# sshaoshuai/PointRCNN

Hardware: AMD Instinct MI355X
Metric: KITTI frames/sec, RPN inference end-to-end (16384 pts/frame, bs32 per GPU) (higher is better)
Workload: dtype f32 via split-bf16x6 MFMA (every fp32 operand cut exactly into 3 bf16 pieces, 6 bf16 MFMA products per fp32 product, fp32 accumulate: fp32-grade, measured error 2.9e-7 of sum|x||w| vs 3.0e-7 for the fp32-MFMA kernel; hoisted grouped layers on the split kernel too, unhoisted grouped first layers (xyz; 1 GPU; Full RPN PointNet++ backbone (4 SA-MSG + 4 FP) + cls/reg heads, tools/cfgs/default.yaml, 16384 pts/frame, batch 32 per GPU, random-init weights, eval-mode BN; frames_per_gpu=32, npoints=16384, parallelism=frames sharded, dp1, launch=hipGraph replay, streams=20, hw_queues=4, proposal_layer=normal, clouds=uniform, group_dedup=True, roi_dedup=True

## Files before the change

include/prcnn_pointops.h:

```cpp
#ifndef PRCNN_POINTOPS_H
#define PRCNN_POINTOPS_H

#include <stddef.h>
#include <stdint.h>

#ifdef __cplusplus
extern "C" {
#endif

typedef void* prcnn_stream_t;

#define PRCNN_OK 0
#define PRCNN_EINVAL (-1)
#define PRCNN_EHIP (-2)
#define PRCNN_EUNSUPPORTED (-3)

int prcnn_abi_version(void);
const char* prcnn_last_error(void);
const char* prcnn_build_id(void);
int prcnn_switches_reload(void);
int prcnn_switch_get(const char* name, int* set, long* num);


int prcnn_fps(const float* xyz, int B, int N, int npoint, float* tmp, int32_t* idx, prcnn_stream_t stream);

int prcnn_fps_nested(const float* xyz, const int32_t* prev_idx, int B, int N, int npoint, float* tmp, int32_t* idx, int32_t* skip,
                     prcnn_stream_t stream);

int prcnn_fps_status(void);

#define PRCNN_FPS_ORDER_CANONICAL 0
#define PRCNN_FPS_ORDER_UPSTREAM 1
int prcnn_fps_order(const float* xyz, int B, int N, int npoint, int order, float* tmp, int32_t* idx, prcnn_stream_t stream);

#define PRCNN_ARITH_CANONICAL 0
#define PRCNN_ARITH_UPSTREAM 1
int prcnn_fps_mode(const float* xyz, int B, int N, int npoint, int order, int arith, float* tmp, int32_t* idx, prcnn_stream_t stream);
int prcnn_ball_query_arith(const float* xyz, const float* new_xyz, int B, int N, int M, float radius, int nsample, int arith,
                           int32_t* idx, prcnn_stream_t stream);
int prcnn_three_nn_arith(const float* unknown, const float* known, int B, int n, int m, int arith, float* dist2, int32_t* idx,
                         prcnn_stream_t stream);

int prcnn_gather(const float* feat, const int32_t* idx, int B, int C, int N, int M, float* out, prcnn_stream_t stream);
int prcnn_gather_grad(const float* grad_out, const int32_t* idx, int B, int C, int N, int M, float* grad_feat,
                      prcnn_stream_t stream);

int prcnn_gather_rows(const float* in_cl, int ld_in, const int32_t* idx, int B, int N, int M, int C, float* out,
                      prcnn_stream_t stream);

int prcnn_ball_query(const float* xyz, const float* new_xyz, int B, int N, int M, float radius, int nsample,
                     int32_t* idx, prcnn_stream_t stream);
int prcnn_ball_query2(const float* xyz, const float* new_xyz, int B, int N, int M, float radius_a, int nsample_a,
                      int32_t* idx_a, float radius_b, int nsample_b, int32_t* idx_b, prcnn_stream_t stream);

int prcnn_group(const float* feat, const int32_t* idx, int B, int C, int N, int M, int nsample, float* out,
                prcnn_stream_t stream);
int prcnn_group_grad(const float* grad_out, const int32_t* idx, int B, int C, int N, int M, int nsample,
                     float* grad_feat, prcnn_stream_t stream);

int prcnn_three_nn(const float* unknown, const float* known, int B, int n, int m, float* dist2, int32_t* idx,
                   float* weight, prcnn_stream_t stream);

int prcnn_three_interp(const float* feat, const int32_t* idx, const float* weight, int B, int C, int m, int n,
                       float* out, prcnn_stream_t stream);
int prcnn_three_interp_grad(const float* grad_out, const int32_t* idx, const float* weight, int B, int C, int n,
                            int m, float* grad_feat, float* workspace, prcnn_stream_t stream);


size_t prcnn_wpack_floats(int Nout, int K);
int prcnn_pack_weight(const float* w, int Nout, int K, int k_rot, float* wpack, prcnn_stream_t stream);

int prcnn_mlp_rows(const float* in, int ld_in, int64_t rows, int K, const float* wpack, const float* bias, int Nout,
                   int relu, float* out, int ld_out, int col_off, int pool_ns, const int32_t* rows_dev, int rows_unit,
                   const int32_t* seg_cnt, int seg_rows, prcnn_stream_t stream);

int prcnn_mlp_group(const float* xyz, const float* new_xyz, const int32_t* idx, const float* feat_cl, int ld_feat,
                    int B, int N, int M, int nsample, int C, const float* act_wx, const float* act_bias,
                    const float* wpack, const float* bias, int Nout, int relu, float* out, int ld_out, int col_off,
                    int pool_ns, const int32_t* groups_dev, prcnn_stream_t stream);

int prcnn_mlp_interp(const float* known_cl, int ld_known, const int32_t* idx3, const float* w3, const float* skip_cl,
                     int ld_skip, int B, int n, int m, int C2, int C1, const float* act_bias, const float* wpack,
                     const float* bias, int Nout, int relu, float* out, int ld_out, int col_off,
                     prcnn_stream_t stream);

int prcnn_mlp_rows_addinterp(const float* in, int ld_in, int K, const float* wpack, const float* bias, int Nout,
                             int relu, const float* y_cl, int ld_y, const int32_t* idx3, const float* w3, int B, int n,
                             int m, float* out, int ld_out, int col_off, prcnn_stream_t stream);

size_t prcnn_wsplit_bytes(int Nout, int K);
int prcnn_pack_weight_split(const float* w, int Nout, int K, int chain, void* wsplit, prcnn_stream_t stream);
int prcnn_mlp_rows_split(const float* in, int ld_in, int64_t rows, int K, const float* wpack, const void* wsplit, int terms,
                         const float* bias, int Nout, int relu, float* out, int ld_out, int col_off, int pool_ns,
                         const int32_t* rows_dev, int rows_unit, const int32_t* seg_cnt, int seg_rows, prcnn_stream_t stream);
int prcnn_mlp_chain_rows_split(const float* in, int ld_in, int64_t rows, int K, const void* const* wchain, const float* const* wpack,
                               const float* const* bias, const int* nout, const int* relu, int terms, float* out, int ld_out,
                               int col_off, prcnn_stream_t stream);
int prcnn_mlp_chain_interp_split(const float* known_cl, int ld_known, const int32_t* idx3, const float* w3, int B, int n, int m,
                                 int C2, const float* act_bias, const void* wchain, const float* wpack, const float* bias, int Nout,
                                 int relu, int terms, float* out, int ld_out, int col_off, prcnn_stream_t stream);
int prcnn_mlp_rows_addinterp_split(const float* in, int ld_in, int K, const float* wpack, const void* wsplit, int terms,
                                   const float* bias, int Nout, int relu, const float* y_cl, int ld_y, const int32_t* idx3,
                                   const float* w3, int B, int n, int m, float* out, int ld_out, int col_off,
                                   prcnn_stream_t stream);
int prcnn_mlp_group_split(const float* xyz, const float* new_xyz, const int32_t* idx, const float* feat_cl, int ld_feat, int B, int N,
                          int M, int nsample, int C, const float* act_wx, const float* act_bias, const float* wpack,
                          const void* wsplit, int terms, const float* bias, int Nout, int relu, float* out, int ld_out, int col_off,
                          int pool_ns, const int32_t* groups_dev, prcnn_stream_t stream);

int prcnn_mlp_chain_supported(int mode, int nlayers, const int* nout, int pool_ns);
int prcnn_mlp_chain_rows(const float* in, int ld_in, int64_t rows, int K, int nlayers, const float* const* wpack,
                         const float* const* bias, const int* nout, const int* relu, float* out, int ld_out,
                         int col_off, int pool_ns, const int32_t* seg_cnt, int seg_rows, prcnn_stream_t stream);
int prcnn_mlp_chain_group(const float* xyz, const float* new_xyz, const int32_t* idx, const float* feat_cl,
                          int ld_feat, int B, int N, int M, int nsample, int C, const float* act_wx,
                          const float* act_bias, int nlayers,
                          const float* const* wpack, const float* const* bias, const int* nout, const int* relu,
                          float* out, int ld_out, int col_off, int pool_ns, const int32_t* groups_dev, prcnn_stream_t stream);
int prcnn_mlp_chain_interp(const float* known_cl, int ld_known, const int32_t* idx3, const float* w3,
                           const float* skip_cl, int ld_skip, int B, int n, int m, int C2, int C1,
                           const float* act_bias, int nlayers, const float* const* wpack, const float* const* bias, const int* nout, const int* relu,
                           float* out, int ld_out, int col_off, prcnn_stream_t stream);

typedef struct prcnn_chain_group_problem {
    const float* xyz; const float* new_xyz; const int32_t* idx; const float* feat_cl;
    const float* act_wx; const float* act_bias;
    const float* const* wpack; const float* const* bias; const int* nout; const int* relu;
    float* out; const int32_t* groups_dev;
    int ld_feat, B, N, M, nsample, C, nlayers, ld_out, col_off, pool_ns;
} prcnn_chain_group_problem_t;
int prcnn_mlp_chain_group_multi(int nprob, const prcnn_chain_group_problem_t* prob, prcnn_stream_t stream);

int prcnn_maxpool_rows(const float* in, int ld_in, int64_t rows_out, int ns, int C, float* out, int ld_out,
                       int col_off, prcnn_stream_t stream);

int prcnn_roipool3d(const float* xyz, const float* boxes3d, const float* feat, int B, int N, int M, int C, int S,
                    float* pooled, int32_t* empty, prcnn_stream_t stream);
size_t prcnn_roipool3d_work_bytes(int B, int N);
int prcnn_roipool3d_ws(const float* xyz, const float* boxes3d, const float* feat, int B, int N, int M, int C, int S, float* pooled,
                       int32_t* empty, void* work, size_t work_bytes, prcnn_stream_t stream);

int prcnn_pts_in_boxes3d(const float* pts, const float* boxes3d, int N, int M, int32_t* flags, prcnn_stream_t stream);

int prcnn_rpn_labels(const float* pts, const float* gt_boxes3d, const int32_t* num_gt, int B, int N, int G, float extra_width,
                     int32_t* cls_label, float* reg_label, prcnn_stream_t stream);

int prcnn_gt_aug_edit(const float* pts, const float* intensity, const int32_t* num_pts, const float* boxes3d,
                      const int32_t* num_boxes, float extra_h, const float* new_pts, const float* new_intensity,
                      const int32_t* num_new, int B, int N, int K, int P, float* out_pts, float* out_intensity,
                      int32_t* out_count, int32_t* removed, prcnn_stream_t stream);

int prcnn_corner_iou3d(const float* corners_a, int N, const float* corners_b, int M, float* iou3d, float* iou_bev, prcnn_stream_t stream);

int prcnn_gt_aug_sample(const float* gt_boxes3d, const int32_t* num_gt, const double* planes, int B, int G, const float* db_boxes, const float* db_alpha, const int32_t* db_npts, int D, const int32_t* easy_idx, int E, const int32_t* hard_idx, int H, const double* cfg4, const double* scope, int try_times, int K, uint32_t seed, int32_t* count, int32_t* db_id, float* boxes3d, float* alpha, double* y_shift, int32_t* stats, int32_t* status, prcnn_stream_t stream);

int prcnn_host_pts_in_boxes3d(const float* pts, const float* boxes3d, int64_t N, int64_t M, int64_t* flags);
int prcnn_host_roipool3d(const float* pts, const float* boxes3d, const float* feat, int64_t N, int64_t M, int64_t C, int64_t S,
                         float* pooled_pts, float* pooled_feat, int64_t* empty);

int prcnn_boxes_overlap_bev(const float* boxes_a, int Na, const float* boxes_b, int Nb, float* out,
                            prcnn_stream_t stream);
int prcnn_boxes_iou_bev(const float* boxes_a, int Na, const float* boxes_b, int Nb, float* out, prcnn_stream_t stream);

#define PRCNN_NMS_ROTATED 0
#define PRCNN_NMS_NORMAL 1
size_t prcnn_nms_workspace_bytes(int N);
int prcnn_nms(const float* boxes, int N, float thresh, int kind, int max_keep, int64_t* keep, int32_t* num_keep,
              void* workspace, size_t workspace_bytes, prcnn_stream_t stream);


int prcnn_decode_bbox_target(const float* roi, int roi_cols, const float* pred_reg, long N, int C, double loc_scope,
                             double loc_bin_size, int num_head_bin, const float* anchor_size_host, int get_xz_fine,
                             int get_y_by_bin, double loc_y_scope, double loc_y_bin_size, int get_ry_fine, int y_to_bottom,
                             float* out, prcnn_stream_t stream);

size_t prcnn_proposal_workspace_bytes(int B, int N, int pre_max, int post_max);
int prcnn_proposal_layer(const float* scores, const float* boxes3d, int B, int N, int use_range, float r0, float r1, float r2,
                         int pre1, int pre2, int post1, int post2, float nms_thresh, int nms_kind, float* out_boxes,
                         float* out_scores, int32_t* out_count, void* workspace, size_t workspace_bytes, prcnn_stream_t stream);

size_t prcnn_nms_batched_workspace_bytes(int B, int M);
int prcnn_nms_batched(const float* boxes3d, const float* scores, const uint8_t* valid, int B, int M, float thresh, int kind,
                      int max_keep, int32_t* keep, int32_t* num_keep, void* workspace, size_t workspace_bytes,
                      prcnn_stream_t stream);

int prcnn_roipool3d_canonical(const float* xyz, const float* pool_boxes3d, const float* rois, const float* extra0,
                              const float* extra1, const float* feat, int ld_feat, int B, int N, int M, int C, int S,
                              float* out_pts, int ld_pts, float* out_feat, int ld_out, int32_t* empty, int32_t* distinct,
                              prcnn_stream_t stream);
int prcnn_roipool3d_canonical_ws(const float* xyz, const float* pool_boxes3d, const float* rois, const float* extra0,
                                 const float* extra1, const float* feat, int ld_feat, int B, int N, int M, int C, int S,
                                 float* out_pts, int ld_pts, float* out_feat, int ld_out, int32_t* empty, int32_t* distinct,
                                 void* work, size_t work_bytes, prcnn_stream_t stream);

size_t prcnn_grid_bytes(int B, int N);
int prcnn_grid_build(const float* xyz, int B, int N, float min_cell, int cells_per_axis, void* grid, size_t grid_bytes,
                     prcnn_stream_t stream);
int prcnn_ball_query2_grid(const void* grid, const float* xyz, const float* new_xyz, int B, int N, int M, float radius_a,
                           int nsample_a, int32_t* idx_a, float radius_b, int nsample_b, int32_t* idx_b, prcnn_stream_t stream);
int prcnn_three_nn_grid(const void* grid, const float* unknown, int B, int n, int m, float* dist2, int32_t* idx, float* weight,
                        prcnn_stream_t stream);

int prcnn_rotate_iou_eval(const float* boxes, int N, const float* query, int K, int criterion, float* out, prcnn_stream_t stream);
int prcnn_kitti_overlaps(int metric, const double* dt, const int32_t* dt_off, const double* gt, const int32_t* gt_off,
                         const int64_t* ov_off, int F, double* out, prcnn_stream_t stream);
int prcnn_kitti_statistics(const double* overlaps, const int64_t* ov_off, const double* gt_datas, const int32_t* gt_off,
                           const double* dt_datas, const int32_t* dt_off, const int32_t* ign_gt, const int32_t* ign_det,
                           const double* dc, const int32_t* dc_off, int F, int max_det_per_frame, int metric, double min_overlap,
                           const double* thresholds, int T, int compute_fp, int compute_aos, double* res, double* matched,
                           prcnn_stream_t stream);

int prcnn_group_compact(const int32_t* idx, const float* new_xyz, int B, int N, int M, int nsample, int sparse_max,
                        const int32_t* valid_n, int32_t* ridx, float* rnx, int32_t* slist, int32_t* soff, int32_t* scnt,
                        int32_t* idxn, float* nxn, int32_t* listn, int32_t* counts, prcnn_stream_t stream);
int prcnn_segmax_scatter(const float* src, int ld_src, const int32_t* list, const int32_t* off, const int32_t* cnt,
                         const int32_t* count, int max_groups, int C, float* dst, int ld_dst, int col_off, prcnn_stream_t stream);
int prcnn_scatter_rows(const float* src, int ld_src, const int32_t* list, const int32_t* count, int max_rows, int C, float* dst,
                       int ld_dst, int col_off, prcnn_stream_t stream);
int prcnn_group_compact_pair(const int32_t* idx_a, int ns_a, int T_a, const int32_t* idx_b, int ns_b, int T_b, const float* new_xyz,
                             int B, int N, int M, void* const* lists_a, void* const* lists_b, int32_t* counts, prcnn_stream_t stream);
int prcnn_level_pool(int nprob, const float* const* src, const int* ld_src, const int32_t* const* list, const int32_t* const* off,
                     const int32_t* const* cnt, const int32_t* const* count, const int* max_items, const int* C, const int* col_off,
                     float* dst, int ld_dst, prcnn_stream_t stream);

size_t prcnn_scene_workspace_bytes(int64_t total_points, int B);
int prcnn_scene_prepare(const float* raw, const int64_t* offsets, int B, int64_t total_points, int max_points_per_frame,
                        const float* calib, const int32_t* img_hw, const double* scope, int npoints, uint32_t seed,
                        float* out_xyz, float* out_intensity, int32_t* out_src, int32_t* nvalid, int32_t* status,
                        void* workspace, size_t workspace_bytes, prcnn_stream_t stream);

size_t prcnn_train_scene_workspace_bytes(int64_t total_points, int B, int K, int db_max_points);
int prcnn_train_scene_prepare(const float* raw, const int64_t* offsets, int B, int64_t total_points, int max_points_per_frame,
                              const float* calib, const int32_t* img_hw, const double* scope, int npoints, uint32_t seed,
                              const float* gt_boxes3d, const float* gt_alpha, const int32_t* num_gt, int G,
                              const int32_t* acc_count, const int32_t* acc_db_id, const float* acc_boxes3d, const float* acc_alpha,
                              const double* acc_y_shift, const int32_t* acc_status, int K, const float* db_points,
                              const float* db_intensity, const int64_t* db_offsets, int D, int db_max_points,
                              const double* aug_cfg, float* out_xyz, float* out_input, float* out_features, int32_t* out_src,
                              int32_t* nvalid, int32_t* status, float* out_gt_boxes3d, int32_t* out_num_gt, double* aug,
                              void* workspace, size_t workspace_bytes, prcnn_stream_t stream);

size_t prcnn_gt_database_workspace_bytes(int64_t max_points_per_frame, int B, int G);
int prcnn_gt_database_count(const float* raw, const int64_t* offsets, int B, int64_t total_points, int max_points_per_frame,
                            const float* calib, const float* boxes3d, const int32_t* num_boxes, int G, int32_t* npts,
                            void* workspace, size_t workspace_bytes, prcnn_stream_t stream);
int prcnn_gt_database_fill(const float* raw, const int64_t* offsets, int B, int64_t total_points, int max_points_per_frame,
                           const float* calib, const float* boxes3d, const int32_t* num_boxes, int G, const int64_t* obj_offsets,
                           int64_t total_out, float* points, float* intensity, int32_t* src, void* workspace,
                           size_t workspace_bytes, prcnn_stream_t stream);

int prcnn_aug_scene_sample(const float* gt_boxes3d, const int32_t* num_gt, const double* planes, const int32_t* frame_ids, int B, int G,
                           const float* db_boxes, const int32_t* db_npts, int D, const double* scope, int K, uint32_t seed,
                           int32_t* count, int32_t* db_id, float* boxes3d, double* y_shift, int32_t* stats, int32_t* status,
                           prcnn_stream_t stream);
size_t prcnn_aug_scene_workspace_bytes(int64_t max_points_per_frame, int B);
int prcnn_aug_scene_count(const float* raw, const int64_t* offsets, int B, int64_t total_points, int max_points_per_frame,
                          const float* calib, const int32_t* img_hw, const double* scope, const int32_t* acc_count,
                          const int32_t* acc_db_id, const float* acc_boxes3d, const int32_t* acc_status, int K,
                          const int64_t* db_offsets, int D, int64_t db_total_points, int32_t* rows, void* workspace,
                          size_t workspace_bytes, prcnn_stream_t stream);
int prcnn_aug_scene_fill(const float* raw, const int64_t* offsets, int B, int64_t total_points, int max_points_per_frame,
                         const float* calib, const int32_t* img_hw, const double* scope, const int32_t* acc_count,
                         const int32_t* acc_db_id, const float* acc_boxes3d, const double* acc_y_shift, const int32_t* acc_status,
                         int K, const float* db_points, const float* db_intensity, const int64_t* db_offsets, int D,
                         int64_t db_total_points, const int64_t* out_offsets, int64_t total_out, float* out, int32_t* src,
                         void* workspace, size_t workspace_bytes, prcnn_stream_t stream);

typedef struct prcnn_train_src {
    int mode;
    int64_t rows;
    int K;
    const float* in; int ld_in; const float* pro_scale; const float* pro_shift;
    const float* xyz; const float* new_xyz; const int32_t* idx; const float* feat; int ld_feat; int B, N, M, ns, C;
    const float* known; const int32_t* idx3; const float* w3; const float* skip; int ld_known, ld_skip, n, m, C2, C1;
    const float* mult; const int32_t* rows_dev; int64_t norm_rows; const int32_t* seg_off; const int32_t* seg_cnt; const int32_t* row_grp;
    int groups;
} prcnn_train_src_t;

typedef struct prcnn_train_layer {
    int Nout;
    const float* W; const float* gamma; const float* beta;
    float eps, momentum;
    float* running_mean; float* running_var;
    float* y;
    float* cst; int ld_c;
    float* wpack; float* wpack_t;
    float* dW; float* dgamma; float* dbeta;
} prcnn_train_layer_t;

size_t prcnn_train_stack_work_bytes(int64_t rows, const prcnn_train_layer_t* layers, int nl, int K0, int backward);
int prcnn_train_stack_fwd(const prcnn_train_src_t* src, const prcnn_train_layer_t* layers, int nl, int pool_ns, float* a_dump, int ld_dump,
                          float* out, int ld_out, int col_off, uint8_t* arg, void* work, size_t work_bytes, prcnn_stream_t stream);
int prcnn_train_stack_bwd(const prcnn_train_src_t* src, const prcnn_train_layer_t* layers, int nl, int pool_ns, const float* a_dump,
                          int ld_dump, const float* gout, int ld_gout, const uint8_t* arg, float* gin, int ld_gin, void* work,
                          size_t work_bytes, prcnn_stream_t stream);
int prcnn_train_stack_fwd_split(const prcnn_train_src_t* src, const prcnn_train_layer_t* layers, int nl, int pool_ns, float* a_dump,
                                int ld_dump, float* out, int ld_out, int col_off, uint8_t* arg, void* const* wsplit, void* work,
                                size_t work_bytes, prcnn_stream_t stream);
int prcnn_train_stack_bwd_split(const prcnn_train_src_t* src, const prcnn_train_layer_t* layers, int nl, int pool_ns, const float* a_dump,
                                int ld_dump, const float* gout, int ld_gout, const uint8_t* arg, float* gin, int ld_gin,
                                void* const* wsplit_t, void* work, size_t work_bytes, prcnn_stream_t stream);
int prcnn_train_stack_bwd_wsplit(const prcnn_train_src_t* src, const prcnn_train_layer_t* layers, int nl, int pool_ns, const float* a_dump,
                                 int ld_dump, const float* gout, int ld_gout, const uint8_t* arg, float* gin, int ld_gin,
                                 void* const* wsplit_t, void* work, size_t work_bytes, prcnn_stream_t stream);
int prcnn_train_group_rows(const int32_t* idx, const float* new_xyz, int B, int N, int M, int ns, int32_t* cnt, int32_t* off,
                           int32_t* rows_dev, int32_t* ridx, float* rnx, float* mult, int32_t* row_grp, prcnn_stream_t stream);
int prcnn_flat_rows_grad(const float* G, int ldG, const int32_t* ridx, const int32_t* rows_dev, int64_t max_rows, int C, float* dfeat,
                         int ld_d, prcnn_stream_t stream);
size_t prcnn_flat_rows_grad_work_bytes(int B, int N, int64_t max_rows);
int prcnn_flat_rows_grad_ws(const float* G, int ldG, const int32_t* ridx, const int32_t* rows_dev, int64_t max_rows, int C, float* dfeat,
                            int ld_d, const int32_t* seg_off, int B, int N, int M, void* work, size_t work_bytes, prcnn_stream_t stream);
int prcnn_group_rows_grad(const float* G, int ldG, const int32_t* idx, int B, int M, int ns, int C, int N, float* dfeat, int ld_d,
                          prcnn_stream_t stream);
int prcnn_interp_rows_grad(const float* G, int ldG, const int32_t* idx3, const float* w3, int B, int n, int m, int C, float* dknown,
                           int ld_d, prcnn_stream_t stream);
size_t prcnn_interp_rows_grad_work_bytes(int B, int n, int m);
int prcnn_interp_rows_grad_ws(const float* G, int ldG, const int32_t* idx3, const float* w3, int B, int n, int m, int C, float* dknown,
                              int ld_d, void* work, size_t work_bytes, prcnn_stream_t stream);

int prcnn_boxes_iou3d(const float* a, int Na, const float* b, int Nb, float* out, prcnn_stream_t stream);
int prcnn_ref_trig(const float* a, const float* b, int n, int fn, float* out, prcnn_stream_t stream);
int prcnn_proposal_target_sample(const float* roi_boxes3d, const float* gt_boxes3d, int B, int M, int G, int gt_cols, int roi_per_image,
                                 const double* cfg6, int aug_times, int aug_method, uint32_t seed, float* rois, float* gt_of_rois,
                                 float* roi_iou, int32_t* src, float* max_overlaps, int32_t* gt_assignment, int32_t* counts,
                                 int32_t* status, prcnn_stream_t stream);

int prcnn_rcnn_offline_sample(const float* roi_boxes3d, const int32_t* num_roi, const float* gt_boxes3d, const int32_t* num_gt,
                              const int32_t* frame_ids, int B, int M, int G, int roi_per_image, const double* cfg6, int aug_times,
                              int aug_method, uint32_t seed, float* iou3d, float* rois, float* gt_of_rois, float* roi_iou, int32_t* src,
                              float* max_overlaps, int32_t* gt_assignment, int32_t* counts, int32_t* status, prcnn_stream_t stream);

int prcnn_rcnn_offline_finish(float* pooled, int ld, int B, int R, int S, const float* rois, const float* gt_of_rois,
                              const float* roi_iou, const int32_t* pooled_empty_flag, const int32_t* status, const int32_t* frame_ids,
                              const double* cfg5, int aug_methods, uint32_t seed, float* out_rois, float* out_gt_of_rois,
                              float* gt_boxes3d_ct, int32_t* cls_label, int32_t* reg_valid_mask, prcnn_stream_t stream);

typedef struct prcnn_rpn_loss_cfg {
    double loc_scope, loc_bin_size;
    double mean_size[3];
    double gamma, alpha;
    double loss_weight[2];
    int num_head_bin, xz_fine, y_by_bin, ry_fine;
    int loss_cls;
    int has_alpha;
} prcnn_rpn_loss_cfg_t;
size_t prcnn_rpn_loss_workspace_bytes(int64_t npts);
int prcnn_rpn_loss_counts(const void* cls_label, int label_is_i64, int64_t npts, int32_t* counts, float* norm, void* work,
                          size_t work_bytes, prcnn_stream_t stream);
int prcnn_rpn_loss_forward(const float* rpn_cls, int64_t ld_cls, const float* rpn_reg, int64_t ld_reg, const void* cls_label,
                           int label_is_i64, const float* reg_label, int64_t npts, int C, const prcnn_rpn_loss_cfg_t* cfg,
                           const int32_t* counts, const float* norm, float* terms, void* work, size_t work_bytes, prcnn_stream_t stream);
int prcnn_rpn_loss_backward(const float* rpn_cls, int64_t ld_cls, const float* rpn_reg, int64_t ld_reg, const void* cls_label,
                            int label_is_i64, const float* reg_label, int64_t npts, int C, const prcnn_rpn_loss_cfg_t* cfg,
                            const int32_t* counts, const float* norm, const float* grad_out, float* dcls, float* dreg,
                            prcnn_stream_t stream);
int prcnn_rpn_loss_cls_sums(const float* rpn_cls, int64_t ld_cls, const void* cls_label, int label_is_i64, int64_t npts, double* cls_sums,
                            void* work, size_t work_bytes, prcnn_stream_t stream);
int prcnn_rpn_loss_forward_kind(const float* rpn_cls, int64_t ld_cls, const float* rpn_reg, int64_t ld_reg, const void* cls_label,
                                int label_is_i64, const float* reg_label, int64_t npts, int C, const prcnn_rpn_loss_cfg_t* cfg,
                                const int32_t* counts, const float* norm, float* terms, void* work, size_t work_bytes,
                                const double* cls_sums, double fg_weight, prcnn_stream_t stream);
int prcnn_rpn_loss_backward_kind(const float* rpn_cls, int64_t ld_cls, const float* rpn_reg, int64_t ld_reg, const void* cls_label,
                                 int label_is_i64, const float* reg_label, int64_t npts, int C, const prcnn_rpn_loss_cfg_t* cfg,
                                 const int32_t* counts, const float* norm, const float* grad_out, float* dcls, float* dreg,
                                 const double* cls_sums, double fg_weight, prcnn_stream_t stream);

typedef struct prcnn_rcnn_loss_cfg {
    double loc_scope, loc_bin_size;
    double loc_y_scope, loc_y_bin_size;
    double mean_size[3];
    double gamma, alpha;
    int num_head_bin, y_by_bin, size_res_on_roi;
    int loss_cls;
    int has_alpha;
} prcnn_rcnn_loss_cfg_t;
size_t prcnn_rcnn_loss_workspace_bytes(int64_t npts);
// ... 65 lines not shown
```

pointrcnn_amd/_cabi.py:

```python
import contextlib
import ctypes
import os

from . import build as _build

_P = ctypes.c_void_p
_I = ctypes.c_int
_F = ctypes.c_float
_L = ctypes.c_int64
_Z = ctypes.c_size_t
_D = ctypes.c_double
_U = ctypes.c_uint32



class TrainSrc(ctypes.Structure):
    _fields_ = [("mode", _I), ("rows", _L), ("K", _I),
                ("in_", _P), ("ld_in", _I), ("pro_scale", _P), ("pro_shift", _P),
                ("xyz", _P), ("new_xyz", _P), ("idx", _P), ("feat", _P), ("ld_feat", _I),
                ("B", _I), ("N", _I), ("M", _I), ("ns", _I), ("C", _I),
                ("known", _P), ("idx3", _P), ("w3", _P), ("skip", _P), ("ld_known", _I), ("ld_skip", _I),
                ("n", _I), ("m", _I), ("C2", _I), ("C1", _I),
                ("mult", _P), ("rows_dev", _P), ("norm_rows", _L), ("seg_off", _P), ("seg_cnt", _P), ("row_grp", _P), ("groups", _I)]


class TrainLayer(ctypes.Structure):
    _fields_ = [("Nout", _I), ("W", _P), ("gamma", _P), ("beta", _P), ("eps", _F), ("momentum", _F),
                ("running_mean", _P), ("running_var", _P), ("y", _P), ("cst", _P), ("ld_c", _I), ("wpack", _P), ("wpack_t", _P),
                ("dW", _P), ("dgamma", _P), ("dbeta", _P)]


class ChainGroupProblem(ctypes.Structure):
    _fields_ = [("xyz", _P), ("new_xyz", _P), ("idx", _P), ("feat_cl", _P), ("act_wx", _P), ("act_bias", _P),
                ("wpack", _P), ("bias", _P), ("nout", _P), ("relu", _P), ("out", _P), ("groups_dev", _P),
                ("ld_feat", _I), ("B", _I), ("N", _I), ("M", _I), ("nsample", _I), ("C", _I), ("nlayers", _I), ("ld_out", _I),
                ("col_off", _I), ("pool_ns", _I)]


class RpnLossCfg(ctypes.Structure):
    _fields_ = [("loc_scope", _D), ("loc_bin_size", _D), ("mean_size", _D * 3), ("gamma", _D), ("alpha", _D), ("loss_weight", _D * 2),
                ("num_head_bin", _I), ("xz_fine", _I), ("y_by_bin", _I), ("ry_fine", _I), ("loss_cls", _I), ("has_alpha", _I)]


class RcnnLossCfg(ctypes.Structure):
    _fields_ = [("loc_scope", _D), ("loc_bin_size", _D), ("loc_y_scope", _D), ("loc_y_bin_size", _D), ("mean_size", _D * 3), ("gamma", _D),
                ("alpha", _D), ("num_head_bin", _I), ("y_by_bin", _I), ("size_res_on_roi", _I), ("loss_cls", _I), ("has_alpha", _I)]


REQUIRED_ABI = 12

SIGNATURES = {
    "prcnn_abi_version": (_I, []),
    "prcnn_last_error": (ctypes.c_char_p, []),
    "prcnn_build_id": (ctypes.c_char_p, []),
    "prcnn_switches_reload": (_I, []),
    "prcnn_switch_get": (_I, [ctypes.c_char_p, ctypes.POINTER(_I), ctypes.POINTER(ctypes.c_long)]),
    "prcnn_fps": (_I, [_P, _I, _I, _I, _P, _P, _P]),
    "prcnn_fps_nested": (_I, [_P, _P, _I, _I, _I, _P, _P, _P, _P]),
    "prcnn_fps_status": (_I, []),
    "prcnn_fps_order": (_I, [_P, _I, _I, _I, _I, _P, _P, _P]),
    "prcnn_fps_mode": (_I, [_P, _I, _I, _I, _I, _I, _P, _P, _P]),
    "prcnn_ball_query_arith": (_I, [_P, _P, _I, _I, _I, _F, _I, _I, _P, _P]),
    "prcnn_three_nn_arith": (_I, [_P, _P, _I, _I, _I, _I, _P, _P, _P]),
    "prcnn_rpn_labels": (_I, [_P, _P, _P, _I, _I, _I, _F, _P, _P, _P]),
    "prcnn_gt_aug_edit": (_I, [_P, _P, _P, _P, _P, _F, _P, _P, _P, _I, _I, _I, _I, _P, _P, _P, _P, _P]),
    "prcnn_corner_iou3d": (_I, [_P, _I, _P, _I, _P, _P, _P]),
    "prcnn_gt_aug_sample": (_I, [_P, _P, _P, _I, _I, _P, _P, _P, _I, _P, _I, _P, _I, _P, _P, _I, _I, ctypes.c_uint32,
                                 _P, _P, _P, _P, _P, _P, _P, _P]),
    "prcnn_host_pts_in_boxes3d": (_I, [_P, _P, _L, _L, _P]),
    "prcnn_host_roipool3d": (_I, [_P, _P, _P, _L, _L, _L, _L, _P, _P, _P]),
    "prcnn_gather": (_I, [_P, _P, _I, _I, _I, _I, _P, _P]),
    "prcnn_gather_grad": (_I, [_P, _P, _I, _I, _I, _I, _P, _P]),
    "prcnn_gather_rows": (_I, [_P, _I, _P, _I, _I, _I, _I, _P, _P]),
    "prcnn_ball_query": (_I, [_P, _P, _I, _I, _I, _F, _I, _P, _P]),
    "prcnn_ball_query2": (_I, [_P, _P, _I, _I, _I, _F, _I, _P, _F, _I, _P, _P]),
    "prcnn_group": (_I, [_P, _P, _I, _I, _I, _I, _I, _P, _P]),
    "prcnn_group_grad": (_I, [_P, _P, _I, _I, _I, _I, _I, _P, _P]),
    "prcnn_three_nn": (_I, [_P, _P, _I, _I, _I, _P, _P, _P, _P]),
    "prcnn_three_interp": (_I, [_P, _P, _P, _I, _I, _I, _I, _P, _P]),
    "prcnn_three_interp_grad": (_I, [_P, _P, _P, _I, _I, _I, _I, _P, _P, _P]),
    "prcnn_wpack_floats": (_Z, [_I, _I]),
    "prcnn_pack_weight": (_I, [_P, _I, _I, _I, _P, _P]),
    "prcnn_mlp_rows": (_I, [_P, _I, _L, _I, _P, _P, _I, _I, _P, _I, _I, _I, _P, _I, _P, _I, _P]),
    "prcnn_mlp_group": (_I, [_P, _P, _P, _P, _I, _I, _I, _I, _I, _I, _P, _P, _P, _P, _I, _I, _P, _I, _I, _I, _P, _P]),
    "prcnn_mlp_group_split": (_I, [_P, _P, _P, _P, _I, _I, _I, _I, _I, _I, _P, _P, _P, _P, _I, _P, _I, _I, _P, _I, _I, _I, _P, _P]),
    "prcnn_mlp_interp": (_I, [_P, _I, _P, _P, _P, _I, _I, _I, _I, _I, _I, _P, _P, _P, _I, _I, _P, _I, _I, _P]),
    "prcnn_mlp_rows_addinterp": (_I, [_P, _I, _I, _P, _P, _I, _I, _P, _I, _P, _P, _I, _I, _I, _P, _I, _I, _P]),
    "prcnn_wsplit_bytes": (_Z, [_I, _I]),
    "prcnn_pack_weight_split": (_I, [_P, _I, _I, _I, _P, _P]),
    "prcnn_mlp_chain_interp_split": (_I, [_P, _I, _P, _P, _I, _I, _I, _I, _P, _P, _P, _P, _I, _I, _I, _P, _I, _I, _P]),
    "prcnn_mlp_chain_rows_split": (_I, [_P, _I, _L, _I, _P, _P, _P, _P, _P, _I, _P, _I, _I, _P]),
    "prcnn_mlp_rows_split": (_I, [_P, _I, _L, _I, _P, _P, _I, _P, _I, _I, _P, _I, _I, _I, _P, _I, _P, _I, _P]),
    "prcnn_mlp_rows_addinterp_split": (_I, [_P, _I, _I, _P, _P, _I, _P, _I, _I, _P, _I, _P, _P, _I, _I, _I, _P, _I, _I, _P]),
    "prcnn_mlp_chain_supported": (_I, [_I, _I, _P, _I]),
    "prcnn_mlp_chain_rows": (_I, [_P, _I, _L, _I, _I, _P, _P, _P, _P, _P, _I, _I, _I, _P, _I, _P]),
    "prcnn_mlp_chain_group": (_I, [_P, _P, _P, _P, _I, _I, _I, _I, _I, _I, _P, _P, _I, _P, _P, _P, _P, _P, _I, _I, _I, _P, _P]),
    "prcnn_mlp_chain_interp": (_I, [_P, _I, _P, _P, _P, _I, _I, _I, _I, _I, _I, _P, _I, _P, _P, _P, _P, _P, _I, _I, _P]),
    "prcnn_mlp_chain_group_multi": (_I, [_I, _P, _P]),
    "prcnn_maxpool_rows": (_I, [_P, _I, _L, _I, _I, _P, _I, _I, _P]),
    "prcnn_roipool3d": (_I, [_P, _P, _P, _I, _I, _I, _I, _I, _P, _P, _P]),
    "prcnn_roipool3d_work_bytes": (_Z, [_I, _I]),
    "prcnn_roipool3d_ws": (_I, [_P, _P, _P, _I, _I, _I, _I, _I, _P, _P, _P, _Z, _P]),
    "prcnn_pts_in_boxes3d": (_I, [_P, _P, _I, _I, _P, _P]),
    "prcnn_boxes_overlap_bev": (_I, [_P, _I, _P, _I, _P, _P]),
    "prcnn_boxes_iou_bev": (_I, [_P, _I, _P, _I, _P, _P]),
    "prcnn_nms_workspace_bytes": (_Z, [_I]),
    "prcnn_nms": (_I, [_P, _I, _F, _I, _I, _P, _P, _P, _Z, _P]),
    "prcnn_decode_bbox_target": (_I, [_P, _I, _P, ctypes.c_long, _I, _D, _D, _I, _P, _I, _I, _D, _D, _I, _I, _P, _P]),
    "prcnn_proposal_workspace_bytes": (_Z, [_I, _I, _I, _I]),
    "prcnn_proposal_layer": (_I, [_P, _P, _I, _I, _I, _F, _F, _F, _I, _I, _I, _I, _F, _I, _P, _P, _P, _P, _Z, _P]),
    "prcnn_nms_batched_workspace_bytes": (_Z, [_I, _I]),
    "prcnn_roipool3d_canonical": (_I, [_P, _P, _P, _P, _P, _P, _I, _I, _I, _I, _I, _I, _P, _I, _P, _I, _P, _P, _P]),
    "prcnn_roipool3d_canonical_ws": (_I, [_P, _P, _P, _P, _P, _P, _I, _I, _I, _I, _I, _I, _P, _I, _P, _I, _P, _P, _P, _Z, _P]),
    "prcnn_grid_bytes": (_Z, [_I, _I]),
    "prcnn_grid_build": (_I, [_P, _I, _I, _F, _I, _P, _Z, _P]),
    "prcnn_ball_query2_grid": (_I, [_P, _P, _P, _I, _I, _I, _F, _I, _P, _F, _I, _P, _P]),
    "prcnn_three_nn_grid": (_I, [_P, _P, _I, _I, _I, _P, _P, _P, _P]),
    "prcnn_rotate_iou_eval": (_I, [_P, _I, _P, _I, _I, _P, _P]),
    "prcnn_kitti_overlaps": (_I, [_I, _P, _P, _P, _P, _P, _I, _P, _P]),
    "prcnn_kitti_statistics": (_I, [_P, _P, _P, _P, _P, _P, _P, _P, _P, _P, _I, _I, _I, _D, _P, _I, _I, _I, _P, _P, _P]),
    "prcnn_group_compact": (_I, [_P, _P, _I, _I, _I, _I, _I, _P, _P, _P, _P, _P, _P, _P, _P, _P, _P, _P]),
    "prcnn_segmax_scatter": (_I, [_P, _I, _P, _P, _P, _P, _I, _I, _P, _I, _I, _P]),
    "prcnn_scatter_rows": (_I, [_P, _I, _P, _P, _I, _I, _P, _I, _I, _P]),
    "prcnn_group_compact_pair": (_I, [_P, _I, _I, _P, _I, _I, _P, _I, _I, _I, _P, _P, _P, _P]),
    "prcnn_level_pool": (_I, [_I, _P, _P, _P, _P, _P, _P, _P, _P, _P, _P, _I, _P]),
    "prcnn_scene_workspace_bytes": (_Z, [_L, _I]),
    "prcnn_scene_prepare": (_I, [_P, _P, _I, _L, _I, _P, _P, _P, _I, ctypes.c_uint32, _P, _P, _P, _P, _P, _P, _Z, _P]),
    "prcnn_train_scene_workspace_bytes": (_Z, [_L, _I, _I, _I]),
    "prcnn_train_scene_prepare": (_I, [_P, _P, _I, _L, _I, _P, _P, _P, _I, ctypes.c_uint32, _P, _P, _P, _I, _P, _P, _P, _P, _P, _P, _I,
                                       _P, _P, _P, _I, _I, _P, _P, _P, _P, _P, _P, _P, _P, _P, _P, _P, _Z, _P]),
    "prcnn_gt_database_workspace_bytes": (_Z, [_L, _I, _I]),
    "prcnn_gt_database_count": (_I, [_P, _P, _I, _L, _I, _P, _P, _P, _I, _P, _P, _Z, _P]),
    "prcnn_gt_database_fill": (_I, [_P, _P, _I, _L, _I, _P, _P, _P, _I, _P, _L, _P, _P, _P, _P, _Z, _P]),
    "prcnn_aug_scene_sample": (_I, [_P, _P, _P, _P, _I, _I, _P, _P, _I, _P, _I, ctypes.c_uint32, _P, _P, _P, _P, _P, _P, _P]),
    "prcnn_aug_scene_workspace_bytes": (_Z, [_L, _I]),
    "prcnn_aug_scene_count": (_I, [_P, _P, _I, _L, _I, _P, _P, _P, _P, _P, _P, _P, _I, _P, _I, _L, _P, _P, _Z, _P]),
    "prcnn_aug_scene_fill": (_I, [_P, _P, _I, _L, _I, _P, _P, _P, _P, _P, _P, _P, _P, _I, _P, _P, _P, _I, _L, _P, _L, _P, _P, _P, _Z, _P]),
    "prcnn_nms_batched": (_I, [_P, _P, _P, _I, _I, _F, _I, _I, _P, _P, _P, _Z, _P]),
    "prcnn_train_stack_work_bytes": (_Z, [_L, ctypes.POINTER(TrainLayer), _I, _I, _I]),
    "prcnn_train_stack_fwd": (_I, [ctypes.POINTER(TrainSrc), ctypes.POINTER(TrainLayer), _I, _I, _P, _I, _P, _I, _I, _P, _P, _Z, _P]),
    "prcnn_train_stack_bwd": (_I, [ctypes.POINTER(TrainSrc), ctypes.POINTER(TrainLayer), _I, _I, _P, _I, _P, _I, _P, _P, _I, _P, _Z, _P]),
    "prcnn_train_stack_fwd_split": (_I, [ctypes.POINTER(TrainSrc), ctypes.POINTER(TrainLayer), _I, _I, _P, _I, _P, _I, _I, _P,
                                         ctypes.POINTER(_P), _P, _Z, _P]),
    "prcnn_train_stack_bwd_split": (_I, [ctypes.POINTER(TrainSrc), ctypes.POINTER(TrainLayer), _I, _I, _P, _I, _P, _I, _P, _P, _I,
                                         ctypes.POINTER(_P), _P, _Z, _P]),
    "prcnn_train_stack_bwd_wsplit": (_I, [ctypes.POINTER(TrainSrc), ctypes.POINTER(TrainLayer), _I, _I, _P, _I, _P, _I, _P, _P, _I,
                                          ctypes.POINTER(_P), _P, _Z, _P]),
    "prcnn_ref_trig": (_I, [_P, _P, _I, _I, _P, _P]),
    "prcnn_boxes_iou3d": (_I, [_P, _I, _P, _I, _P, _P]),
    "prcnn_proposal_target_sample": (_I, [_P, _P, _I, _I, _I, _I, _I, _P, _I, _I, ctypes.c_uint32, _P, _P, _P, _P, _P, _P, _P, _P, _P]),
    "prcnn_rcnn_offline_sample": (_I, [_P, _P, _P, _P, _P, _I, _I, _I, _I, _P, _I, _I, ctypes.c_uint32, _P, _P, _P, _P, _P, _P, _P, _P, _P, _P]),
    "prcnn_rcnn_offline_finish": (_I, [_P, _I, _I, _I, _I, _P, _P, _P, _P, _P, _P, _P, _I, ctypes.c_uint32, _P, _P, _P, _P, _P, _P]),
    "prcnn_train_group_rows": (_I, [_P, _P, _I, _I, _I, _I, _P, _P, _P, _P, _P, _P, _P, _P]),
    "prcnn_flat_rows_grad": (_I, [_P, _I, _P, _P, _L, _I, _P, _I, _P]),
    "prcnn_flat_rows_grad_work_bytes": (_Z, [_I, _I, _L]),
    "prcnn_flat_rows_grad_ws": (_I, [_P, _I, _P, _P, _L, _I, _P, _I, _P, _I, _I, _I, _P, _Z, _P]),
    "prcnn_group_rows_grad": (_I, [_P, _I, _P, _I, _I, _I, _I, _I, _P, _I, _P]),
    "prcnn_interp_rows_grad": (_I, [_P, _I, _P, _P, _I, _I, _I, _I, _P, _I, _P]),
    "prcnn_interp_rows_grad_work_bytes": (_Z, [_I, _I, _I]),
    "prcnn_interp_rows_grad_ws": (_I, [_P, _I, _P, _P, _I, _I, _I, _I, _P, _I, _P, _Z, _P]),
    "prcnn_rpn_loss_workspace_bytes": (_Z, [_L]),
    "prcnn_rpn_loss_counts": (_I, [_P, _I, _L, _P, _P, _P, _Z, _P]),
    "prcnn_rpn_loss_forward": (_I, [_P, _L, _P, _L, _P, _I, _P, _L, _I, ctypes.POINTER(RpnLossCfg), _P, _P, _P, _P, _Z, _P]),
    "prcnn_rpn_loss_backward": (_I, [_P, _L, _P, _L, _P, _I, _P, _L, _I, ctypes.POINTER(RpnLossCfg), _P, _P, _P, _P, _P, _P]),
    "prcnn_rpn_loss_cls_sums": (_I, [_P, _L, _P, _I, _L, _P, _P, _Z, _P]),
    "prcnn_rpn_loss_forward_kind": (_I, [_P, _L, _P, _L, _P, _I, _P, _L, _I, ctypes.POINTER(RpnLossCfg), _P, _P, _P, _P, _Z, _P, _D, _P]),
    "prcnn_rpn_loss_backward_kind": (_I, [_P, _L, _P, _L, _P, _I, _P, _L, _I, ctypes.POINTER(RpnLossCfg), _P, _P, _P, _P, _P, _P, _D, _P]),
    "prcnn_rcnn_loss_workspace_bytes": (_Z, [_L]),
    "prcnn_rcnn_loss_forward": (_I, [_P, _L, _P, _L, _P, _I, _P, _I, _P, _P, _L, _I, ctypes.POINTER(RcnnLossCfg), _I, _P, _P, _P, _Z, _P]),
    "prcnn_rcnn_loss_finalize": (_I, [_L, _I, ctypes.POINTER(RcnnLossCfg), _P, _P, _P, _P, _Z, _P]),
    "prcnn_rcnn_loss_backward": (_I, [_P, _L, _P, _L, _P, _I, _P, _I, _P, _P, _L, _I, ctypes.POINTER(RcnnLossCfg), _P, _P, _P, _P, _P, _P]),
    "prcnn_eval_stats_workspace_bytes": (_Z, [_I, _I, _I]),
    "prcnn_eval_gt_max_iou": (_I, [_P, _P, _I, _I, _I, _P, _I, _I, _I, _P, _P, _P]),
    "prcnn_eval_stats_accumulate": (_I, [_P, _P, _I, _I, _I, _P, _P, _P, _I, _L, _I, _P, _P, _I, _F, _F, _F, _P, _P]),
    "prcnn_optim_chunk_elems": (_Z, []),
    "prcnn_optim_grad_norm": (_I, [_P, _P, _L, _P, _P]),
    "prcnn_optim_step": (_I, [_P, _P, _L, _P, _F, _P, _P, _F, _F, _F, _F, _F, _F, _F, _P]),
    "prcnn_optim_step_adam": (_I, [_P, _P, _L, _P, _F, _P, _P, _F, _F, _F, _F, _F, _F, _F, _P]),
    "prcnn_optim_step_sgd": (_I, [_P, _P, _L, _P, _F, _P, _P, _F, _F, _F, _P]),
    "prcnn_kitti_result_text": (_I, [_P, _P, _P, _P, _I, _I, _P, _P, ctypes.c_char_p, _P, _P, _P, _P, _P, _P]),
    "prcnn_head_tail_fwd": (_I, [_P, _P, _P, _P, _L, _I, _I, _U, _U, _U, _F, _P]),
    "prcnn_head_tail_work_bytes": (_Z, [_L, _I, _I]),
    "prcnn_head_tail_bwd": (_I, [_P, _P, _P, _L, _P, _P, _P, _P, _Z, _L, _I, _I, _U, _U, _U, _F, _P]),
    "prcnn_dropout_rows": (_I, [_P, _P, _L, _I, _U, _U, _U, _F, _P]),
}

_lib = None


class PointOpsError(RuntimeError):
    pass


def library_path():
    return _build.LIB


def lib():
    global _lib
    if _lib is not None:
        return _lib
    import torch
    path = _build.LIB
    if not os.path.exists(path):
        try:
            _build.build(verbose=False)
        except Exception as e:
            raise PointOpsError(
                "libprcnn_pointops.so is missing and could not be built (%s). The HIP extension is "
                "mandatory: there is no CPU fallback. Run `python -m pointrcnn_amd.build`." % e)
    elif not os.environ.get("PRCNN_POINTOPS_LIB") and _build.have_sources() and _build.library_id(path) != _build.source_id():
        if not os.path.exists(_build.HIPCC):
            raise PointOpsError("%s is stale (built from %s, sources are %s) and hipcc is not available to rebuild it"
                                % (path, _build.library_id(path), _build.source_id()))
        try:
            _build.build(verbose=False)
        except Exception as e:
            raise PointOpsError("%s is stale and could not be rebuilt (%s)" % (path, e))
    try:
        handle = ctypes.CDLL(path)
    except OSError as e:
        raise PointOpsError("cannot load %s: %s" % (path, e))
    handle.prcnn_abi_version.restype = _I
    if handle.prcnn_abi_version() < REQUIRED_ABI:
        raise PointOpsError("%s implements ABI %d, this binding needs %d (include/prcnn_pointops.h)"
                            % (path, handle.prcnn_abi_version(), REQUIRED_ABI))
    for name, (res, args) in SIGNATURES.items():
        fn = getattr(handle, name)
        fn.restype = res
        fn.argtypes = args
    _lib = handle
    return handle


EUNSUPPORTED = -3


def check(rc, what=""):
    if rc != 0:
        msg = lib().prcnn_last_error()
        raise PointOpsError("%s failed (code %d): %s" % (what or "prcnn call", rc, msg.decode() if msg else "?"))


def switch_get(name):
    is_set, num = _I(), ctypes.c_long()
    check(lib().prcnn_switch_get(name.encode(), ctypes.byref(is_set), ctypes.byref(num)), "prcnn_switch_get")
    return bool(is_set.value), num.value


@contextlib.contextmanager
def switches(**env):
    for name in env:
        switch_get(name)
    old = {name: os.environ.get(name) for name in env}

    def apply(values):
        for name, value in values.items():
            if value is None:
                os.environ.pop(name, None)
            else:
                os.environ[name] = value
        lib().prcnn_switches_reload()
    apply(env)
    try:
        yield
    finally:
        apply(old)
```

pointrcnn_amd/csrc/dedup.hip:

```cpp
#include "common.h"

struct CompactParams {
    const int32_t* idx;
    const float* new_xyz;
    int32_t* ridx;
    float* rnx;
    int32_t* slist;
    int32_t* soff;
    int32_t* scnt;
    int32_t* idxn;
    float* nxn;
    int32_t* listn;
    int32_t* counts;
    const int32_t* valid_n;
    int G, N, M, ns, T;
};

constexpr int COMPACT_THREADS = 1024;
constexpr int DEDUP_GRID_CAP = 8192;

template <int NS>
__device__ __forceinline__ void group_compact_body(const CompactParams& P, int block, int (*wsum)[3], int* bbase) {
    const int g = block * COMPACT_THREADS + threadIdx.x;
    const int lane = threadIdx.x & 63;
    const bool ok = g < P.G;
    const int ns = NS > 0 ? NS : P.ns;
    int cnt = 0, first = 0;
    const int32_t* row = P.idx + (size_t)(ok ? g : 0) * ns;
    if (ok) {
        if constexpr (NS > 0) {
            int4 v[NS / 4];
#pragma unroll
            for (int q = 0; q < NS / 4; q++) v[q] = reinterpret_cast<const int4*>(row)[q];
            first = v[0].x;
            cnt = NS;
#pragma unroll
            for (int q = NS / 4 - 1; q >= 0; q--) {
                if (v[q].w == first) cnt = 4 * q + 3;
                if (v[q].z == first) cnt = 4 * q + 2;
                if (v[q].y == first) cnt = 4 * q + 1;
                if (q > 0 && v[q].x == first) cnt = 4 * q;
            }
        } else {
            first = row[0];
            cnt = ns;
            for (int s = 1; s < ns; s++)
                if (row[s] == first) { cnt = s; break; }
        }
    }
    const int b = (ok ? g : 0) / P.M;
    const int vn = P.valid_n ? P.valid_n[b] : P.N;
    if (ok && P.valid_n) {
        int c2 = 0;
        while (c2 < cnt && row[c2] < vn) c2++;
        cnt = c2 > 0 ? c2 : 1;
    }
    const bool sparse = ok && cnt <= P.T, dense = ok && cnt > P.T;
    const int v = sparse ? cnt : 0;
    int incl = v;
#pragma unroll
    for (int d = 1; d < 64; d <<= 1) {
        const int t = __shfl_up(incl, d);
        if (lane >= d) incl += t;
    }
    const int total = __shfl(incl, 63);
    const unsigned long long bs = __ballot(sparse), bd = __ballot(dense);
    const int wave = threadIdx.x >> 6;
    if (lane == 0) { wsum[wave][0] = total; wsum[wave][1] = (int)__popcll(bd); wsum[wave][2] = (int)__popcll(bs); }
    __syncthreads();
    if (threadIdx.x < 3) {
        int t = 0;
        for (int w = 0; w < COMPACT_THREADS / 64; w++) t += wsum[w][threadIdx.x];
        bbase[threadIdx.x] = t > 0 ? atomicAdd(P.counts + threadIdx.x, t) : 0;
    }
    __syncthreads();
    int base_rows = bbase[0], base_d = bbase[1], base_s = bbase[2];
    for (int w = 0; w < wave; w++) { base_rows += wsum[w][0]; base_d += wsum[w][1]; base_s += wsum[w][2]; }
    const unsigned long long below = (1ULL << lane) - 1ULL;
    float c3[3] = {0.f, 0.f, 0.f};
    if (ok) {
#pragma unroll
        for (int c = 0; c < 3; c++) c3[c] = P.new_xyz[(size_t)g * 3 + c];
    }
    if (sparse) {
        const int j = base_s + (int)__popcll(bs & below), r0 = base_rows + incl - v;
        P.slist[j] = g; P.soff[j] = r0; P.scnt[j] = cnt;
        for (int s = 0; s < cnt; s++) {
            P.ridx[r0 + s] = b * P.N + row[s];
#pragma unroll
            for (int c = 0; c < 3; c++) P.rnx[(size_t)(r0 + s) * 3 + c] = c3[c];
        }
    }
    if (dense) {
        const int pn = base_d + (int)__popcll(bd & below);
        P.listn[pn] = g;
        for (int s = 0; s < ns; s++) P.idxn[(size_t)pn * ns + s] = b * P.N + (row[s] < vn ? row[s] : first);
#pragma unroll
        for (int c = 0; c < 3; c++) P.nxn[(size_t)pn * 3 + c] = c3[c];
    }
}

template <int NS>
__global__ __launch_bounds__(COMPACT_THREADS) void group_compact_kernel(CompactParams P) {
    __shared__ int wsum[COMPACT_THREADS / 64][3];
    __shared__ int bbase[3];
    group_compact_body<NS>(P, blockIdx.x, wsum, bbase);
}

template <int NSA, int NSB>
__global__ __launch_bounds__(COMPACT_THREADS) void group_compact_pair_kernel(CompactParams A, CompactParams B) {
    __shared__ int wsum[COMPACT_THREADS / 64][3];
    __shared__ int bbase[3];
    if (blockIdx.y == 0) group_compact_body<NSA>(A, blockIdx.x, wsum, bbase);
    else group_compact_body<NSB>(B, blockIdx.x, wsum, bbase);
}

__global__ __launch_bounds__(256) void scatter_rows_kernel(const float* __restrict__ src, int ld_src, const int32_t* __restrict__ list,
                                                           const int32_t* __restrict__ count, int C, float* __restrict__ dst, int ld_dst,
                                                           int col_off) {
    const long total = (long)(*count) * C;
    for (long e = (long)blockIdx.x * 256 + threadIdx.x; e < total; e += (long)gridDim.x * 256) {
        const long r = e / C;
        const int c = (int)(e - r * C);
        dst[(size_t)list[r] * ld_dst + col_off + c] = src[(size_t)r * ld_src + c];
    }
}

__global__ __launch_bounds__(256) void segmax_scatter_kernel(const float* __restrict__ src, int ld_src, const int32_t* __restrict__ list,
                                                             const int32_t* __restrict__ off, const int32_t* __restrict__ cnt,
                                                             const int32_t* __restrict__ count, int C, float* __restrict__ dst,
                                                             int ld_dst, int col_off) {
    const long total = (long)(*count) * C;
    for (long e = (long)blockIdx.x * 256 + threadIdx.x; e < total; e += (long)gridDim.x * 256) {
        const long j = e / C;
        const int c = (int)(e - j * C);
        const float* p = src + (size_t)off[j] * ld_src + c;
        const int rows = cnt[j];
        float m = p[0];
        for (int r = 1; r < rows; r++) m = fmaxf(m, p[(size_t)r * ld_src]);
        dst[(size_t)list[j] * ld_dst + col_off + c] = m;
    }
}

#define LEVEL_POOL_MAX 4
struct LevelPoolParams {
    const float* src[LEVEL_POOL_MAX];
    const int32_t* list[LEVEL_POOL_MAX];
    const int32_t* off[LEVEL_POOL_MAX];
    const int32_t* cnt[LEVEL_POOL_MAX];
    const int32_t* count[LEVEL_POOL_MAX];
    int ld_src[LEVEL_POOL_MAX], C[LEVEL_POOL_MAX], col_off[LEVEL_POOL_MAX];
    float* dst;
    int ld_dst;
};

__global__ __launch_bounds__(256) void level_pool_kernel(LevelPoolParams L) {
    const int q = blockIdx.y;
    const float* __restrict__ src = L.src[q];
    const int32_t* __restrict__ list = L.list[q];
    const int32_t* __restrict__ off = L.off[q];
    const int32_t* __restrict__ cnt = L.cnt[q];
    const int ld_src = L.ld_src[q], C = L.C[q], col_off = L.col_off[q], ld_dst = L.ld_dst;
    float* __restrict__ dst = L.dst;
    const long total = (long)(*L.count[q]) * C;
    if (off) {
        for (long e = (long)blockIdx.x * 256 + threadIdx.x; e < total; e += (long)gridDim.x * 256) {
            const long j = e / C;
            const int c = (int)(e - j * C);
            const float* p = src + (size_t)off[j] * ld_src + c;
            const int rows = cnt[j];
            float m = p[0];
            for (int r = 1; r < rows; r++) m = fmaxf(m, p[(size_t)r * ld_src]);
            dst[(size_t)list[j] * ld_dst + col_off + c] = m;
        }
    } else {
        for (long e = (long)blockIdx.x * 256 + threadIdx.x; e < total; e += (long)gridDim.x * 256) {
            const long r = e / C;
            const int c = (int)(e - r * C);
            dst[(size_t)list[r] * ld_dst + col_off + c] = src[(size_t)r * ld_src + c];
        }
    }
}

static int compact_check(const char* who, int B, int N, int M, int nsample, int sparse_max) {
    PRCNN_REQUIRE(B >= 0 && N > 0 && M >= 0 && nsample > 0, "%s: bad shape B=%d N=%d M=%d nsample=%d", who, B, N, M, nsample);
    PRCNN_REQUIRE(sparse_max >= 1 && sparse_max <= nsample, "%s: sparse_max=%d (1..nsample)", who, sparse_max);
    PRCNN_REQUIRE((long)B * N < 2147483647L && (long)B * M * sparse_max < 2147483647L, "%s: 32-bit row index overflow", who);
    return PRCNN_OK;
}

PRCNN_API int prcnn_group_compact_pair(const int32_t* idx_a, int ns_a, int T_a, const int32_t* idx_b, int ns_b, int T_b, const float* new_xyz,
                                       int B, int N, int M, void* const* lists_a, void* const* lists_b, int32_t* counts, prcnn_stream_t stream) {
    int rc = compact_check("prcnn_group_compact_pair", B, N, M, ns_a, T_a);
    if (rc) return rc;
    rc = compact_check("prcnn_group_compact_pair", B, N, M, ns_b, T_b);
    if (rc) return rc;
    PRCNN_REQUIRE(counts && lists_a && lists_b, "prcnn_group_compact_pair: null counts / list table");
    hipStream_t s = (hipStream_t)stream;
    if (prcnn_fill_words(counts, 0u, 6, s) != hipSuccess) return prcnn_fail(PRCNN_EHIP, "prcnn_group_compact_pair: clearing the counters failed");
    if (B == 0 || M == 0) return PRCNN_OK;
    PRCNN_REQUIRE(idx_a && idx_b && new_xyz, "prcnn_group_compact_pair: null pointer");
    CompactParams P[2];
    for (int q = 0; q < 2; q++) {
        void* const* L = q ? lists_b : lists_a;
        const int ns = q ? ns_b : ns_a, T = q ? T_b : T_a;
        for (int i = 0; i < 5; i++) PRCNN_REQUIRE(L[i], "prcnn_group_compact_pair: null pointer");
        PRCNN_REQUIRE(T == ns || (L[5] && L[6] && L[7]), "prcnn_group_compact_pair: null dense-list pointer");
        P[q].idx = q ? idx_b : idx_a; P[q].new_xyz = new_xyz;
        P[q].ridx = (int32_t*)L[0]; P[q].rnx = (float*)L[1]; P[q].slist = (int32_t*)L[2]; P[q].soff = (int32_t*)L[3]; P[q].scnt = (int32_t*)L[4];
        P[q].idxn = (int32_t*)L[5]; P[q].nxn = (float*)L[6]; P[q].listn = (int32_t*)L[7];
        P[q].counts = counts + 3 * q; P[q].valid_n = nullptr; P[q].G = B * M; P[q].N = N; P[q].M = M; P[q].ns = ns; P[q].T = T;
    }
    const dim3 grid(prcnn_divup(B * M, COMPACT_THREADS), 2);
    const bool vec = ((uintptr_t)idx_a % 16) == 0 && ((uintptr_t)idx_b % 16) == 0;
    if (vec && ns_a == 16 && ns_b == 32) hipLaunchKernelGGL((group_compact_pair_kernel<16, 32>), grid, dim3(COMPACT_THREADS), 0, s, P[0], P[1]);
    else hipLaunchKernelGGL((group_compact_pair_kernel<0, 0>), grid, dim3(COMPACT_THREADS), 0, s, P[0], P[1]);
    PRCNN_LAUNCH_CHECK("prcnn_group_compact_pair");
    return PRCNN_OK;
}

PRCNN_API int prcnn_level_pool(int nprob, const float* const* src, const int* ld_src, const int32_t* const* list, const int32_t* const* off,
                               const int32_t* const* cnt, const int32_t* const* count, const int* max_items, const int* C, const int* col_off,
                               float* dst, int ld_dst, prcnn_stream_t stream) {
    PRCNN_REQUIRE(nprob >= 1 && nprob <= LEVEL_POOL_MAX, "prcnn_level_pool: nprob=%d (1..%d)", nprob, LEVEL_POOL_MAX);
    PRCNN_REQUIRE(src && ld_src && list && off && cnt && count && max_items && C && col_off, "prcnn_level_pool: null table");
    LevelPoolParams L = {};
    int n = 0;
    long need = 0;
    for (int q = 0; q < nprob; q++) {
        PRCNN_REQUIRE(max_items[q] >= 0 && C[q] > 0 && ld_src[q] >= C[q] && ld_dst >= col_off[q] + C[q] && col_off[q] >= 0,
                      "prcnn_level_pool: bad shape of problem %d", q);
        if (max_items[q] == 0) continue;
        PRCNN_REQUIRE(src[q] && list[q] && count[q] && dst && (!off[q] || cnt[q]), "prcnn_level_pool: null pointer in problem %d", q);
        L.src[n] = src[q]; L.list[n] = list[q]; L.off[n] = off[q]; L.cnt[n] = cnt[q]; L.count[n] = count[q];
        L.ld_src[n] = ld_src[q]; L.C[n] = C[q]; L.col_off[n] = col_off[q];
        need = max(need, (long)prcnn_divup((long)max_items[q] * C[q], 256));
        n++;
    }
    if (n == 0) return PRCNN_OK;
    L.dst = dst; L.ld_dst = ld_dst;
    hipLaunchKernelGGL(level_pool_kernel, dim3((unsigned)min(need, (long)(DEDUP_GRID_CAP / 2)), n), dim3(256), 0, (hipStream_t)stream, L);
    PRCNN_LAUNCH_CHECK("prcnn_level_pool");
    return PRCNN_OK;
}

PRCNN_API int prcnn_group_compact(const int32_t* idx, const float* new_xyz, int B, int N, int M, int nsample, int sparse_max,
                                  const int32_t* valid_n, int32_t* ridx, float* rnx, int32_t* slist, int32_t* soff, int32_t* scnt,
                                  int32_t* idxn, float* nxn, int32_t* listn, int32_t* counts, prcnn_stream_t stream) {
    PRCNN_REQUIRE(B >= 0 && N > 0 && M >= 0 && nsample > 0, "prcnn_group_compact: bad shape B=%d N=%d M=%d nsample=%d", B, N, M, nsample);
    PRCNN_REQUIRE(sparse_max >= 1 && sparse_max <= nsample, "prcnn_group_compact: sparse_max=%d (1..nsample)", sparse_max);
    PRCNN_REQUIRE(counts, "prcnn_group_compact: null counts");
    hipStream_t s = (hipStream_t)stream;
    if (prcnn_fill_words(counts, 0u, 3, s) != hipSuccess) return prcnn_fail(PRCNN_EHIP, "prcnn_group_compact: clearing the counters failed");
    if (B == 0 || M == 0) return PRCNN_OK;
    PRCNN_REQUIRE((long)B * N < 2147483647L && (long)B * M * sparse_max < 2147483647L, "prcnn_group_compact: 32-bit row index overflow");
    PRCNN_REQUIRE(idx && new_xyz && ridx && rnx && slist && soff && scnt, "prcnn_group_compact: null pointer");
    PRCNN_REQUIRE(sparse_max == nsample || (idxn && nxn && listn), "prcnn_group_compact: null dense-list pointer");
    CompactParams P;
    P.idx = idx; P.new_xyz = new_xyz; P.ridx = ridx; P.rnx = rnx; P.slist = slist; P.soff = soff; P.scnt = scnt;
    P.idxn = idxn; P.nxn = nxn; P.listn = listn;
    P.counts = counts; P.valid_n = valid_n; P.G = B * M; P.N = N; P.M = M; P.ns = nsample; P.T = sparse_max;
    const dim3 grid(prcnn_divup(P.G, COMPACT_THREADS));
    const bool vec = ((uintptr_t)idx % 16) == 0;
    if (vec && nsample == 16) hipLaunchKernelGGL(group_compact_kernel<16>, grid, dim3(COMPACT_THREADS), 0, s, P);
    else if (vec && nsample == 32) hipLaunchKernelGGL(group_compact_kernel<32>, grid, dim3(COMPACT_THREADS), 0, s, P);
    else if (vec && nsample == 64) hipLaunchKernelGGL(group_compact_kernel<64>, grid, dim3(COMPACT_THREADS), 0, s, P);
    else hipLaunchKernelGGL(group_compact_kernel<0>, grid, dim3(COMPACT_THREADS), 0, s, P);
    PRCNN_LAUNCH_CHECK("prcnn_group_compact");
    return PRCNN_OK;
}

PRCNN_API int prcnn_segmax_scatter(const float* src, int ld_src, const int32_t* list, const int32_t* off, const int32_t* cnt,
                                   const int32_t* count, int max_groups, int C, float* dst, int ld_dst, int col_off,
                                   prcnn_stream_t stream) {
    PRCNN_REQUIRE(max_groups >= 0 && C > 0 && ld_src >= C && ld_dst >= col_off + C, "prcnn_segmax_scatter: bad shape");
    if (max_groups == 0) return PRCNN_OK;
    PRCNN_REQUIRE(src && list && off && cnt && count && dst, "prcnn_segmax_scatter: null pointer");
    hipLaunchKernelGGL(segmax_scatter_kernel, dim3(min(prcnn_divup((long)max_groups * C, 256), DEDUP_GRID_CAP)), dim3(256), 0, (hipStream_t)stream, src, ld_src,
                       list, off, cnt, count, C, dst, ld_dst, col_off);
    PRCNN_LAUNCH_CHECK("prcnn_segmax_scatter");
    return PRCNN_OK;
}

PRCNN_API int prcnn_scatter_rows(const float* src, int ld_src, const int32_t* list, const int32_t* count, int max_rows, int C, float* dst,
                                 int ld_dst, int col_off, prcnn_stream_t stream) {
    PRCNN_REQUIRE(max_rows >= 0 && C > 0 && ld_src >= C && ld_dst >= col_off + C, "prcnn_scatter_rows: bad shape");
    if (max_rows == 0) return PRCNN_OK;
    PRCNN_REQUIRE(src && list && count && dst, "prcnn_scatter_rows: null pointer");
    hipLaunchKernelGGL(scatter_rows_kernel, dim3(min(prcnn_divup((long)max_rows * C, 256), DEDUP_GRID_CAP)), dim3(256), 0, (hipStream_t)stream, src, ld_src, list,
                       count, C, dst, ld_dst, col_off);
    PRCNN_LAUNCH_CHECK("prcnn_scatter_rows");
    return PRCNN_OK;
}
```

pointrcnn_amd/csrc/mlp.hip:

```cpp
#include "common.h"
#include "switches.h"

#define MLP_BM 128
#define MLP_BN 64
#define MLP_BK 32
#define MLP_THREADS 256
#define MLP_ALD 36

typedef float f32x16 __attribute__((ext_vector_type(16)));

enum { MODE_PLAIN = 0, MODE_GROUP = 1, MODE_INTERP = 2 };

struct MlpParams {
    long rows;
    int K, KB, NB;
    const float* wpack;
    const float* bias;
    int Nout, relu;
    float* out;
    int ld_out, col_off, pool_ns;
    const float* in;
    int ld_in;
    const float* xyz;
    const float* new_xyz;
    const int32_t* idx;
    const float* feat;
    int ld_feat, N, M, ns, C;
    const float* known;
    const int32_t* idx3;
    const float* w3;
    const float* skip;
    int ld_known, ld_skip, n, m, C2, C1;
    int vec_a, vec_b;
    int act;
    const float* act_wx;
    const float* act_bias;
    const float* addY;
    int ldY;
    const int32_t* rows_dev;
    int rows_unit;
    const int32_t* seg_cnt;
    int seg_rows;
    int xcd_tpf;
    int wgm_cols;
    int addy_phase;
    const void* wsplit;
    int split_terms;
};

__device__ __forceinline__ long tile_of_block(const MlpParams& P, long bid) {
    if (P.xcd_tpf > 0) {
        const long xcd = bid & 7, slot = bid >> 3;
        const long k = slot / P.xcd_tpf, t = slot - k * P.xcd_tpf;
        return (k * 8 + xcd) * P.xcd_tpf + t;
    }
    if (!P.seg_cnt) return bid;
    const long nseg = P.rows / P.seg_rows, tps = P.seg_rows / 128;
    const long q = bid / nseg, sg = bid - q * nseg;
    return sg * tps + q;
}
__device__ __forceinline__ bool tile_dead(const MlpParams& P, long row0) {
    if (!P.seg_cnt) return false;
    const long s = row0 / P.seg_rows;
    return (int)(row0 - s * P.seg_rows) >= P.seg_cnt[s];
}
__device__ __forceinline__ long effective_rows(const MlpParams& P) {
    if (!P.rows_dev) return P.rows;
    const long r = (long)(*P.rows_dev) * P.rows_unit;
    return r < P.rows ? r : P.rows;
}

template <int MODE> struct RowMeta;
template <> struct RowMeta<MODE_PLAIN> { long off; bool valid; };
template <> struct RowMeta<MODE_GROUP> { long off; float dx, dy, dz; bool valid; };
template <> struct RowMeta<MODE_INTERP> { long o0, o1, o2, os; float w0, w1, w2; bool valid; };

template <int MODE> struct Raw;
template <> struct Raw<MODE_PLAIN> { float4 a; };
template <> struct Raw<MODE_GROUP> { float4 a; };
template <> struct Raw<MODE_INTERP> { float4 a, b, c; };

__host__ __device__ static inline bool aligned16(const void* p) { return (reinterpret_cast<uintptr_t>(p) & 15) == 0; }

__device__ __forceinline__ float4 ld4(const float* p) { return *reinterpret_cast<const float4*>(p); }

template <int MODE> __device__ __forceinline__ void make_meta(const MlpParams& P, long grow, RowMeta<MODE>& r);

template <> __device__ __forceinline__ void make_meta<MODE_PLAIN>(const MlpParams& P, long grow, RowMeta<MODE_PLAIN>& r) {
    r.valid = grow < P.rows;
    r.off = r.valid ? grow * (long)P.ld_in : 0;
}
template <> __device__ __forceinline__ void make_meta<MODE_GROUP>(const MlpParams& P, long grow, RowMeta<MODE_GROUP>& r) {
    r.valid = grow < P.rows;
    r.off = 0; r.dx = r.dy = r.dz = 0.f;
    if (r.valid) {
        long per_b = (long)P.M * P.ns;
        int b = (int)(grow / per_b);
        int m_ = (int)((grow - (long)b * per_b) / P.ns);
        int p = P.idx[grow];
        long pt = (long)b * P.N + p;
        r.off = pt * (long)P.ld_feat;
        float x = P.xyz[pt * 3], y = P.xyz[pt * 3 + 1], z = P.xyz[pt * 3 + 2];
        if (P.new_xyz) {
            const float* q = P.new_xyz + ((long)b * P.M + m_) * 3;
            x = x - q[0]; y = y - q[1]; z = z - q[2];
        }
        r.dx = x; r.dy = y; r.dz = z;
    }
}
template <> __device__ __forceinline__ void make_meta<MODE_INTERP>(const MlpParams& P, long grow, RowMeta<MODE_INTERP>& r) {
    r.valid = grow < P.rows;
    r.o0 = r.o1 = r.o2 = r.os = 0; r.w0 = r.w1 = r.w2 = 0.f;
    if (r.valid) {
        int b = (int)(grow / P.n);
        const int32_t* id = P.idx3 + grow * 3;
        const float* w = P.w3 + grow * 3;
        long base = (long)b * P.m;
        r.o0 = (base + id[0]) * (long)P.ld_known;
        r.o1 = (base + id[1]) * (long)P.ld_known;
        r.o2 = (base + id[2]) * (long)P.ld_known;
        r.os = grow * (long)P.ld_skip;
        r.w0 = w[0]; r.w1 = w[1]; r.w2 = w[2];
    }
}

template <int MODE> __device__ __forceinline__ void fetch(const MlpParams& P, const RowMeta<MODE>& r, int k, Raw<MODE>& v);
template <int MODE> __device__ __forceinline__ float4 finish(const MlpParams& P, const RowMeta<MODE>& r, int k, const Raw<MODE>& v);

template <> __device__ __forceinline__ void fetch<MODE_PLAIN>(const MlpParams& P, const RowMeta<MODE_PLAIN>& r, int k, Raw<MODE_PLAIN>& v) {
    v.a = make_float4(0.f, 0.f, 0.f, 0.f);
    if (!r.valid || k >= P.K) return;
    const float* s = P.in + r.off + k;
    if (P.vec_a && k + 4 <= P.K) { v.a = ld4(s); return; }
    v.a.x = s[0];
    if (k + 1 < P.K) v.a.y = s[1];
    if (k + 2 < P.K) v.a.z = s[2];
    if (k + 3 < P.K) v.a.w = s[3];
}
template <> __device__ __forceinline__ float4 finish<MODE_PLAIN>(const MlpParams&, const RowMeta<MODE_PLAIN>&, int, const Raw<MODE_PLAIN>& v) {
    return v.a;
}

__device__ __forceinline__ float group_elem(const MlpParams& P, const RowMeta<MODE_GROUP>& r, int kk) {
    if (kk < P.C) return P.feat[r.off + kk];
    if (P.act) return 0.f;
    int t = kk - P.C;
    return t == 0 ? r.dx : (t == 1 ? r.dy : (t == 2 ? r.dz : 0.f));
}
template <> __device__ __forceinline__ void fetch<MODE_GROUP>(const MlpParams& P, const RowMeta<MODE_GROUP>& r, int k, Raw<MODE_GROUP>& v) {
    v.a = make_float4(0.f, 0.f, 0.f, 0.f);
    if (!r.valid || k >= P.K) return;
    if (P.vec_a && k + 4 <= P.C) { v.a = ld4(P.feat + r.off + k); return; }
    v.a.x = group_elem(P, r, k);
    v.a.y = group_elem(P, r, k + 1);
    v.a.z = group_elem(P, r, k + 2);
    v.a.w = group_elem(P, r, k + 3);
}
__device__ __forceinline__ float4 act_group4(const MlpParams& P, float4 z, int k, float dx, float dy, float dz) {
    const float4 w0 = ld4(P.act_wx + (long)k * 3), w1 = ld4(P.act_wx + (long)k * 3 + 4), w2 = ld4(P.act_wx + (long)k * 3 + 8);
    const float4 b = ld4(P.act_bias + k);
    float4 o;
    o.x = fmaxf(z.x + (w0.x * dx + w0.y * dy + w0.z * dz) + b.x, 0.f);
    o.y = fmaxf(z.y + (w0.w * dx + w1.x * dy + w1.y * dz) + b.y, 0.f);
    o.z = fmaxf(z.z + (w1.z * dx + w1.w * dy + w2.x * dz) + b.z, 0.f);
    o.w = fmaxf(z.w + (w2.y * dx + w2.z * dy + w2.w * dz) + b.w, 0.f);
    return o;
}
template <> __device__ __forceinline__ float4 finish<MODE_GROUP>(const MlpParams& P, const RowMeta<MODE_GROUP>& r, int k, const Raw<MODE_GROUP>& v) {
    if (!P.act || !r.valid || k >= P.K) return v.a;
    float4 o = act_group4(P, v.a, k, r.dx, r.dy, r.dz);
    if (k + 1 >= P.K) o.y = 0.f;
    if (k + 2 >= P.K) o.z = 0.f;
    if (k + 3 >= P.K) o.w = 0.f;
    return o;
}

__device__ __forceinline__ float interp1(float w0, float f0, float w1, float f1, float w2, float f2) {
    return __fadd_rn(__fadd_rn(__fmul_rn(w0, f0), __fmul_rn(w1, f1)), __fmul_rn(w2, f2));
}
template <> __device__ __forceinline__ void fetch<MODE_INTERP>(const MlpParams& P, const RowMeta<MODE_INTERP>& r, int k, Raw<MODE_INTERP>& v) {
    v.a = v.b = v.c = make_float4(0.f, 0.f, 0.f, 0.f);
    if (!r.valid || k >= P.K) return;
    if (k + 4 <= P.C2) {
        if (P.vec_a) {
            v.a = ld4(P.known + r.o0 + k); v.b = ld4(P.known + r.o1 + k); v.c = ld4(P.known + r.o2 + k);
        } else {
            const float *a = P.known + r.o0 + k, *b = P.known + r.o1 + k, *c = P.known + r.o2 + k;
            v.a = make_float4(a[0], a[1], a[2], a[3]);
            v.b = make_float4(b[0], b[1], b[2], b[3]);
            v.c = make_float4(c[0], c[1], c[2], c[3]);
        }
        return;
    }
    if (k >= P.C2) {
        int ks = k - P.C2;
        const float* s = P.skip + r.os + ks;
        if (P.vec_b && ks + 4 <= P.C1) { v.a = ld4(s); return; }
        if (ks < P.C1) v.a.x = s[0];
        if (ks + 1 < P.C1) v.a.y = s[1];
        if (ks + 2 < P.C1) v.a.z = s[2];
        if (ks + 3 < P.C1) v.a.w = s[3];
// ... 779 lines not shown
    for (int c = 0; c < nchunks; c += 2) {
        chunk_body(c, raB, raA);
        if (c + 1 < nchunks) chunk_body(c + 1, raA, raB);
    }
#undef SPL_STEP
#undef SPL_TERM
    if (PRCNN_ABL & (16 | 128)) {
        float sum = 0.f;
#pragma unroll
        for (int r = 0; r < 2; r++)
#pragma unroll
            for (int n = 0; n < WNB; n++)
#pragma unroll
                for (int e = 0; e < 16; e++) sum += acc[r][n][e];
        if (PRCNN_ABL & 128) {
#pragma unroll
            for (int r = 0; r < 2; r++)
#pragma unroll
                for (int p = 0; p < NP; p++) sum += (float)a0[r][p][0] + (float)a1[r][p][3] + __uint_as_float(bq[0][0][p].x) + __uint_as_float(bq[1][WNB - 1][p].w);
        }
        if (sum == 123.456f) P.out[tid] = sum;
        if (PRCNN_ABL & 16) return;
    }
    if (!(PRCNN_ABL & (16 | 128))) {
        bool bad = wave_has_nonfinite<2 * WNB>(reinterpret_cast<const f32x16 (&)[2 * WNB]>(acc));
        if (ADDY && addy_done) bad = __syncthreads_or(bad) != 0;
        if (bad && n_active) split_redo_f32<MODE, WNB>(P, acc, row0, wm, wn, nb0, lane);
        if (bad) addy_done = false;
    }
    layer_epilogue<MODE, WNB, ADDY>(P, acc, reinterpret_cast<float*>(Ls), nullptr, tid, row0, nb0, n_active, addy_done);
}

template <int MODE, int WNB, int TERMS, bool ADDY, bool LOOP>
__global__ __launch_bounds__(MLP_THREADS, 2) void mlp_layer_s_kernel(const MlpParams Pin) {
    MlpParams P = Pin;
    P.rows = effective_rows(Pin);
    __shared__ __attribute__((aligned(16))) unsigned char Ls[2 * 3 * SPL_PLANE];
    if constexpr (LOOP) {
        const long nbid = ((P.rows + MLP_BM - 1) / MLP_BM + 7) / 8 * 8 * P.wgm_cols;
        for (long bid = blockIdx.x; bid < nbid; bid += gridDim.x) {
            int tid;
            asm volatile("v_mov_b32 %0, %1" : "=v"(tid) : "v"(threadIdx.x));
            layer_s_tile<MODE, WNB, TERMS, ADDY>(P, bid, 0, tid, Ls);
            __syncthreads();
        }
    } else {
        layer_s_tile<MODE, WNB, TERMS, ADDY>(P, blockIdx.x, blockIdx.y, threadIdx.x, Ls);
    }
}

struct ChainParams {
    MlpParams a;
    const float* wpack1; const float* bias1; int KB1, N1, relu1;
    const float* wpack2; const float* bias2; int KB2, N2, relu2;
    int nlayers;
    int stack_split;
    const void* wsplit1;
};

#define CH_DPP_FMAX(v, ctrl) asm volatile("s_nop 1\n\tv_max_f32_dpp %0, %0, %0 " ctrl : "+v"(v))
#define CH_DPP_FMAX4(v, ctrl)                                                                                   \
    asm volatile("s_nop 1\n\tv_max_f32_dpp %0, %0, %0 " ctrl "\n\tv_max_f32_dpp %1, %1, %1 " ctrl               \
                 "\n\tv_max_f32_dpp %2, %2, %2 " ctrl "\n\tv_max_f32_dpp %3, %3, %3 " ctrl                       \
                 : "+v"(v[0]), "+v"(v[1]), "+v"(v[2]), "+v"(v[3]))

__device__ __forceinline__ float4 ldw(const float* __restrict__ wpack, int KB, int ob, int kb, int lane) {
    return ld4(wpack + (((long)ob * KB + kb) * 64 + lane) * 4);
}

template <int NB>
__device__ __forceinline__ void bias_act(f32x16 (&acc)[NB], const float* __restrict__ bias, int relu, int h) {
#pragma unroll
    for (int ob = 0; ob < NB; ob++)
#pragma unroll
        for (int q = 0; q < 4; q++) {
            float4 b = bias ? ld4(bias + ob * 32 + 8 * q + 4 * h) : make_float4(0.f, 0.f, 0.f, 0.f);
            float v0 = acc[ob][4 * q + 0] + b.x, v1 = acc[ob][4 * q + 1] + b.y;
            float v2 = acc[ob][4 * q + 2] + b.z, v3 = acc[ob][4 * q + 3] + b.w;
            if (relu) { v0 = fmaxf(v0, 0.f); v1 = fmaxf(v1, 0.f); v2 = fmaxf(v2, 0.f); v3 = fmaxf(v3, 0.f); }
            acc[ob][4 * q + 0] = v0; acc[ob][4 * q + 1] = v1; acc[ob][4 * q + 2] = v2; acc[ob][4 * q + 3] = v3;
        }
}

#define CH_WAVES 4
#define CH_STAGE_TILES 16
template <int NB> struct ChStage { static constexpr int G = CH_STAGE_TILES / NB; static constexpr int TPW = (G * NB + CH_WAVES - 1) / CH_WAVES; };

template <int NB>
__device__ __forceinline__ void stage_load(const float* __restrict__ wpack, int KB, int st, int wave, int lane, float4 (&r)[4]) {
    constexpr int G = ChStage<NB>::G;
#pragma unroll
    for (int u = 0; u < ChStage<NB>::TPW; u++) {
        int tt = wave + CH_WAVES * u, kbl = tt / NB, ob = tt - kbl * NB, kb = st * G + kbl;
        r[u] = (tt < G * NB && kb < KB) ? ldw(wpack, KB, ob, kb, lane) : make_float4(0.f, 0.f, 0.f, 0.f);
    }
}
template <int NB>
__device__ __forceinline__ void stage_store(float* ws, int wave, int lane, const float4 (&r)[4]) {
#pragma unroll
    for (int u = 0; u < ChStage<NB>::TPW; u++) {
        int tt = wave + CH_WAVES * u;
        if (tt < ChStage<NB>::G * NB) *reinterpret_cast<float4*>(ws + (tt * 64 + lane) * 4) = r[u];
    }
}
__device__ __forceinline__ float4 lds_w(const float* ws, int tile, int lane) {
    return *reinterpret_cast<const float4*>(ws + (tile * 64 + lane) * 4);
}

template <int NBI, int NBO>
__device__ __forceinline__ void chain_layer(const f32x16 (&in)[NBI], f32x16 (&out)[NBO], const float* __restrict__ wpack,
                                            int KB, float (*Ws)[CH_STAGE_TILES * 256], int wave, int lane) {
    constexpr int G = ChStage<NBO>::G;
    constexpr int NST = (NBI * 4 + G - 1) / G;
#pragma unroll
    for (int ob = 0; ob < NBO; ob++) out[ob] = (f32x16){0};
    float4 wr[4];
    stage_load<NBO>(wpack, KB, 0, wave, lane, wr);
    stage_store<NBO>(Ws[0], wave, lane, wr);
    __syncthreads();
#pragma unroll
    for (int st = 0; st < NST; st++) {
        if (st * G < KB) {
            const bool more = (st + 1) * G < KB;
            if (more) stage_load<NBO>(wpack, KB, st + 1, wave, lane, wr);
            const float* ws = Ws[st & 1];
#pragma unroll
            for (int kbl = 0; kbl < G; kbl++) {
                const int kb = st * G + kbl;
                if (kb < NBI * 4 && kb < KB) {
                    const int pb = kb < NBI * 4 ? kb / 4 : 0, q = kb % 4;
                    float4 w[NBO];
#pragma unroll
                    for (int ob = 0; ob < NBO; ob++) w[ob] = lds_w(ws, kbl * NBO + ob, lane);
#pragma unroll
                    for (int ob = 0; ob < NBO; ob++) out[ob] = __builtin_amdgcn_mfma_f32_32x32x2f32(w[ob].x, in[pb][4 * q + 0], out[ob], 0, 0, 0);
#pragma unroll
                    for (int ob = 0; ob < NBO; ob++) out[ob] = __builtin_amdgcn_mfma_f32_32x32x2f32(w[ob].y, in[pb][4 * q + 1], out[ob], 0, 0, 0);
#pragma unroll
                    for (int ob = 0; ob < NBO; ob++) out[ob] = __builtin_amdgcn_mfma_f32_32x32x2f32(w[ob].z, in[pb][4 * q + 2], out[ob], 0, 0, 0);
#pragma unroll
                    for (int ob = 0; ob < NBO; ob++) out[ob] = __builtin_amdgcn_mfma_f32_32x32x2f32(w[ob].w, in[pb][4 * q + 3], out[ob], 0, 0, 0);
                }
            }
            if (more) stage_store<NBO>(Ws[(st + 1) & 1], wave, lane, wr);
            __syncthreads();
        }
    }
}

template <int NB>
__device__ __forceinline__ void chain_store(const ChainParams& C, f32x16 (&acc)[NB], int Nlast, long row, bool valid,
                                            int lane, int h) {
    const MlpParams& P = C.a;
    const bool vec = ((P.ld_out | P.col_off) % 4 == 0) && aligned16(P.out);
    if (P.pool_ns == 0) {
        if (!valid) return;
        float* o = P.out + row * P.ld_out + P.col_off;
#pragma unroll
        for (int ob = 0; ob < NB; ob++)
#pragma unroll
            for (int q = 0; q < 4; q++) {
                int c = ob * 32 + 8 * q + 4 * h;
                if (c >= Nlast) continue;
                if (vec && c + 4 <= Nlast) {
                    *reinterpret_cast<float4*>(o + c) = make_float4(acc[ob][4 * q], acc[ob][4 * q + 1], acc[ob][4 * q + 2], acc[ob][4 * q + 3]);
                } else {
#pragma unroll
                    for (int s = 0; s < 4; s++)
                        if (c + s < Nlast) o[c + s] = acc[ob][4 * q + s];
                }
            }
        return;
    }
    const int j = lane & 31;
    const bool writer = P.pool_ns == 16 ? ((j & 15) == 15) : (j == 31);
    const long group = P.pool_ns == 16 ? (row / 16) : (row / 32);
    const long groups = P.rows / P.pool_ns;
    float* o = P.out + group * P.ld_out + P.col_off;
#pragma unroll
    for (int ob = 0; ob < NB; ob++)
#pragma unroll
        for (int q = 0; q < 4; q++) {
            float v[4] = {acc[ob][4 * q], acc[ob][4 * q + 1], acc[ob][4 * q + 2], acc[ob][4 * q + 3]};
            CH_DPP_FMAX4(v, "row_shr:1 row_mask:0xf bank_mask:0xf");
            CH_DPP_FMAX4(v, "row_shr:2 row_mask:0xf bank_mask:0xf");
            CH_DPP_FMAX4(v, "row_shr:4 row_mask:0xf bank_mask:0xf");
            CH_DPP_FMAX4(v, "row_shr:8 row_mask:0xf bank_mask:0xf");
            if (P.pool_ns == 32) CH_DPP_FMAX4(v, "row_bcast:15 row_mask:0xa bank_mask:0xf");
            asm volatile("s_nop 1");
            int c = ob * 32 + 8 * q + 4 * h;
            if (writer && valid && group < groups && c < Nlast) {
                if (vec && c + 4 <= Nlast) *reinterpret_cast<float4*>(o + c) = make_float4(v[0], v[1], v[2], v[3]);
                else {
#pragma unroll
                    for (int s = 0; s < 4; s++)
                        if (c + s < Nlast) o[c + s] = v[s];
                }
            }
        }
}

template <int NB>
__device__ __forceinline__ void chain_out1(const ChainParams& C, const f32x16 (&a)[NB], long row, bool valid, int lane, int h) {
    const MlpParams& P = C.a;
    float s0 = 0.f, s1 = 0.f, s2 = 0.f, s3 = 0.f;
#pragma unroll
    for (int ob = 0; ob < NB; ob++)
#pragma unroll
        for (int q = 0; q < 4; q++) {
            const float4 w = ld4(C.wpack1 + ((4 * ob + q) * 64 + h * 32) * 4);
            s0 = fmaf(a[ob][4 * q + 0], w.x, s0); s1 = fmaf(a[ob][4 * q + 1], w.y, s1);
            s2 = fmaf(a[ob][4 * q + 2], w.z, s2); s3 = fmaf(a[ob][4 * q + 3], w.w, s3);
        }
    float sum = (s0 + s1) + (s2 + s3);
    sum += __shfl_xor(sum, 32);
    sum += C.bias1 ? C.bias1[0] : 0.f;
    if (C.relu1) sum = fmaxf(sum, 0.f);
    if (valid && h == 0) P.out[row * P.ld_out + P.col_off] = sum;
}
template <int NB1, int NB2> __device__ __forceinline__ bool chain_out1_applies(const ChainParams& C) {
    return NB1 == 1 && NB2 == 0 && C.N1 == 1 && C.a.pool_ns == 0;
}

template <int MODE, int NB0, int NB1, int NB2>
__global__ __launch_bounds__(256) void mlp_chain_kernel(const ChainParams Cin) {
    ChainParams C = Cin;
    C.a.rows = effective_rows(Cin.a);
    const MlpParams& P = C.a;
    const long tile_id = tile_of_block(P, blockIdx.x);
    if (tile_id * 128 >= P.rows) return;
    if (tile_dead(P, tile_id * 128)) return;
    const int lane = threadIdx.x & 63, wave = threadIdx.x >> 6;
    const int h = lane >> 5, j = lane & 31;
    const long row = (tile_id * 4 + wave) * 32 + j;
    RowMeta<MODE> meta;
    make_meta<MODE>(P, row, meta);

    __shared__ __attribute__((aligned(16))) float Ws[2][CH_STAGE_TILES * 256];

    f32x16 a0[NB0];
#pragma unroll
    for (int ob = 0; ob < NB0; ob++) a0[ob] = (f32x16){0};
    {
        constexpr int G = ChStage<NB0>::G;
        const int nst = (P.KB + G - 1) / G;
        float4 wr[4];
        stage_load<NB0>(P.wpack, P.KB, 0, wave, lane, wr);
        Raw<MODE> cur, nxt;
        fetch<MODE>(P, meta, 4 * h, cur);
        stage_store<NB0>(Ws[0], wave, lane, wr);
        __syncthreads();
        for (int st = 0; st < nst; st++) {
            const bool more_st = st + 1 < nst;
            if (more_st) stage_load<NB0>(P.wpack, P.KB, st + 1, wave, lane, wr);
            const float* ws = Ws[st & 1];
            for (int kbl = 0; kbl < G; kbl++) {
                const int kb = st * G + kbl;
                if (kb >= P.KB) break;
                const bool more = kb + 1 < P.KB;
                if (more) fetch<MODE>(P, meta, 8 * (kb + 1) + 4 * h, nxt);
                float4 b = finish<MODE>(P, meta, 8 * kb + 4 * h, cur);
                float4 w[NB0];
#pragma unroll
                for (int ob = 0; ob < NB0; ob++) w[ob] = lds_w(ws, kbl * NB0 + ob, lane);
#pragma unroll
                for (int ob = 0; ob < NB0; ob++) a0[ob] = __builtin_amdgcn_mfma_f32_32x32x2f32(w[ob].x, b.x, a0[ob], 0, 0, 0);
#pragma unroll
                for (int ob = 0; ob < NB0; ob++) a0[ob] = __builtin_amdgcn_mfma_f32_32x32x2f32(w[ob].y, b.y, a0[ob], 0, 0, 0);
#pragma unroll
                for (int ob = 0; ob < NB0; ob++) a0[ob] = __builtin_amdgcn_mfma_f32_32x32x2f32(w[ob].z, b.z, a0[ob], 0, 0, 0);
#pragma unroll
                for (int ob = 0; ob < NB0; ob++) a0[ob] = __builtin_amdgcn_mfma_f32_32x32x2f32(w[ob].w, b.w, a0[ob], 0, 0, 0);
                if (more) cur = nxt;
            }
            if (more_st) stage_store<NB0>(Ws[(st + 1) & 1], wave, lane, wr);
            __syncthreads();
        }
    }
    bias_act<NB0>(a0, P.bias, P.relu, h);
    if (NB1 == 0) { chain_store<NB0>(C, a0, P.Nout, row, meta.valid, lane, h); return; }
    if (chain_out1_applies<NB1, NB2>(C)) { chain_out1<NB0>(C, a0, row, meta.valid, lane, h); return; }

    f32x16 a1[NB1 ? NB1 : 1];
    chain_layer<NB0, (NB1 ? NB1 : 1)>(a0, a1, C.wpack1, C.KB1, Ws, wave, lane);
    bias_act<(NB1 ? NB1 : 1)>(a1, C.bias1, C.relu1, h);
    if (NB2 == 0) { chain_store<(NB1 ? NB1 : 1)>(C, a1, C.N1, row, meta.valid, lane, h); return; }

    f32x16 a2[NB2 ? NB2 : 1];
    chain_layer<(NB1 ? NB1 : 1), (NB2 ? NB2 : 1)>(a1, a2, C.wpack2, C.KB2, Ws, wave, lane);
    bias_act<(NB2 ? NB2 : 1)>(a2, C.bias2, C.relu2, h);
    chain_store<(NB2 ? NB2 : 1)>(C, a2, C.N2, row, meta.valid, lane, h);
}

template <int NB> struct FStage { static constexpr int G = NB == 3 ? 4 : CH_STAGE_TILES / NB; static constexpr int TPW = (G * NB + CH_WAVES - 1) / CH_WAVES; };

template <int NB>
__device__ __forceinline__ void fstage_load(const float* __restrict__ wpack, int KB, int st, int wave, int lane, float4 (&r)[4]) {
    constexpr int G = FStage<NB>::G;
#pragma unroll
    for (int u = 0; u < FStage<NB>::TPW; u++) {
        const int tt = wave + CH_WAVES * u, kbl = tt / NB, ob = tt - kbl * NB;
        if (tt < G * NB) r[u] = ldw(wpack, KB, ob, st * G + kbl, lane);
    }
}
template <int NB>
__device__ __forceinline__ void fstage_store(float* ws, int wave, int lane, const float4 (&r)[4]) {
#pragma unroll
    for (int u = 0; u < FStage<NB>::TPW; u++) {
        const int tt = wave + CH_WAVES * u;
        if (tt < FStage<NB>::G * NB) *reinterpret_cast<float4*>(ws + (tt * 64 + lane) * 4) = r[u];
    }
}

template <int MODE> __device__ __forceinline__ void fast_fetch(const MlpParams& P, const RowMeta<MODE>& r, int k, Raw<MODE>& v);
template <> __device__ __forceinline__ void fast_fetch<MODE_PLAIN>(const MlpParams& P, const RowMeta<MODE_PLAIN>& r, int k, Raw<MODE_PLAIN>& v) {
    v.a = ld4(P.in + r.off + k);
}
template <> __device__ __forceinline__ void fast_fetch<MODE_GROUP>(const MlpParams& P, const RowMeta<MODE_GROUP>& r, int k, Raw<MODE_GROUP>& v) {
    v.a = ld4(P.feat + r.off + k);
}
template <> __device__ __forceinline__ void fast_fetch<MODE_INTERP>(const MlpParams& P, const RowMeta<MODE_INTERP>& r, int k, Raw<MODE_INTERP>& v) {
    v.a = ld4(P.known + r.o0 + k); v.b = ld4(P.known + r.o1 + k); v.c = ld4(P.known + r.o2 + k);
}
template <int MODE> __device__ __forceinline__ float4 fast_finish(const RowMeta<MODE>& r, int k, const Raw<MODE>& v, const float* s_wx, const float* s_b);
template <> __device__ __forceinline__ float4 fast_finish<MODE_PLAIN>(const RowMeta<MODE_PLAIN>&, int, const Raw<MODE_PLAIN>& v, const float*, const float*) {
    return v.a;
}
template <> __device__ __forceinline__ float4 fast_finish<MODE_GROUP>(const RowMeta<MODE_GROUP>& r, int k, const Raw<MODE_GROUP>& v, const float* s_wx, const float* s_b) {
    const float4 w0 = ld4(s_wx + k * 3), w1 = ld4(s_wx + k * 3 + 4), w2 = ld4(s_wx + k * 3 + 8), b = ld4(s_b + k);
    float4 o;
    o.x = fmaxf(v.a.x + (w0.x * r.dx + w0.y * r.dy + w0.z * r.dz) + b.x, 0.f);
// ... 1011 lines not shown
    }
    wpack[e] = val;
}

__global__ void maxpool_rows_kernel(const float* __restrict__ in, int ld_in, long rows_out, int ns, int C,
                                    float* __restrict__ out, int ld_out, int col_off) {
    long e = (long)blockIdx.x * blockDim.x + threadIdx.x;
    if (e >= rows_out * C) return;
    long r = e / C; int c = (int)(e - r * C);
    const float* p = in + r * ns * (long)ld_in + c;
    float m = p[0];
    for (int s = 1; s < ns; s++) m = fmaxf(m, p[(long)s * ld_in]);
    out[r * ld_out + col_off + c] = m;
}

#define ST_ROWS 32
#define ST_MAX_K0 256
#define ST_MAX_NB0 12
#define ST_RING 8
template <int NBW0>
__device__ __forceinline__ void mlp_stack2_body(const ChainParams& Cin, int blk, int nblk, int tiles_all, float* st_lds) {
    MlpParams P = Cin.a;
    P.rows = effective_rows(Cin.a);
    const int tiles_eff = (int)((P.rows + ST_ROWS - 1) / ST_ROWS);
    const int tiles_split = tiles_all >= 0 ? tiles_all : tiles_eff;
    const int ysplit = min(Cin.stack_split, max(1, (256 + tiles_split - 1) / max(tiles_split, 1)));
    for (long unit = blk; unit < (long)tiles_eff * ysplit; unit += nblk) {
    const int tile = (int)(unit / ysplit), ysl = (int)(unit - (long)tile * ysplit);
    const long row0 = (long)tile * ST_ROWS;
    const int lda = P.K + 4;
    const int n0pad = P.NB * 32, ldb = n0pad + 4;
    float* actA = st_lds;
    float* actB = st_lds + ST_ROWS * lda;
    const int tid = threadIdx.x;
    const int lane = tid & 63, wave = __builtin_amdgcn_readfirstlane(tid >> 6);
    const int h = lane >> 5, j = lane & 31;

    const int NB1 = (Cin.N1 + 31) / 32, NCG = (NB1 + 3) / 4;
    const int KBa = (PRCNN_ABL & 32) ? 1 : P.KB, KBb = (PRCNN_ABL & 64) ? 1 : Cin.KB1;
    int nbsA[4];
    const float* bpA[4];
    float4 bqA[ST_RING][4], bqB[ST_RING][4];
#pragma unroll
    for (int q = 0; q < 4; q++) {
        nbsA[q] = wave + 4 * q;
        bpA[q] = P.wpack + ((long)min(nbsA[q], P.NB - 1) * P.KB) * 256 + lane * 4;
    }
    const float* bpB[4];
    auto prime_b = [&](int cg) {
        bpB[0] = Cin.wpack1 + ((long)min(cg * 4 + wave, NB1 - 1) * Cin.KB1) * 256 + lane * 4;
#pragma unroll
        for (int g = 0; g < ST_RING; g++) bqB[g][0] = ld4(bpB[0] + (long)min(g, KBb - 1) * 256);
    };
#pragma unroll
    for (int g = 0; g < ST_RING; g++) {
#pragma unroll
        for (int q = 0; q < 4; q++)
            if (q < NBW0) bqA[g][q] = ld4(bpA[q] + (long)min(g, KBa - 1) * 256);
    }
    bpB[1] = bpB[2] = bpB[3] = Cin.wpack1;
    prime_b(ysl);

    {
        const int r = tid >> 3, c4 = tid & 7;
        long grow = row0 + r;
        if (grow >= P.rows) grow = P.rows - 1;
        RowMeta<MODE_GROUP> meta;
        make_meta<MODE_GROUP>(P, grow, meta);
        const float dx = meta.dx, dy = meta.dy, dz = meta.dz;
        float4 zr[ST_MAX_K0 / 32];
#pragma unroll
        for (int u = 0; u < ST_MAX_K0 / 32; u++) {
            const int k = c4 * 4 + 32 * u;
            zr[u] = (k < P.K && !(PRCNN_ABL & 16)) ? ld4(P.feat + meta.off + k) : make_float4(0.f, 0.f, 0.f, 0.f);
        }
#pragma unroll
        for (int u = 0; u < ST_MAX_K0 / 32; u++) {
            const int k = c4 * 4 + 32 * u;
            if (k >= P.K) break;
            const float4 z = zr[u];
            const float4 aw0 = ld4(P.act_wx + (long)k * 3), aw1 = ld4(P.act_wx + (long)k * 3 + 4), aw2 = ld4(P.act_wx + (long)k * 3 + 8);
            const float4 ab = ld4(P.act_bias + k);
            float4 v;
            v.x = fmaxf(z.x + (aw0.x * dx + aw0.y * dy + aw0.z * dz) + ab.x, 0.f);
            v.y = fmaxf(z.y + (aw0.w * dx + aw1.x * dy + aw1.y * dz) + ab.y, 0.f);
            v.z = fmaxf(z.z + (aw1.z * dx + aw1.w * dy + aw2.x * dz) + ab.z, 0.f);
            v.w = fmaxf(z.w + (aw2.y * dx + aw2.z * dy + aw2.w * dz) + ab.w, 0.f);
            *reinterpret_cast<float4*>(actA + r * lda + k) = v;
        }
    }

    auto run_layer = [&](auto& acc, float4 (&bq)[ST_RING][4], const float* const (&bptr)[4], int nbw, int KB, const float* act, int ld) {
        auto load_b = [&](int g, int slot) {
            const long off = (long)min(g, KB - 1) * 256;
#pragma unroll
            for (int q = 0; q < 4; q++)
                if (q < nbw) bq[slot][q] = ld4(bptr[q] + off);
        };
        const float* a_base = act + j * ld + 4 * h;
        float4 a_next = *reinterpret_cast<const float4*>(a_base);
        for (int kb0 = 0; kb0 < KB; kb0 += ST_RING) {
#pragma unroll
            for (int u = 0; u < ST_RING; u++) {
                const int kb = kb0 + u;
                if (kb < KB) {
                    const float4 a = a_next;
                    a_next = *reinterpret_cast<const float4*>(a_base + min(kb + 1, KB - 1) * 8);
#pragma unroll
                    for (int q = 0; q < 4; q++) if (q < nbw) acc[q] = __builtin_amdgcn_mfma_f32_32x32x2f32(a.x, bq[u][q].x, acc[q], 0, 0, 0);
#pragma unroll
                    for (int q = 0; q < 4; q++) if (q < nbw) acc[q] = __builtin_amdgcn_mfma_f32_32x32x2f32(a.y, bq[u][q].y, acc[q], 0, 0, 0);
#pragma unroll
                    for (int q = 0; q < 4; q++) if (q < nbw) acc[q] = __builtin_amdgcn_mfma_f32_32x32x2f32(a.z, bq[u][q].z, acc[q], 0, 0, 0);
#pragma unroll
                    for (int q = 0; q < 4; q++) if (q < nbw) acc[q] = __builtin_amdgcn_mfma_f32_32x32x2f32(a.w, bq[u][q].w, acc[q], 0, 0, 0);
                }
                if (!(PRCNN_ABL & 128)) load_b(kb + ST_RING, u);
            }
        }
    };

    __syncthreads();
    {
        f32x16 acc[4];
#pragma unroll
        for (int q = 0; q < 4; q++) acc[q] = (f32x16){0};
        run_layer(acc, bqA, bpA, NBW0, KBa, actA, lda);
#pragma unroll
        for (int q = 0; q < NBW0; q++) {
            const int nb = nbsA[q];
            if (nb >= P.NB) continue;
            const int n = nb * 32 + j;
            const float bias = (P.bias && n < P.Nout) ? P.bias[n] : 0.f;
#pragma unroll
            for (int r = 0; r < 16; r++) {
                const int rin = (r & 3) + 8 * (r >> 2) + 4 * h;
                float v = acc[q][r] + bias;
                if (P.relu) v = fmaxf(v, 0.f);
                actB[rin * ldb + n] = n < P.Nout ? v : 0.f;
            }
        }
    }
    __syncthreads();
    for (int cg = ysl; cg < NCG; cg += ysplit) {
        if (cg != ysl) prime_b(cg);
        f32x16 acc[4];
        acc[0] = (f32x16){0};
        run_layer(acc, bqB, bpB, 1, KBb, actB, ldb);
        const int nb = cg * 4 + wave;
        if (nb >= NB1) continue;
        const int n = nb * 32 + j;
        const bool n_ok = n < Cin.N1;
        const float bias = (Cin.bias1 && n_ok) ? Cin.bias1[n] : 0.f;
        if (row0 + 32 <= P.rows && nb * 32 + 32 <= Cin.N1) {
            float* o = P.out + (row0 + 4 * h) * P.ld_out + P.col_off + n;
            const long ld = P.ld_out;
#pragma unroll
            for (int r = 0; r < 16; r++) {
                float v = acc[0][r] + bias;
                v = Cin.relu1 ? fmaxf(v, 0.f) : v;
                o[((r & 3) + 8 * (r >> 2)) * ld] = v;
            }
        } else {
#pragma unroll
            for (int r = 0; r < 16; r++) {
                const int rin = (r & 3) + 8 * (r >> 2) + 4 * h;
                const long g = row0 + rin;
                float v = acc[0][r] + bias;
                if (Cin.relu1) v = fmaxf(v, 0.f);
                if (n_ok && g < P.rows) P.out[g * P.ld_out + P.col_off + n] = v;
            }
        }
    }
    __syncthreads();
    }
}
template <int NBW0>
__global__ __launch_bounds__(256, 1) void mlp_stack2_kernel(const ChainParams Cin) {
    extern __shared__ __attribute__((aligned(16))) float st_lds[];
    mlp_stack2_body<NBW0>(Cin, blockIdx.x, gridDim.x, -1, st_lds);
}

#define R32_MAX_K 1024
__global__ __launch_bounds__(256, 1) void mlp_rows32_kernel(const MlpParams Pin, int split_max) {
    MlpParams P = Pin;
    P.rows = effective_rows(Pin);
    const int tiles_eff = (int)((P.rows + ST_ROWS - 1) / ST_ROWS);
    const int ysplit = min(split_max, max(1, (256 + tiles_eff - 1) / max(tiles_eff, 1)));
    extern __shared__ __attribute__((aligned(16))) float st_lds[];
    const int lda = P.K + 4;
    const int tid = threadIdx.x;
    const int lane = tid & 63, wave = __builtin_amdgcn_readfirstlane(tid >> 6);
    const int h = lane >> 5, j = lane & 31;
    const int NCG = (P.NB + 3) / 4;
    for (long unit = blockIdx.x; unit < (long)tiles_eff * ysplit; unit += gridDim.x) {
        const int tile = (int)(unit / ysplit), ysl = (int)(unit - (long)tile * ysplit);
        const long row0 = (long)tile * ST_ROWS;
        const float* bp;
        float4 bq[ST_RING];
        auto prime = [&](int cg) {
            bp = P.wpack + ((long)min(cg * 4 + wave, P.NB - 1) * P.KB) * 256 + lane * 4;
#pragma unroll
            for (int g = 0; g < ST_RING; g++) bq[g] = ld4(bp + (long)min(g, P.KB - 1) * 256);
        };
        prime(ysl);
        {
            const int r = tid >> 3, c4 = tid & 7;
            long grow = row0 + r;
            if (grow >= P.rows) grow = P.rows - 1;
            const float* src = P.in + grow * (long)P.ld_in + c4 * 4;
            float* dst = st_lds + r * lda + c4 * 4;
            for (int k0 = 0; k0 < P.K; k0 += 512) {
                float4 v[16];
#pragma unroll
                for (int u = 0; u < 16; u++) v[u] = (k0 + 32 * u + c4 * 4 < P.K) ? ld4(src + k0 + 32 * u) : make_float4(0.f, 0.f, 0.f, 0.f);
#pragma unroll
                for (int u = 0; u < 16; u++)
                    if (k0 + 32 * u + c4 * 4 < P.K) *reinterpret_cast<float4*>(dst + k0 + 32 * u) = v[u];
            }
        }
        __syncthreads();
        const float* a_base = st_lds + j * lda + 4 * h;
        for (int cg = ysl; cg < NCG; cg += ysplit) {
            if (cg != ysl) prime(cg);
            f32x16 acc = (f32x16){0};
            float4 a_next = *reinterpret_cast<const float4*>(a_base);
            for (int kb0 = 0; kb0 < P.KB; kb0 += ST_RING) {
#pragma unroll
                for (int u = 0; u < ST_RING; u++) {
                    const int kb = kb0 + u;
                    if (kb < P.KB) {
                        const float4 a = a_next;
                        a_next = *reinterpret_cast<const float4*>(a_base + min(kb + 1, P.KB - 1) * 8);
                        acc = __builtin_amdgcn_mfma_f32_32x32x2f32(a.x, bq[u].x, acc, 0, 0, 0);
                        acc = __builtin_amdgcn_mfma_f32_32x32x2f32(a.y, bq[u].y, acc, 0, 0, 0);
                        acc = __builtin_amdgcn_mfma_f32_32x32x2f32(a.z, bq[u].z, acc, 0, 0, 0);
                        acc = __builtin_amdgcn_mfma_f32_32x32x2f32(a.w, bq[u].w, acc, 0, 0, 0);
                    }
                    bq[u] = ld4(bp + (long)min(kb + ST_RING, P.KB - 1) * 256);
                }
            }
            const int nb = cg * 4 + wave;
            if (nb >= P.NB) continue;
            const int n = nb * 32 + j;
            const bool n_ok = n < P.Nout;
            const float bias = (P.bias && n_ok) ? P.bias[n] : 0.f;
            if (row0 + 32 <= P.rows && nb * 32 + 32 <= P.Nout) {
                float* o = P.out + (row0 + 4 * h) * P.ld_out + P.col_off + n;
                const long ld = P.ld_out;
#pragma unroll
                for (int r = 0; r < 16; r++) {
                    float v = acc[r] + bias;
                    v = P.relu ? fmaxf(v, 0.f) : v;
                    o[((r & 3) + 8 * (r >> 2)) * ld] = v;
                }
            } else {
#pragma unroll
                for (int r = 0; r < 16; r++) {
                    const int rin = (r & 3) + 8 * (r >> 2) + 4 * h;
                    const long g = row0 + rin;
                    float v = acc[r] + bias;
                    if (P.relu) v = fmaxf(v, 0.f);
                    if (n_ok && g < P.rows) P.out[g * P.ld_out + P.col_off + n] = v;
                }
            }
        }
        __syncthreads();
    }
}

#include "mlp_host.h"

#include "mlp_multi.h"

#include "mlp_train.h"
```

pointrcnn_amd/csrc/mlp_multi.h:

```cpp
#pragma once
#include "level_units.h"

struct MultiParams {
    LevelUnits U;
    int variant[LEVEL_MAX_PROBLEMS];
    ChainParams c[LEVEL_MAX_PROBLEMS];
};
static_assert(sizeof(MultiParams) <= 4096, "the multi-problem kernels take their problems as kernel arguments");

#define FAST_MULTI_TABLE(X) X(3, 2)
#define STACK_MULTI_TABLE(X) X(2, 2) X(3, 2)

enum {
#define X(W0, W1, NBL, NSV) SA0V_##W0##_##NSV,
    SA0_TABLE(X)
#undef X
    SA0V_COUNT
};

__global__ __launch_bounds__(256) void sa0_multi_kernel(const MultiParams M) {
    int prob, local, count;
    level_units_find(M.U, blockIdx.x, prob, local, count);
    switch (M.variant[prob]) {
#define X(W0, W1, NBL, NSV) case SA0V_##W0##_##NSV: sa_xyz_chain_body<W0 / 8, W1 / 8, NBL, NSV>(M.c[prob], local, count); break;
        SA0_TABLE(X)
#undef X
    }
}

template <int NBA, int NBB>
__global__ __launch_bounds__(256) __attribute__((amdgpu_waves_per_eu(2, 8))) void chain_fast_multi_kernel(const MultiParams M) {
    FAST_CHAIN_LDS;
    int prob, local, count;
    level_units_find(M.U, blockIdx.x, prob, local, count);
    if (M.variant[prob] == 0) mlp_chain_fast_body<MODE_GROUP, NBA, 4, 0>(M.c[prob], local, Ws, s_wx, s_b, s_bias);
    else mlp_chain_fast_body<MODE_GROUP, NBB, 4, 0>(M.c[prob], local, Ws, s_wx, s_b, s_bias);
}

template <int NBWA, int NBWB>
__global__ __launch_bounds__(256, 1) void stack2_multi_kernel(const MultiParams M) {
    extern __shared__ __attribute__((aligned(16))) float st_lds[];
    int prob, local, count;
    level_units_find(M.U, blockIdx.x, prob, local, count);
    int tiles_all = 0;
    for (int p = 0; p < M.U.nprob; p++) tiles_all += (int)((effective_rows(M.c[p].a) + ST_ROWS - 1) / ST_ROWS);
    if (NBWA == NBWB || M.variant[prob] == 0) mlp_stack2_body<NBWA>(M.c[prob], local, count, tiles_all, st_lds);
    else mlp_stack2_body<NBWB>(M.c[prob], local, count, tiles_all, st_lds);
}

#define STACK_MULTI_GRID_CAP 2048L

PRCNN_API int prcnn_mlp_chain_group_multi(int nprob, const prcnn_chain_group_problem_t* prob, prcnn_stream_t stream) {
    PRCNN_REQUIRE(nprob >= 1 && nprob <= LEVEL_MAX_PROBLEMS && prob, "prcnn_mlp_chain_group_multi: nprob=%d (1..%d) or a null table", nprob,
                  LEVEL_MAX_PROBLEMS);
    MultiParams M = {};
    MlpLaunch L[LEVEL_MAX_PROBLEMS];
    int n = 0, family = K_NONE;
    for (int q = 0; q < nprob; q++) {
        const prcnn_chain_group_problem_t& a = prob[q];
        ChainParams& C = M.c[n];
        C = ChainParams{};
        int rc = fill_chain_group(C, a.xyz, a.new_xyz, a.idx, a.feat_cl, a.ld_feat, a.B, a.N, a.M, a.nsample, a.C, a.act_wx, a.act_bias, a.nlayers, a.wpack,
                                  a.bias, a.nout, a.relu, a.out, a.ld_out, a.col_off, a.pool_ns, a.groups_dev);
        if (rc) return rc;
        L[n] = MlpLaunch();
        rc = decide_chain(MODE_GROUP, C, L[n]);
        if (rc) return rc;
        if (L[n].family == K_NONE) continue;
        const bool known = L[n].family == K_SA0 || L[n].family == K_CHAIN_FAST || L[n].family == K_STACK2;
        if (!known || L[n].block.x != 256 || (family != K_NONE && L[n].family != family)) return PRCNN_EUNSUPPORTED;
        family = L[n].family;
        n++;
    }
    if (n == 0) return PRCNN_OK;
    hipStream_t s = (hipStream_t)stream;
    long want[LEVEL_MAX_PROBLEMS] = {0, 0, 0, 0};
    for (int p = 0; p < n; p++) want[p] = L[p].grid.x;
    if (family == K_SA0) {
        for (int p = 0; p < n; p++) {
            M.variant[p] = -1;
#define X(W0, W1, NBL, NSV) if (L[p].a == W0 / 8 && L[p].b == W1 / 8 && L[p].c == NBL && L[p].d == NSV) M.variant[p] = SA0V_##W0##_##NSV;
            SA0_TABLE(X)
#undef X
            if (M.variant[p] < 0) return PRCNN_EUNSUPPORTED;
        }
        const long grid = level_units_share(M.U, want, nullptr, n, 0);
        if (grid <= 0) return prcnn_fail(PRCNN_EINVAL, "prcnn_mlp_chain_group_multi: bad grid");
        hipLaunchKernelGGL(sa0_multi_kernel, dim3((unsigned)grid), dim3(256), 0, s, M);
        PRCNN_LAUNCH_CHECK("prcnn_mlp_chain_group_multi(sa0)");
        return PRCNN_OK;
    }
    int va = 0, vb = 1 << 30;
    for (int p = 0; p < n; p++) {
        if (family == K_CHAIN_FAST && (L[p].b != 4 || L[p].c != 0)) return PRCNN_EUNSUPPORTED;
        va = max(va, L[p].a);
        vb = min(vb, L[p].a);
    }
    for (int p = 0; p < n; p++) {
        if (L[p].a != va && L[p].a != vb) return PRCNN_EUNSUPPORTED;
        M.variant[p] = L[p].a == va ? 0 : 1;
    }
    if (family == K_CHAIN_FAST) {
        const long grid = level_units_share(M.U, want, nullptr, n, 0);
        if (grid <= 0) return prcnn_fail(PRCNN_EINVAL, "prcnn_mlp_chain_group_multi: bad grid");
#define X(A, B)                                                                                                          \
        if (va == A && vb == B) {                                                                                        \
            hipLaunchKernelGGL((chain_fast_multi_kernel<A, B>), dim3((unsigned)grid), dim3(256), 0, s, M);               \
            PRCNN_LAUNCH_CHECK("prcnn_mlp_chain_group_multi(fast)");                                                     \
            return PRCNN_OK;                                                                                             \
        }
        FAST_MULTI_TABLE(X)
#undef X
        return PRCNN_EUNSUPPORTED;
    }
    size_t lds = 0;
    for (int p = 0; p < n; p++) lds = max(lds, L[p].lds);
    const long grid = level_units_share(M.U, want, nullptr, n, STACK_MULTI_GRID_CAP);
    if (grid <= 0) return prcnn_fail(PRCNN_EINVAL, "prcnn_mlp_chain_group_multi: bad grid");
#define X(A, B)                                                                                                          \
    if (va == A && vb == B) {                                                                                            \
        static PrcnnLdsLimit attr;                                                                                       \
        if (!attr.raise((const void*)stack2_multi_kernel<A, B>, 96 * 1024))                                              \
            return prcnn_fail(PRCNN_EHIP, "prcnn_mlp_chain_group_multi(stack): cannot raise the dynamic LDS limit");     \
        hipLaunchKernelGGL((stack2_multi_kernel<A, B>), dim3((unsigned)grid), dim3(256), lds, s, M);                     \
        PRCNN_LAUNCH_CHECK("prcnn_mlp_chain_group_multi(stack)");                                                        \
        return PRCNN_OK;                                                                                                 \
    }
    STACK_MULTI_TABLE(X)
#undef X
    return PRCNN_EUNSUPPORTED;
}
```

pointrcnn_amd/dropin/pointnet2_lib/pointnet2/pointnet2_modules.py:

```python
import os

import torch
import torch.nn as nn
import torch.nn.functional as F

from pointrcnn_amd import ops, train_mlp
from . import pointnet2_utils
from . import pytorch_utils as pt_utils

_POOL_FUSED = (16, 32, 64)
HOIST_FIRST_LAYER = True
GROUP_DEDUP = os.environ.get("PRCNN_GROUP_DEDUP", "1") != "0"
DEDUP_SPARSE_DIV = int(os.environ.get("PRCNN_DEDUP_SPARSE_DIV", "4"))
STACK_ALL_FLAT = os.environ.get("PRCNN_STACK_ALL_FLAT", "1") != "0"
STACK_ALL_FLAT_MAX_ROWS = 1 << 20
LEVEL_MERGE = os.environ.get("PRCNN_LEVEL_MERGE", "1") != "0"
DENSE_CHUNK_BYTES = int(float(os.environ.get("PRCNN_DENSE_CHUNK_MB", "2048")) * 2 ** 20) or (1 << 62)
TRAIN_FUSED = os.environ.get("PRCNN_TRAIN_FUSED", "1") != "0"
TRAIN_DEDUP = os.environ.get("PRCNN_TRAIN_DEDUP", "1") != "0"


def _channels_last(features):
    if features is None:
        return None
    return pt_utils._rows_view(features.transpose(1, 2))


def _run_mlp_tail(x_rows, layers, start, out, pool_ns):
    n = len(layers)
    for li in range(start, n):
        last = li == n - 1
        x_rows = ops.mlp_rows(x_rows, layers[li], out=out if last else None, pool_ns=pool_ns if last else 0)
    return x_rows


def _flatten_frames(x):
    B, N, C = x.shape
    if C == 1 and x.stride(2) != 1:
        x = x.as_strided((B, N, 1), (x.stride(0), x.stride(1), 1), x.storage_offset())
    assert x.stride(2) == 1 and (B == 1 or x.stride(0) == N * x.stride(1)), "rows must have one uniform stride"
    return x.as_strided((1, B * N, C), (B * N * x.stride(1), x.stride(1), 1), x.storage_offset())


def _stack_scale(layers, act, src):
    return (any(l.nout > 128 for l in layers) and act is not None and src is not None and src.shape[-1] <= 256
            and src.shape[-1] % 8 == 0 and ops.chain_supported(1, layers, 0))


class _SliceCount:
    slice_count = True

    def __init__(self, counts):
        self.counts = counts


def _one_launch(src, layers, act, ns, pool):
    wide = any(l.nout > 128 for l in layers)
    return (ns == 1 or (pool and ns in (16, 32))) and (not wide or (ns == 1 and _stack_scale(layers, act, src))) \
        and ops.chain_supported(1, layers, ns if pool else 0)


def _run_scale(xyz, ctr, idx, src, layers, act, out, ns, pool, groups_dev):
    pool_ns = ns if pool else 0
    if _one_launch(src, layers, act, ns, pool):
        return ops.mlp_chain_group(xyz, ctr, idx, src, layers, out=out, pool_ns=pool_ns, act=act, groups_dev=groups_dev)
    if len(layers) == 1:
        return ops.mlp_group(xyz, ctr, idx, src, layers[0], out=out, pool_ns=pool_ns, act=act, groups_dev=groups_dev)
    n = len(layers)
    G = idx.shape[1] if idx.shape[0] == 1 else 0
    inter_bytes = idx.numel() * max(l.nout for l in layers[:-1]) * 4
    if groups_dev is not None and (pool or ns == 1) and out is not None and G > 1 and inter_bytes > DENSE_CHUNK_BYTES:
        nchunk = -(-inter_bytes // DENSE_CHUNK_BYTES)
        gc = -(-G // nchunk)
        dst, col = out
        for g0 in range(0, G, gc):
            g1 = min(G, g0 + gc)
            cnt = (groups_dev - g0).clamp_(0, g1 - g0)
            if ops._split_log is not None:
                ops._split_log.append(_SliceCount(cnt))
            x = ops.mlp_group(xyz, None if ctr is None else ctr[:, g0:g1], idx[:, g0:g1], src, layers[0], act=act, groups_dev=cnt)
            for li in range(1, n):
                last = li == n - 1
                x = ops.mlp_rows(x, layers[li], out=(dst[g0:g1], col) if last else None, pool_ns=pool_ns if last else 0, rows_dev=cnt, rows_unit=ns)
            del x
        return dst
    x = ops.mlp_group(xyz, ctr, idx, src, layers[0], act=act, groups_dev=groups_dev)
    for li in range(1, n):
        last = li == n - 1
        x = ops.mlp_rows(x, layers[li], out=out if last else None, pool_ns=pool_ns if last else 0, rows_dev=groups_dev, rows_unit=ns)
    return x


class _PointnetSAModuleBase(nn.Module):
    def __init__(self):
        super().__init__()
        self.npoint = None
        self.groupers = None
        self.mlps = None
        self.pool_method = "max_pool"

    def _fused_ok(self, xyz, features):
        if torch.is_grad_enabled() or not xyz.is_cuda or self.pool_method != "max_pool":
            return False
        if xyz.dtype != torch.float32 or (features is not None and features.dtype != torch.float32):
            return False
        for g, m in zip(self.groupers, self.mlps):
            if not getattr(g, "use_xyz", True) or not m.fusable():
                return False
        return True

    def forward(self, xyz, features=None, new_xyz=None):
        if self._fused_ok(xyz, features):
            return self._forward_fused(xyz, features, new_xyz)
        if self._train_ok(xyz, features):
            return self._forward_train(xyz, features, new_xyz)
        new_features_list = []
        xyz_flipped = xyz.transpose(1, 2).contiguous()
        if new_xyz is None:
            new_xyz = pointnet2_utils.gather_operation(
                xyz_flipped, pointnet2_utils.furthest_point_sample(xyz, self.npoint)
            ).transpose(1, 2).contiguous() if self.npoint is not None else None
        for i in range(len(self.groupers)):
            new_features = self.groupers[i](xyz, new_xyz, features)
            new_features = self.mlps[i](new_features)
            if self.pool_method == "max_pool":
                new_features = new_features.max(dim=3, keepdim=True)[0]
            elif self.pool_method == "avg_pool":
                new_features = F.avg_pool2d(new_features, kernel_size=[1, new_features.size(3)])
            else:
                raise NotImplementedError
            new_features_list.append(new_features.squeeze(-1))
        return new_xyz, torch.cat(new_features_list, dim=1)

    def _train_ok(self, xyz, features):
        if not TRAIN_FUSED or not train_mlp.usable(xyz, features) or self.pool_method != "max_pool":
            return False
        if self.npoint is None:
            g = self.groupers[0]
            return len(self.groupers) == 1 and isinstance(g, pointnet2_utils.GroupAll) and g.use_xyz and features is not None \
                and xyz.shape[1] <= 255 and train_mlp.stack_ok(self.mlps[0].layers())
        for g, m in zip(self.groupers, self.mlps):
            if not isinstance(g, pointnet2_utils.QueryAndGroup) or not g.use_xyz or g.nsample > 255 or not train_mlp.stack_ok(m.layers()):
                return False
        return True

    def _forward_train(self, xyz, features, new_xyz):
        xyz = xyz.contiguous()
        B = xyz.shape[0]
        if self.npoint is None:
            N = xyz.shape[1]
            idx = torch.arange(N, dtype=torch.int32, device=xyz.device).view(1, 1, N).expand(B, 1, N).contiguous()
            src = train_mlp.Source("group", xyz=xyz, new_xyz=torch.zeros((B, 1, 3), dtype=xyz.dtype, device=xyz.device), idx=idx)
            out = train_mlp.run_stack(self.mlps[0].layers(), src, _channels_last(features), None, pool_ns=N)
            return None, out.view(B, 1, -1).transpose(1, 2)
        with torch.no_grad():
            if new_xyz is None:
                new_xyz = ops.gather_rows(xyz, ops.furthest_point_sample(xyz, self.npoint))
            new_xyz = new_xyz.contiguous()
            if len(self.groupers) == 2:
                a, b = self.groupers
                idxs = list(ops.ball_query2(a.radius, a.nsample, b.radius, b.nsample, xyz, new_xyz))
            else:
                idxs = [ops.ball_query(g.radius, g.nsample, xyz, new_xyz) for g in self.groupers]
        feat_cl = _channels_last(features)
        M = new_xyz.shape[1]
        outs = []
        for g, mlp, idx in zip(self.groupers, self.mlps, idxs):
            if TRAIN_DEDUP:
                with torch.no_grad():
                    rows = train_mlp.GroupRows(idx, new_xyz, xyz.shape[1])
                src = train_mlp.Source("group", xyz=xyz.view(1, -1, 3), rows=rows)
            else:
                src = train_mlp.Source("group", xyz=xyz, new_xyz=new_xyz, idx=idx)
            outs.append(train_mlp.run_stack(mlp.layers(), src, feat_cl, None, pool_ns=g.nsample).view(B, M, -1))
        out_cl = outs[0] if len(outs) == 1 else torch.cat(outs, dim=2)
        return new_xyz, out_cl.transpose(1, 2)

    def _forward_fused(self, xyz, features, new_xyz):
        valid_n = getattr(xyz, "_prcnn_valid_n", None)
        xyz = xyz.contiguous()
        B, N, _ = xyz.shape
        feat_cl = _channels_last(features)
        if new_xyz is None and self.npoint is not None:
            new_xyz = ops.gather_rows(xyz, ops.furthest_point_sample(xyz, self.npoint))
        M = new_xyz.shape[1] if new_xyz is not None else 1
        c_outs = [m.layers()[-1]._parts()[0].out_channels for m in self.mlps]
        out_cl = torch.empty((B, M, sum(c_outs)), dtype=torch.float32, device=xyz.device)

        idxs = [None] * len(self.groupers)
        qg = [i for i, g in enumerate(self.groupers) if isinstance(g, pointnet2_utils.QueryAndGroup)]
        if len(qg) == 2 and new_xyz is not None:
            a, b = self.groupers[qg[0]], self.groupers[qg[1]]
            idxs[qg[0]], idxs[qg[1]] = ops.ball_query2(a.radius, a.nsample, b.radius, b.nsample, xyz, new_xyz)
        for i, g in enumerate(self.groupers):
            if idxs[i] is not None:
                continue
            if isinstance(g, pointnet2_utils.QueryAndGroup):
                idxs[i] = ops.ball_query(g.radius, g.nsample, xyz, new_xyz)
            else:
                idxs[i] = torch.arange(N, dtype=torch.int32, device=xyz.device).view(1, 1, N).expand(B, 1, N).contiguous()

        hoist = None
        if feat_cl is not None and HOIST_FIRST_LAYER:
            parts = [mlp.layers()[0].hoisted_group() if len(mlp.layers()) >= 2 else None for mlp in self.mlps]
            if all(p is not None for p in parts):
                key = tuple(id(p[0]) for p in parts)
                if getattr(self, "_prcnn_zlin", (None, None))[0] != key:
                    self._prcnn_zlin = (key, ops.PackedLinear(torch.cat([p[0] for p in parts], 0).contiguous(), None, relu=False))
                z_all = ops.mlp_rows(feat_cl, self._prcnn_zlin[1], seg=None if valid_n is None else (valid_n, N)).view(B, N, -1)
                hoist, zoff = [], 0
                for p in parts:
                    hoist.append((z_all[..., zoff:zoff + p[0].shape[0]], (p[1], p[2])))
                    zoff += p[0].shape[0]

        if LEVEL_MERGE and GROUP_DEDUP and valid_n is None and len(self.groupers) == 2 and len(qg) == 2 and new_xyz is not None \
                and self._forward_merged(xyz, new_xyz, idxs, hoist, feat_cl, out_cl, c_outs):
            return new_xyz, out_cl.transpose(1, 2)

        col = 0
        for i, (g, mlp) in enumerate(zip(self.groupers, self.mlps)):
            group_all = not isinstance(g, pointnet2_utils.QueryAndGroup)
            ns = idxs[i].shape[2]
            mods = mlp.layers()
            fused_pool = ns in _POOL_FUSED
            dst = (out_cl.view(B * M, -1), col)
            ctr = None if group_all else new_xyz
            if hoist is not None:
                src, act = hoist[i]
                layers = [m.packed() for m in mods[1:]]
            else:
                src, act = feat_cl, None
                layers = [mods[0].packed(k_rot=3 if feat_cl is not None else 0)] + [m.packed() for m in mods[1:]]
            if valid_n is not None and not (GROUP_DEDUP and not group_all and fused_pool):
                raise RuntimeError("a cloud tagged with _prcnn_valid_n needs the padding-free grouping path on every scale")
            if GROUP_DEDUP and not group_all and fused_pool:
                all_flat = STACK_ALL_FLAT and B * M * ns <= STACK_ALL_FLAT_MAX_ROWS and _stack_scale(layers, act, src)
                sp = ops.GroupSplit(idxs[i], new_xyz, N, ns if all_flat else max(1, ns // DEDUP_SPARSE_DIV), valid_n=valid_n)
                xyz_f = xyz.view(1, B * N, 3)
                src_f = None if src is None else _flatten_frames(src)
                t1 = torch.empty((sp.max_rows, c_outs[i]), dtype=torch.float32, device=xyz.device)
                _run_scale(xyz_f, sp.rnx, sp.ridx, src_f, layers, act, (t1, 0), 1, False, sp.rows)
                ops.segmax_scatter(t1, sp, dst[0], col)
                del t1
                if not all_flat:
                    tn = torch.empty((sp.G, c_outs[i]), dtype=torch.float32, device=xyz.device)
                    _run_scale(xyz_f, sp.nxn, sp.idxn, src_f, layers, act, (tn, 0), ns, True, sp.count_dense)
                    ops.scatter_rows(tn, sp.listn, sp.count_dense, dst[0], col)
            else:
                x = _run_scale(xyz, ctr, idxs[i], src, layers, act, dst if fused_pool else None, ns, fused_pool, None)
                if not fused_pool:
                    ops.maxpool_rows(x, ns, out=dst)
            col += c_outs[i]
        return new_xyz, out_cl.transpose(1, 2)

    def _forward_merged(self, xyz, new_xyz, idxs, hoist, feat_cl, out_cl, c_outs):
        B, N, _ = xyz.shape
        M = new_xyz.shape[1]
        scales = []
        for i, mlp in enumerate(self.mlps):
            ns = idxs[i].shape[2]
            mods = mlp.layers()
            if hoist is not None:
                src, act = hoist[i]
                layers = [m.packed() for m in mods[1:]]
            else:
                src, act = feat_cl, None
                layers = [mods[0].packed(k_rot=3 if feat_cl is not None else 0)] + [m.packed() for m in mods[1:]]
            all_flat = STACK_ALL_FLAT and B * M * ns <= STACK_ALL_FLAT_MAX_ROWS and _stack_scale(layers, act, src)
            if ns not in _POOL_FUSED or not _one_launch(src, layers, act, 1, False) or not (all_flat or _one_launch(src, layers, act, ns, True)):
                return False
            scales.append((ns, src, act, layers, all_flat))
        (ns_a, _, _, _, flat_a), (ns_b, _, _, _, flat_b) = scales
        sps = ops.GroupSplit.pair(idxs[0], ns_a if flat_a else max(1, ns_a // DEDUP_SPARSE_DIV),
                                  idxs[1], ns_b if flat_b else max(1, ns_b // DEDUP_SPARSE_DIV), new_xyz, N)
        xyz_f = xyz.view(1, B * N, 3)
        dst = out_cl.view(B * M, -1)
        flat, dense, pools, col = [], [], [], 0
        order = sorted(range(2), key=lambda i: -sum(l.nout for l in scales[i][3]) * scales[i][0])
        cols = [0, c_outs[0]]
        for i in order:
            (ns, src, act, layers, all_flat), sp, col = scales[i], sps[i], cols[i]
            src_f = None if src is None else _flatten_frames(src)
            t1 = torch.empty((sp.max_rows, c_outs[i]), dtype=torch.float32, device=xyz.device)
            flat.append(dict(xyz=xyz_f, new_xyz=sp.rnx, idx=sp.ridx, feat_cl=src_f, layers=layers, out=(t1, 0), pool_ns=0, act=act, groups_dev=sp.rows))
            pools.append((t1, sp, col, "flat"))
            if not all_flat:
                tn = torch.empty((sp.G, c_outs[i]), dtype=torch.float32, device=xyz.device)
                dense.append(dict(xyz=xyz_f, new_xyz=sp.nxn, idx=sp.idxn, feat_cl=src_f, layers=layers, out=(tn, 0), pool_ns=ns, act=act,
                                  groups_dev=sp.count_dense))
                pools.append((tn, sp, col, "dense"))
        if not ops.mlp_chain_group_multi(flat + dense):
            for pr in flat + dense:
                ops.mlp_chain_group(**pr)
        ops.level_pool(pools, dst)
        return True


class PointnetSAModuleMSG(_PointnetSAModuleBase):

    def __init__(self, *, npoint, radii, nsamples, mlps, bn=True, use_xyz=True, pool_method="max_pool",
                 instance_norm=False):
        super().__init__()
        assert len(radii) == len(nsamples) == len(mlps)
        self.npoint = npoint
        self.groupers = nn.ModuleList()
        self.mlps = nn.ModuleList()
        for i in range(len(radii)):
            self.groupers.append(pointnet2_utils.QueryAndGroup(radii[i], nsamples[i], use_xyz=use_xyz)
                                 if npoint is not None else pointnet2_utils.GroupAll(use_xyz))
            mlp_spec = list(mlps[i])
            if use_xyz:
                mlp_spec[0] += 3
            self.mlps.append(pt_utils.SharedMLP(mlp_spec, bn=bn, instance_norm=instance_norm))
        self.pool_method = pool_method


class PointnetSAModule(PointnetSAModuleMSG):

    def __init__(self, *, mlp, npoint=None, radius=None, nsample=None, bn=True, use_xyz=True,
                 pool_method="max_pool", instance_norm=False):
        super().__init__(mlps=[mlp], npoint=npoint, radii=[radius], nsamples=[nsample], bn=bn, use_xyz=use_xyz,
                         pool_method=pool_method, instance_norm=instance_norm)


class PointnetFPModule(nn.Module):

    def __init__(self, *, mlp, bn=True):
        super().__init__()
        self.mlp = pt_utils.SharedMLP(mlp, bn=bn)

    def forward(self, unknown, known, unknow_feats, known_feats):
        if (not torch.is_grad_enabled()) and known is not None and unknown.is_cuda and self.mlp.fusable() \
                and known_feats.dtype == torch.float32:
            return self._forward_fused(unknown, known, unknow_feats, known_feats)
        if TRAIN_FUSED and known is not None and train_mlp.usable(unknown, known_feats, unknow_feats) \
                and train_mlp.stack_ok(self.mlp.layers()):
            unknown, known = unknown.contiguous(), known.contiguous()
            B, n, _ = unknown.shape
            with torch.no_grad():
                _, idx3, w3 = ops.three_nn(unknown, known, want_weight=True)
            src = train_mlp.Source("interp", idx3=idx3, w3=w3)
            x = train_mlp.run_stack(self.mlp.layers(), src, _channels_last(known_feats), _channels_last(unknow_feats))
            return x.view(B, n, -1).transpose(1, 2)
        if known is not None:
            dist, idx = pointnet2_utils.three_nn(unknown, known)
            dist_recip = 1.0 / (dist + 1e-8)
            norm = torch.sum(dist_recip, dim=2, keepdim=True)
            weight = dist_recip / norm
            interpolated_feats = pointnet2_utils.three_interpolate(known_feats, idx, weight)
        else:
            interpolated_feats = known_feats.expand(*known_feats.size()[0:2], unknown.size(1))
        if unknow_feats is not None:
            new_features = torch.cat([interpolated_feats, unknow_feats], dim=1)
        else:
            new_features = interpolated_feats
        new_features = self.mlp(new_features.unsqueeze(-1))
        return new_features.squeeze(-1)

    def _forward_fused(self, unknown, known, unknow_feats, known_feats):
        unknown, known = unknown.contiguous(), known.contiguous()
        B, n, _ = unknown.shape
        _, idx3, w3 = ops.three_nn(unknown, known, want_weight=True)
        known_cl = _channels_last(known_feats)
        skip_cl = _channels_last(unknow_feats)
        mods = self.mlp.layers()
        parts = mods[0].hoisted_interp(known_cl.shape[-1]) if HOIST_FIRST_LAYER else None
        if parts is not None and (skip_cl is not None or len(mods) >= 2):
            lin_a, lin_b, bias0 = parts
            y = ops.mlp_rows(known_cl, lin_a).view(B, known_cl.shape[1], -1)
            rest = [m.packed() for m in mods[1:]]
            if skip_cl is not None:
                x = ops.mlp_rows_addinterp(skip_cl, lin_b, y, idx3, w3)
                x = _run_mlp_tail(x, rest, 0, None, 0) if rest else x
            elif ops.chain_supported(2, rest, 0):
                x = ops.mlp_chain_interp(y, idx3, w3, None, rest, act_bias=bias0)
            else:
                x = ops.mlp_interp(y, idx3, w3, None, rest[0], act_bias=bias0)
                x = _run_mlp_tail(x, rest, 1, None, 0)
            return x.view(B, n, -1).transpose(1, 2)
        layers = [m.packed() for m in mods]
        if ops.chain_supported(2, layers, 0):
            x = ops.mlp_chain_interp(known_cl, idx3, w3, skip_cl, layers)
        else:
            x = ops.mlp_interp(known_cl, idx3, w3, skip_cl, layers[0])
            x = _run_mlp_tail(x, layers, 1, None, 0)
        return x.view(B, n, -1).transpose(1, 2)
```

pointrcnn_amd/ops.py:

```python
import ctypes
import math
import os
import threading
import weakref

import torch

from . import _cabi

_INT = torch.int32
_F32 = torch.float32
FPS_PRUNED = os.environ.get("PRCNN_FPS_PRUNED", "1") == "1"
FPS_NESTED = os.environ.get("PRCNN_FPS_NESTED", "1") == "1"


def _stream():
    return torch.cuda.current_stream().cuda_stream


def _chk(t, name, dtype=_F32, ndim=None):
    if not isinstance(t, torch.Tensor):
        raise TypeError("%s must be a torch.Tensor" % name)
    if not t.is_cuda:
        raise RuntimeError("%s must be a CUDA(HIP) tensor: the HIP kernels are the only implementation" % name)
# ... 211 lines not shown
    out = torch.empty((B, C, n), dtype=_F32, device=features.device)
    _cabi.check(_cabi.lib().prcnn_three_interp(_p(features), _p(idx), _p(weight), B, C, m, n, _p(out), _stream()),
                "prcnn_three_interp")
    return out


def three_interpolate_grad(grad_out, idx, weight, m):
    _chk(grad_out, "grad_out", ndim=3); _chk(idx, "idx", _INT, 3); _chk(weight, "weight", ndim=3)
    B, C, n = grad_out.shape
    g = torch.zeros((B, C, m), dtype=_F32, device=grad_out.device)
    ws = torch.empty((B, m, C), dtype=_F32, device=grad_out.device)
    _cabi.check(_cabi.lib().prcnn_three_interp_grad(_p(grad_out), _p(idx), _p(weight), B, C, n, m, _p(g), _p(ws), _stream()),
                "prcnn_three_interp_grad")
    return g


class PackedLinear:

    def __init__(self, weight, bias=None, relu=True, k_rot=0):
        _chk(weight, "weight", ndim=2)
        self.nout, self.k = weight.shape
        self.relu = bool(relu)
        L = _cabi.lib()
        self.wpack = torch.empty((L.prcnn_wpack_floats(self.nout, self.k),), dtype=_F32, device=weight.device)
        _cabi.check(L.prcnn_pack_weight(_p(weight), self.nout, self.k, k_rot, _p(self.wpack), _stream()),
                    "prcnn_pack_weight")
        self._w = weight if k_rot == 0 else None
        self._wsplit = None
        self.bias = None
        if bias is not None:
            _chk(bias.contiguous(), "bias", ndim=1)
            self.bias = torch.zeros(((self.nout + 31) // 32 * 32,), dtype=_F32, device=weight.device)
            self.bias[: self.nout] = bias


    def wsplit(self, chain=0):
        if self._wsplit is None:
            self._wsplit = {}
        if chain not in self._wsplit and self._w is not None and self.k % 32 == 0:
            L = _cabi.lib()
            img = torch.empty((L.prcnn_wsplit_bytes(self.nout, self.k),), dtype=torch.uint8, device=self._w.device)
            _cabi.check(L.prcnn_pack_weight_split(_p(self._w.contiguous()), self.nout, self.k, int(chain), _p(img), _stream()),
                        "prcnn_pack_weight_split")
            self._wsplit[chain] = img
        return self._wsplit.get(chain)


MLP_SPLIT_TERMS = int(os.environ.get("PRCNN_MLP_SPLIT", "6") or 0)
if MLP_SPLIT_TERMS not in (0, 3, 6):
    raise RuntimeError("PRCNN_MLP_SPLIT=%r: 6 (default) / 3 split-bf16 terms, 0 = fp32 MFMA" % os.environ.get("PRCNN_MLP_SPLIT"))

_MODE_ROWS, _MODE_GROUP, _MODE_INTERP = 0, 1, 2
_chain_ok = {}


def chain_supported(mode, layers, pool_ns=0):
    key = (mode, tuple(l.nout for l in layers), pool_ns)
    hit = _chain_ok.get(key)
    if hit is None:
        arr = (ctypes.c_int * len(layers))(*[l.nout for l in layers])
        hit = bool(_cabi.lib().prcnn_mlp_chain_supported(mode, len(layers), arr, pool_ns)) if 1 <= len(layers) <= 3 else False
        _chain_ok[key] = hit
    return hit


class _ChainArgs:

    def __init__(self, layers):
        n = len(layers)
        self.n = n
        self.layers = tuple(layers)
        self.wpack = (ctypes.c_void_p * n)(*[l.wpack.data_ptr() for l in layers])
        self.bias = (ctypes.c_void_p * n)(*[(l.bias.data_ptr() if l.bias is not None else None) for l in layers])
        self.nout = (ctypes.c_int * n)(*[l.nout for l in layers])
        self.relu = (ctypes.c_int * n)(*[int(l.relu) for l in layers])


def _chain_args(layers):
    key = tuple(id(l) for l in layers)
    hit = getattr(layers[0], "_chain_cache", None)
    if hit is None or hit[0] != key:
        hit = (key, _ChainArgs(layers))
        layers[0]._chain_cache = hit
    return hit[1]


def _row_stride(x):
    for size, stride in zip(reversed(x.shape[:-1]), reversed(x.stride()[:-1])):
        if size != 1:
            return stride
    return x.shape[-1]


def _out_buf(out, rows, nout, device):
    if out is None:
        return torch.empty((rows, nout), dtype=_F32, device=device), nout, 0
    buf, col_off = out
    return buf, _row_stride(buf), col_off


def _rows_prelude(name, x, last, out, pool_ns):
    if x.stride(-1) != 1:
        raise RuntimeError("%s: last dim must be contiguous" % name)
    K = x.shape[-1]
    rows = x.numel() // K
    return (K, rows, _row_stride(x)) + _out_buf(out, rows // pool_ns if pool_ns else rows, last.nout, x.device)


def _group_prelude(xyz, idx, feat_cl, last, out, pool_ns, act):
    B, N, _ = xyz.shape
    _, M, ns = idx.shape
    C = 0 if feat_cl is None else feat_cl.shape[-1]
    ld_feat = 0 if feat_cl is None else _row_stride(feat_cl)
    rows = B * M * ns
    return (B, N, M, ns, C, ld_feat) + ((None, None) if act is None else tuple(act)) + _out_buf(out, rows // pool_ns if pool_ns else rows, last.nout, xyz.device)


def _interp_prelude(known_cl, idx3, skip_cl, last, out):
    B, m, C2 = known_cl.shape
    n = idx3.shape[1]
    C1 = 0 if skip_cl is None else skip_cl.shape[-1]
    ld_skip = 0 if skip_cl is None else _row_stride(skip_cl)
    return (B, n, m, C2, C1, ld_skip) + _out_buf(out, B * n, last.nout, known_cl.device)


def mlp_chain_rows(x, layers, out=None, pool_ns=0, seg=None):
    K, rows, ld_in, buf, ld_out, col_off = _rows_prelude("mlp_chain_rows", x, layers[-1], out, pool_ns)
    a = _chain_args(layers)
    seg_cnt, seg_rows = (None, 0) if seg is None else (seg[0], int(seg[1]))
    if (MLP_SPLIT_TERMS and not pool_ns and seg is None and a.n == 2 and K == 128 and layers[0].nout == 128
            and (layers[1].nout == 1 or 64 < layers[1].nout <= 128) and layers[0].wsplit(1) is not None and layers[1].wsplit(1) is not None):
        if getattr(a, "wchain", None) is None:
            a.wchain = (ctypes.c_void_p * 2)(layers[0].wsplit(1).data_ptr(), layers[1].wsplit(1).data_ptr())
        rc = _cabi.lib().prcnn_mlp_chain_rows_split(_p(x), ld_in, rows, K, a.wchain, a.wpack, a.bias, a.nout, a.relu,
                                                    MLP_SPLIT_TERMS, _p(buf), ld_out, col_off, _stream())
        if rc != _cabi.EUNSUPPORTED:
            _cabi.check(rc, "prcnn_mlp_chain_rows_split")
            return buf
    _cabi.check(_cabi.lib().prcnn_mlp_chain_rows(_p(x), ld_in, rows, K, a.n, a.wpack, a.bias, a.nout, a.relu, _p(buf),
                                                 ld_out, col_off, pool_ns, _p(seg_cnt), seg_rows, _stream()), "prcnn_mlp_chain_rows")
    return buf


def mlp_chain_group(xyz, new_xyz, idx, feat_cl, layers, out=None, pool_ns=0, act=None, groups_dev=None):
    B, N, M, ns, C, ld_feat, awx, ab, buf, ld_out, col_off = _group_prelude(xyz, idx, feat_cl, layers[-1], out, pool_ns, act)
    a = _chain_args(layers)
    _cabi.check(_cabi.lib().prcnn_mlp_chain_group(_p(xyz), _p(new_xyz), _p(idx), _p(feat_cl), ld_feat, B, N, M, ns, C, _p(awx), _p(ab), a.n,
                                                  a.wpack, a.bias, a.nout, a.relu, _p(buf), ld_out, col_off, pool_ns,
                                                  _p(groups_dev), _stream()), "prcnn_mlp_chain_group")
    return buf


def mlp_chain_group_multi(problems):
    arr = (_cabi.ChainGroupProblem * len(problems))()
    for q, pr in zip(arr, problems):
        layers = pr["layers"]
        B, N, M, ns, C, ld_feat, awx, ab, buf, ld_out, col_off = _group_prelude(pr["xyz"], pr["idx"], pr.get("feat_cl"), layers[-1], pr["out"],
                                                                                pr.get("pool_ns", 0), pr.get("act"))
        a = _chain_args(layers)
        q.xyz, q.new_xyz, q.idx, q.feat_cl, q.act_wx, q.act_bias = (_p(pr["xyz"]), _p(pr.get("new_xyz")), _p(pr["idx"]), _p(pr.get("feat_cl")),
                                                                    _p(awx), _p(ab))
        q.wpack, q.bias = ctypes.cast(a.wpack, ctypes.c_void_p), ctypes.cast(a.bias, ctypes.c_void_p)
        q.nout, q.relu = ctypes.cast(a.nout, ctypes.c_void_p), ctypes.cast(a.relu, ctypes.c_void_p)
        q.out, q.groups_dev = _p(buf), _p(pr.get("groups_dev"))
        q.ld_feat, q.B, q.N, q.M, q.nsample, q.C, q.nlayers = ld_feat, B, N, M, ns, C, a.n
        q.ld_out, q.col_off, q.pool_ns = ld_out, col_off, pr.get("pool_ns", 0)
    rc = _cabi.lib().prcnn_mlp_chain_group_multi(len(problems), arr, _stream())
    if rc == _cabi.EUNSUPPORTED:
        return False
    _cabi.check(rc, "prcnn_mlp_chain_group_multi")
    return True


def mlp_chain_interp(known_cl, idx3, w3, skip_cl, layers, out=None, act_bias=None):
    B, n, m, C2, C1, ld_skip, buf, ld_out, col_off = _interp_prelude(known_cl, idx3, skip_cl, layers[-1], out)
    a = _chain_args(layers)
    if (MLP_SPLIT_TERMS and skip_cl is None and act_bias is not None and a.n == 1 and C2 == 128 and layers[0].nout == 128
            and layers[0].wsplit(1) is not None):
        l0 = layers[0]
        rc = _cabi.lib().prcnn_mlp_chain_interp_split(_p(known_cl), _row_stride(known_cl), _p(idx3), _p(w3), B, n, m, C2, _p(act_bias),
                                                      _p(l0.wsplit(1)), _p(l0.wpack), _p(l0.bias), l0.nout, int(l0.relu), MLP_SPLIT_TERMS, _p(buf),
                                                      ld_out, col_off, _stream())
        if rc != _cabi.EUNSUPPORTED:
            _cabi.check(rc, "prcnn_mlp_chain_interp_split")
            return buf
    _cabi.check(_cabi.lib().prcnn_mlp_chain_interp(_p(known_cl), _row_stride(known_cl), _p(idx3), _p(w3), _p(skip_cl), ld_skip,
                                                   B, n, m, C2, C1, _p(act_bias), a.n, a.wpack, a.bias, a.nout, a.relu, _p(buf),
                                                   ld_out, col_off, _stream()), "prcnn_mlp_chain_interp")
    return buf


def mlp_rows(x, lin, out=None, pool_ns=0, rows_dev=None, rows_unit=1, seg=None):
    K, rows, ld_in, buf, ld_out, col_off = _rows_prelude("mlp_rows", x, lin, out, pool_ns)
    if MLP_SPLIT_TERMS and ld_in % 4 == 0 and (seg is None or (rows_dev is None and not pool_ns)) and lin.wsplit() is not None:
        _cabi.check(_cabi.lib().prcnn_mlp_rows_split(_p(x), ld_in, rows, K, _p(lin.wpack), _p(lin.wsplit()), MLP_SPLIT_TERMS,
                                                     _p(lin.bias), lin.nout, int(lin.relu), _p(buf), ld_out, col_off, int(pool_ns), _p(rows_dev),
                                                     int(rows_unit), _p(None if seg is None else seg[0]), 0 if seg is None else int(seg[1]),
                                                     _stream()), "prcnn_mlp_rows_split")
        return buf
    _cabi.check(_cabi.lib().prcnn_mlp_rows(_p(x), ld_in, rows, K, _p(lin.wpack), _p(lin.bias), lin.nout, int(lin.relu),
                                           _p(buf), ld_out, col_off, pool_ns, _p(rows_dev), int(rows_unit),
                                           _p(None if seg is None else seg[0]), 0 if seg is None else int(seg[1]), _stream()), "prcnn_mlp_rows")
    return buf


def mlp_group(xyz, new_xyz, idx, feat_cl, lin, out=None, pool_ns=0, act=None, groups_dev=None):
    B, N, M, ns, C, ld_feat, awx, ab, buf, ld_out, col_off = _group_prelude(xyz, idx, feat_cl, lin, out, pool_ns, act)
    if MLP_SPLIT_TERMS and act is not None and C % 32 == 0 and ld_feat % 4 == 0 and lin.wsplit() is not None:
        _cabi.check(_cabi.lib().prcnn_mlp_group_split(_p(xyz), _p(new_xyz), _p(idx), _p(feat_cl), ld_feat, B, N, M, ns, C, _p(awx), _p(ab),
                                                      _p(lin.wpack), _p(lin.wsplit()), MLP_SPLIT_TERMS, _p(lin.bias), lin.nout, int(lin.relu),
                                                      _p(buf), ld_out, col_off, pool_ns, _p(groups_dev), _stream()), "prcnn_mlp_group_split")
        return buf
    _cabi.check(_cabi.lib().prcnn_mlp_group(_p(xyz), _p(new_xyz), _p(idx), _p(feat_cl), ld_feat, B, N, M, ns, C, _p(awx), _p(ab),
                                            _p(lin.wpack), _p(lin.bias), lin.nout, int(lin.relu), _p(buf), ld_out,
                                            col_off, pool_ns, _p(groups_dev), _stream()), "prcnn_mlp_group")
    return buf


def mlp_interp(known_cl, idx3, w3, skip_cl, lin, out=None, act_bias=None):
    B, n, m, C2, C1, ld_skip, buf, ld_out, col_off = _interp_prelude(known_cl, idx3, skip_cl, lin, out)
    _cabi.check(_cabi.lib().prcnn_mlp_interp(_p(known_cl), _row_stride(known_cl), _p(idx3), _p(w3), _p(skip_cl), ld_skip,
                                             B, n, m, C2, C1, _p(act_bias), _p(lin.wpack), _p(lin.bias), lin.nout,
                                             int(lin.relu), _p(buf), ld_out, col_off, _stream()), "prcnn_mlp_interp")
    return buf


def mlp_rows_addinterp(skip_cl, lin_b, y_cl, idx3, w3, out=None):
    B, n, C1 = skip_cl.shape
    m = y_cl.shape[1]
    buf, ld_out, col_off = _out_buf(out, B * n, lin_b.nout, skip_cl.device)
    if MLP_SPLIT_TERMS and _row_stride(skip_cl) % 4 == 0 and lin_b.wsplit() is not None:
        _cabi.check(_cabi.lib().prcnn_mlp_rows_addinterp_split(_p(skip_cl), _row_stride(skip_cl), C1, _p(lin_b.wpack), _p(lin_b.wsplit()),
                                                               MLP_SPLIT_TERMS, _p(lin_b.bias), lin_b.nout, int(lin_b.relu), _p(y_cl),
                                                               _row_stride(y_cl), _p(idx3), _p(w3), B, n, m, _p(buf), ld_out, col_off,
                                                               _stream()), "prcnn_mlp_rows_addinterp_split")
        return buf
    _cabi.check(_cabi.lib().prcnn_mlp_rows_addinterp(_p(skip_cl), _row_stride(skip_cl), C1, _p(lin_b.wpack), _p(lin_b.bias),
                                                     lin_b.nout, int(lin_b.relu), _p(y_cl), _row_stride(y_cl), _p(idx3),
                                                     _p(w3), B, n, m, _p(buf), ld_out, col_off, _stream()),
                "prcnn_mlp_rows_addinterp")
    return buf


def maxpool_rows(x, ns, out=None):
    rows, C = x.shape
    rows_out = rows // ns
    buf, ld_out, col_off = _out_buf(out, rows_out, C, x.device)
    _cabi.check(_cabi.lib().prcnn_maxpool_rows(_p(x), x.stride(0), rows_out, ns, C, _p(buf), ld_out, col_off, _stream()),
                "prcnn_maxpool_rows")
    return buf


ROIPOOL_BINS = os.environ.get("PRCNN_ROIPOOL_BINS", "1") != "0"
ROIPOOL_BINS_MIN_BOXES = 8


def _roipool_work(B, N, M, dev):
    if not ROIPOOL_BINS or M < ROIPOOL_BINS_MIN_BOXES:
        return None, 0
    nbytes = _cabi.lib().prcnn_roipool3d_work_bytes(B, N)
    if nbytes == 0:
        return None, 0
    return torch.empty((nbytes,), dtype=torch.uint8, device=dev), nbytes


def roipool3d(xyz, boxes3d_enlarged, pts_feature, sampled_pt_num):
    _chk(xyz, "xyz", ndim=3); _chk(boxes3d_enlarged, "boxes3d", ndim=3); _chk(pts_feature, "pts_feature", ndim=3)
    B, N, _ = xyz.shape
    M, C = boxes3d_enlarged.shape[1], pts_feature.shape[2]
    pooled = torch.empty((B, M, sampled_pt_num, 3 + C), dtype=_F32, device=xyz.device)
    empty = torch.empty((B, M), dtype=_INT, device=xyz.device)
    work, nbytes = _roipool_work(B, N, M, xyz.device)
    _cabi.check(_cabi.lib().prcnn_roipool3d_ws(_p(xyz), _p(boxes3d_enlarged), _p(pts_feature), B, N, M, C, sampled_pt_num,
                                               _p(pooled), _p(empty), _p(work), nbytes, _stream()), "prcnn_roipool3d")
    return pooled, empty


def roipool3d_canonical(xyz, pool_boxes3d, rois, extras, feat_cl, sampled_pt_num, out_feat=None, want_distinct=False):
    _chk(xyz, "xyz", ndim=3); _chk(pool_boxes3d, "pool_boxes3d", ndim=3)
    B, N, _ = xyz.shape
    if not (isinstance(feat_cl, torch.Tensor) and feat_cl.is_cuda and feat_cl.dtype == _F32 and feat_cl.dim() == 3
            and feat_cl.stride(-1) == 1 and feat_cl.stride(0) == N * feat_cl.stride(1)):
        raise RuntimeError("roipool3d_canonical: feat must be a (B,N,C) fp32 device tensor of uniformly strided rows")
    M, C, S = pool_boxes3d.shape[1], feat_cl.shape[2], int(sampled_pt_num)
    ex = [e.contiguous() for e in extras]
    if len(ex) > 2:
        raise ValueError("roipool3d_canonical: at most 2 scalar channels")
    for e in ex:
        _chk(e, "extra", ndim=2)
    P = 3 + len(ex)
    dev = xyz.device
    pts = torch.empty((B * M, S, P), dtype=_F32, device=dev)
    if out_feat is None:
        fbuf, col = torch.empty((B * M * S, C), dtype=_F32, device=dev), 0
    else:
        fbuf, col = out_feat
        if fbuf.dim() != 2 or fbuf.shape[0] != B * M * S or fbuf.stride(1) != 1 or col + C > fbuf.shape[1]:
            raise ValueError("roipool3d_canonical: out_feat buffer must be (B*M*S, >= col + C) rows")
    empty = torch.empty((B, M), dtype=_INT, device=dev)
    distinct = torch.empty((B, M), dtype=_INT, device=dev) if want_distinct else None
    if rois is not None:
        _chk(rois, "rois", ndim=3)
    work, nbytes = _roipool_work(B, N, M, dev)
    _cabi.check(_cabi.lib().prcnn_roipool3d_canonical_ws(
        _p(xyz), _p(pool_boxes3d), _p(rois), _p(ex[0]) if ex else None, _p(ex[1]) if len(ex) > 1 else None, _p(feat_cl),
        _row_stride(feat_cl), B, N, M, C, S, _p(pts), P, fbuf.data_ptr() + 4 * col, fbuf.stride(0), _p(empty), _p(distinct),
        _p(work), nbytes, _stream()), "prcnn_roipool3d_canonical")
    return (pts, fbuf, empty, distinct) if want_distinct else (pts, fbuf, empty)


def rpn_labels(pts, gt_boxes3d, num_gt=None, extra_width=0.2):
    _chk(pts, "pts", ndim=3); _chk(gt_boxes3d, "gt_boxes3d", ndim=3)
    B, N, _ = pts.shape
    G = gt_boxes3d.shape[1]
    if gt_boxes3d.shape[0] != B or gt_boxes3d.shape[2] != 7:
        raise ValueError("rpn_labels: gt_boxes3d must be (%d, G, 7)" % B)
    if num_gt is not None:
        _chk(num_gt, "num_gt", _INT, 1)
    cls = torch.empty((B, N), dtype=_INT, device=pts.device)
    reg = torch.empty((B, N, 7), dtype=_F32, device=pts.device)
    _cabi.check(_cabi.lib().prcnn_rpn_labels(_p(pts), _p(gt_boxes3d), _p(num_gt), B, N, G, float(extra_width), _p(cls), _p(reg),
                                             _stream()), "prcnn_rpn_labels")
    return cls, reg
# ... 455 lines not shown
_NMS_STAGE = threading.local()


def nms_sorted_to_host(boxes_sorted, thresh, rotated, keep_cpu):
    _chk(boxes_sorted, "boxes", ndim=2)
    N = boxes_sorted.shape[0]
    if N == 0:
        return 0
    dev = boxes_sorted.device
    stages = getattr(_NMS_STAGE, "buf", None)
    if stages is None:
        stages = _NMS_STAGE.buf = {}
    stage = stages.get(dev.index)
    if stage is None or stage.numel() < N + 1:
        stage = stages[dev.index] = torch.empty((max(2 * N, 8192) + 1,), dtype=torch.int64).pin_memory()
    L = _cabi.lib()
    wsb = L.prcnn_nms_workspace_bytes(N)
    ws = torch.empty((max(wsb, 8),), dtype=torch.uint8, device=dev)
    out = torch.empty((N + 1,), dtype=torch.int64, device=dev)
    stream = torch.cuda.current_stream(dev)
    _cabi.check(L.prcnn_nms(_p(boxes_sorted), N, float(thresh), 0 if rotated else 1, 0, _p(out), _p(out) + 8 * N,
                            _p(ws), wsb, stream.cuda_stream), "prcnn_nms")
    stage[:N + 1].copy_(out, non_blocking=True)
    stream.synchronize()
    n = int(stage[N:N + 1].view(torch.int32)[0])
    if n:
        keep_cpu[:n].copy_(stage[:n])
    return n


def decode_bbox_target(roi, pred_reg, loc_scope, loc_bin_size, num_head_bin, anchor_size, get_xz_fine=True,
                       get_y_by_bin=False, loc_y_scope=0.5, loc_y_bin_size=0.25, get_ry_fine=False, y_to_bottom=False):
    _chk(roi, "roi", ndim=2)
    _chk(pred_reg, "pred_reg", ndim=2)
    if roi.shape[0] != pred_reg.shape[0]:
        raise ValueError("decode_bbox_target: %d rois vs %d regression rows" % (roi.shape[0], pred_reg.shape[0]))
    N, C = pred_reg.shape
    out = torch.empty((N, 7), dtype=torch.float32, device=pred_reg.device)
    anchor = (ctypes.c_float * 3)(*[float(a) for a in anchor_size])
    _cabi.check(_cabi.lib().prcnn_decode_bbox_target(
        _p(roi), roi.shape[1], _p(pred_reg), N, C, float(loc_scope), float(loc_bin_size), int(num_head_bin),
        ctypes.cast(anchor, ctypes.c_void_p), int(bool(get_xz_fine)), int(bool(get_y_by_bin)), float(loc_y_scope),
        float(loc_y_bin_size), int(bool(get_ry_fine)), int(bool(y_to_bottom)), _p(out), _stream()), "prcnn_decode_bbox_target")
    return out


def proposal_layer(scores, boxes3d, pre, post, nms_thresh, rotated=False, ranges=(0.0, 40.0, 80.0)):
    _chk(scores, "scores", ndim=2)
    _chk(boxes3d, "boxes3d", ndim=3)
    B, N = scores.shape
    if tuple(boxes3d.shape) != (B, N, 7):
        raise ValueError("proposal_layer: boxes3d must be (%d, %d, 7), got %s" % (B, N, tuple(boxes3d.shape)))
    L = _cabi.lib()
    tot = int(post[0]) + int(post[1])
    dev = scores.device
    rois = torch.empty((B, tot, 7), dtype=torch.float32, device=dev)
    roi_scores = torch.empty((B, tot), dtype=torch.float32, device=dev)
    count = torch.empty((B,), dtype=_INT, device=dev)
    wsb = L.prcnn_proposal_workspace_bytes(B, N, max(pre), max(post))
    ws = torch.empty((max(wsb, 8),), dtype=torch.uint8, device=dev)
    r = ranges if ranges is not None else (0.0, 0.0, 0.0)
    _cabi.check(L.prcnn_proposal_layer(_p(scores), _p(boxes3d), B, N, int(ranges is not None), float(r[0]), float(r[1]),
                                       float(r[2]), int(pre[0]), int(pre[1]), int(post[0]), int(post[1]), float(nms_thresh),
                                       0 if rotated else 1, _p(rois), _p(roi_scores), _p(count), _p(ws), wsb, _stream()),
                "prcnn_proposal_layer")
    return rois, roi_scores, count


def nms_batched(boxes3d, scores, valid=None, thresh=0.1, rotated=True, max_keep=0):
    _chk(boxes3d, "boxes3d", ndim=3)
    _chk(scores, "scores", ndim=2)
    B, M = scores.shape
    if tuple(boxes3d.shape) != (B, M, 7):
        raise ValueError("nms_batched: boxes3d must be (%d, %d, 7), got %s" % (B, M, tuple(boxes3d.shape)))
    if valid is not None:
        if tuple(valid.shape) != (B, M) or not valid.is_cuda:
            raise ValueError("nms_batched: valid must be a (%d, %d) device tensor" % (B, M))
        valid = valid.to(torch.uint8).contiguous()
    mk = M if max_keep <= 0 or max_keep > M else int(max_keep)
    L = _cabi.lib()
    dev = scores.device
    keep = torch.empty((B, max(mk, 1)), dtype=_INT, device=dev)
    num = torch.empty((B,), dtype=_INT, device=dev)
    wsb = L.prcnn_nms_batched_workspace_bytes(B, M)
    ws = torch.empty((max(wsb, 8),), dtype=torch.uint8, device=dev)
    _cabi.check(L.prcnn_nms_batched(_p(boxes3d), _p(scores), _p(valid) if valid is not None else None, B, M, float(thresh),
                                    0 if rotated else 1, mk, _p(keep), _p(num), _p(ws), wsb, _stream()), "prcnn_nms_batched")
    return keep[:, :mk], num


def rotate_iou_eval(boxes, query_boxes, criterion=-1):
    _chk(boxes, "boxes", ndim=2); _chk(query_boxes, "query_boxes", ndim=2)
    N, K = boxes.shape[0], query_boxes.shape[0]
    out = torch.zeros((N, K), dtype=_F32, device=boxes.device)
    _cabi.check(_cabi.lib().prcnn_rotate_iou_eval(_p(boxes), N, _p(query_boxes), K, int(criterion), _p(out), _stream()),
                "prcnn_rotate_iou_eval")
    return out


def kitti_overlaps(metric, dt, dt_off, gt, gt_off, ov_off, total):
    F = dt_off.shape[0] - 1
    out = torch.zeros((max(int(total), 1),), dtype=torch.float64, device=dt_off.device)
    _cabi.check(_cabi.lib().prcnn_kitti_overlaps(int(metric), _p(dt), _p(dt_off), _p(gt), _p(gt_off), _p(ov_off), F, _p(out), _stream()),
                "prcnn_kitti_overlaps")
    return out[:int(total)]


def kitti_statistics(overlaps, ov_off, gt_datas, gt_off, dt_datas, dt_off, ign_gt, ign_det, dc, dc_off, metric, min_overlap,
                     thresholds, compute_fp, compute_aos):
    F, T = gt_off.shape[0] - 1, thresholds.shape[0]
    dev = gt_off.device
    res = torch.zeros((F, T, 4), dtype=torch.float64, device=dev)
    G = gt_datas.shape[0]
    matched = torch.full((max(G, 1),), float("nan"), dtype=torch.float64, device=dev)
    max_det = int((dt_off[1:] - dt_off[:-1]).max().item()) if F > 0 else 0
    _cabi.check(_cabi.lib().prcnn_kitti_statistics(_p(overlaps), _p(ov_off), _p(gt_datas), _p(gt_off), _p(dt_datas), _p(dt_off),
                                                   _p(ign_gt), _p(ign_det), _p(dc), _p(dc_off), F, max_det, int(metric),
                                                   float(min_overlap), _p(thresholds), T, int(compute_fp), int(compute_aos), _p(res),
                                                   _p(matched), _stream()), "prcnn_kitti_statistics")
    return res, matched[:G]


_split_log = None


class GroupSplit:

    def __init__(self, idx, new_xyz, N, sparse_max, valid_n=None, counts=None):
        _chk(idx, "idx", _INT, 3)
        _chk(new_xyz, "new_xyz", ndim=3)
        B, M, ns = idx.shape
        G, dev = B * M, idx.device
        T = max(1, min(int(sparse_max), ns))
        self.G, self.ns, self.T, self.max_rows = G, ns, T, G * T
        e = lambda shape, dt=_INT: torch.empty(shape, dtype=dt, device=dev)
        self.ridx, self.rnx = e((1, G * T, 1)), e((1, G * T, 3), _F32)
        self.slist, self.soff, self.scnt = e((G,)), e((G,)), e((G,))
        self.idxn, self.nxn, self.listn = e((1, G, ns)), e((1, G, 3), _F32), e((G,))
        self.counts = e((3,)) if counts is None else counts
        if valid_n is not None and (valid_n.dtype != _INT or valid_n.numel() != B or not valid_n.is_contiguous()):
            raise RuntimeError("valid_n must be a contiguous (B,) int32 tensor")
        if counts is None:
            _cabi.check(_cabi.lib().prcnn_group_compact(_p(idx), _p(new_xyz), B, N, M, ns, T, _p(valid_n), _p(self.ridx), _p(self.rnx), _p(self.slist),
                                                        _p(self.soff), _p(self.scnt), _p(self.idxn), _p(self.nxn), _p(self.listn),
                                                        _p(self.counts), _stream()), "prcnn_group_compact")
        self.rows, self.count_dense, self.count_sparse = self.counts[0:1], self.counts[1:2], self.counts[2:3]
        if _split_log is not None:
            _split_log.append(self)

    def _lists(self):
        return (ctypes.c_void_p * 8)(*[_p(t) for t in (self.ridx, self.rnx, self.slist, self.soff, self.scnt, self.idxn, self.nxn, self.listn)])

    @staticmethod
    def pair(idx_a, sparse_max_a, idx_b, sparse_max_b, new_xyz, N):
        if idx_a.shape[:2] != idx_b.shape[:2]:
            raise RuntimeError("GroupSplit.pair: the two index tensors must share (B, M)")
        counts = torch.empty((6,), dtype=_INT, device=idx_a.device)
        a = GroupSplit(idx_a, new_xyz, N, sparse_max_a, counts=counts[0:3])
        b = GroupSplit(idx_b, new_xyz, N, sparse_max_b, counts=counts[3:6])
        B, M, _ = idx_a.shape
        _cabi.check(_cabi.lib().prcnn_group_compact_pair(_p(idx_a), a.ns, a.T, _p(idx_b), b.ns, b.T, _p(new_xyz), B, N, M, a._lists(), b._lists(),
                                                         _p(counts), _stream()), "prcnn_group_compact_pair")
        return a, b


def segmax_scatter(src, sp, dst, col_off):
    C = src.shape[-1]
    _cabi.check(_cabi.lib().prcnn_segmax_scatter(_p(src), src.stride(-2), _p(sp.slist), _p(sp.soff), _p(sp.scnt), _p(sp.count_sparse),
                                                 sp.G, C, _p(dst), dst.stride(-2), int(col_off), _stream()), "prcnn_segmax_scatter")


def scatter_rows(src, rows_list, count, dst, col_off):
    C = src.shape[-1]
    _cabi.check(_cabi.lib().prcnn_scatter_rows(_p(src), src.stride(-2), _p(rows_list), _p(count), rows_list.shape[0], C, _p(dst),
                                               dst.stride(-2), int(col_off), _stream()), "prcnn_scatter_rows")


def level_pool(problems, dst):
    n = len(problems)
    P, I = ctypes.c_void_p * n, ctypes.c_int * n
    src, ld, lst, off, cnt, count, cap, C, col = P(), I(), P(), P(), P(), P(), I(), I(), I()
    for q, (s, sp, c0, kind) in enumerate(problems):
        flat = kind == "flat"
        src[q], ld[q], C[q], col[q], cap[q] = _p(s), s.stride(-2), s.shape[-1], int(c0), sp.G
        lst[q], count[q] = (_p(sp.slist), _p(sp.count_sparse)) if flat else (_p(sp.listn), _p(sp.count_dense))
        off[q], cnt[q] = (_p(sp.soff), _p(sp.scnt)) if flat else (None, None)
    _cabi.check(_cabi.lib().prcnn_level_pool(n, src, ld, lst, off, cnt, count, cap, C, col, _p(dst), dst.stride(-2), _stream()), "prcnn_level_pool")


def _frames(raw, offsets, calib, *img_hw):
    _chk(raw, "raw", ndim=2)
    _chk(calib, "calib", ndim=2)
    for hw in img_hw:
        _chk(hw, "img_hw", _INT, 2)
    if offsets.dtype != torch.int64 or not offsets.is_contiguous() or offsets.device != raw.device:
        raise RuntimeError("offsets must be a contiguous int64 tensor on the device of raw")
    B = offsets.shape[0] - 1
    if raw.shape[1] != 4 or calib.shape[1] != 24 or any(hw.shape[1] != 2 for hw in img_hw):
        raise RuntimeError("expected raw (total,4), calib (B,24), img_hw (B,2)")
    if calib.shape[0] != B or any(hw.shape[0] != B for hw in img_hw):
        raise RuntimeError("calib / img_hw must have one row per frame")
    return B, raw.shape[0], raw.device


def _scope(scope):
    return None if scope is None else (ctypes.c_double * 6)(*[float(v) for v in scope])


def _sample_outputs(B, npoints, dev):
    return (torch.empty((B, npoints, 3), dtype=_F32, device=dev), torch.empty((B, npoints), dtype=_INT, device=dev),
            torch.empty((B,), dtype=_INT, device=dev), torch.empty((B,), dtype=_INT, device=dev))


def scene_prepare(raw, offsets, max_points_per_frame, calib, img_hw, scope, npoints, seed):
    B, total, dev = _frames(raw, offsets, calib, img_hw)
    L = _cabi.lib()
    ws = torch.empty((int(L.prcnn_scene_workspace_bytes(total, B)),), dtype=torch.uint8, device=dev)
    xyz, src, nvalid, status = _sample_outputs(B, npoints, dev)
    inten = torch.empty((B, npoints), dtype=_F32, device=dev)
    _cabi.check(L.prcnn_scene_prepare(_p(raw), _p(offsets), B, total, int(max_points_per_frame), _p(calib), _p(img_hw), _scope(scope),
                                      int(npoints), int(seed) & 0xFFFFFFFF, _p(xyz), _p(inten), _p(src), _p(nvalid), _p(status), _p(ws),
                                      ws.numel(), _stream()), "prcnn_scene_prepare")
    return xyz, inten, src, nvalid, status


AUG_METHODS = ("rotation", "scaling", "flip")


def train_scene_prepare(raw, offsets, max_points_per_frame, calib, img_hw, scope, npoints, seed, gt_boxes3d, gt_alpha, num_gt=None,
                        accepted=None, db=None, aug_methods=AUG_METHODS, aug_prob=(1.0, 1.0, 0.5), aug_rot_range=18,
                        use_intensity=False, workspace=None):
    B, total, dev = _frames(raw, offsets, calib, img_hw)
    _chk(gt_boxes3d, "gt_boxes3d", ndim=3); _chk(gt_alpha, "gt_alpha", ndim=2)
    G = gt_boxes3d.shape[1]
    if tuple(gt_boxes3d.shape) != (B, G, 7) or tuple(gt_alpha.shape) != (B, G):
        raise ValueError("train_scene_prepare: gt_boxes3d must be (%d, G, 7), gt_alpha (%d, G)" % (B, B))
    if num_gt is not None:
        _chk(num_gt, "num_gt", _INT, 1)
        if num_gt.shape[0] != B:
            raise ValueError("train_scene_prepare: num_gt must be (%d,)" % B)
    unknown = [m for m in aug_methods if m not in AUG_METHODS]
    if unknown:
        raise ValueError("train_scene_prepare: unknown augmentation %r" % unknown)
    K, D, db_max = 0, 0, 0
    acc = [None] * 6
    dbt = [None] * 3
    if accepted is not None:
        if db is None:
            raise ValueError("train_scene_prepare: accepted objects need the database they came from")
        K, D, db_max = accepted["db_id"].shape[1], int(db.size), int(db.max_points)
        acc = [_chk(accepted["count"], "count", _INT, 1), _chk(accepted["db_id"], "db_id", _INT, 2),
               _chk(accepted["boxes3d"], "boxes3d", ndim=3), _chk(accepted["alpha"], "alpha", ndim=2),
               _chk(accepted["y_shift"], "y_shift", torch.float64, 2), _chk(accepted["status"], "status", _INT, 1)]
        if acc[0].shape[0] != B or tuple(acc[2].shape) != (B, K, 7) or tuple(acc[3].shape) != (B, K) or tuple(acc[4].shape) != (B, K):
            raise ValueError("train_scene_prepare: the accepted objects must describe %d frames" % B)
        dbt = [_chk(db.points, "db.points", ndim=2), _chk(db.intensity, "db.intensity", ndim=1), db.offsets]
        if dbt[2].dtype != torch.int64 or dbt[2].shape[0] != D + 1 or dbt[1].shape[0] != dbt[0].shape[0]:
            raise ValueError("train_scene_prepare: db.offsets must be (D+1,) int64, db.intensity one value per point")
    L = _cabi.lib()
    need = int(L.prcnn_train_scene_workspace_bytes(total, B, K, db_max))
    ws = torch.empty((need,), dtype=torch.uint8, device=dev) if workspace is None else workspace
    xyz, src, nvalid, status = _sample_outputs(B, npoints, dev)
    pin = torch.empty((B, npoints, 4), dtype=_F32, device=dev) if use_intensity else None
    feat = torch.empty((B, npoints), dtype=_F32, device=dev)
    out_gt = torch.empty((B, G + K, 7), dtype=_F32, device=dev)
    out_ng = torch.empty((B,), dtype=_INT, device=dev)
    aug = torch.empty((B, 8), dtype=torch.float64, device=dev)
    hi = math.pi / aug_rot_range
    cfg = (ctypes.c_double * 10)(*([1.0 if m in aug_methods else 0.0 for m in AUG_METHODS] + [float(p) for p in aug_prob] +
                                   [-hi, hi, 0.95, 1.05]))
    _cabi.check(L.prcnn_train_scene_prepare(
        _p(raw), _p(offsets), B, total, int(max_points_per_frame), _p(calib), _p(img_hw), _scope(scope), int(npoints),
        int(seed) & 0xFFFFFFFF, _p(gt_boxes3d), _p(gt_alpha), _p(num_gt), G, _p(acc[0]), _p(acc[1]), _p(acc[2]), _p(acc[3]), _p(acc[4]), _p(acc[5]), K,
        _p(dbt[0]), _p(dbt[1]), _p(dbt[2]), D, db_max, cfg, _p(xyz), _p(pin), _p(feat), _p(src), _p(nvalid), _p(status), _p(out_gt),
        _p(out_ng), _p(aug), _p(ws), ws.numel(), _stream()), "prcnn_train_scene_prepare")
    return {"pts_rect": xyz, "pts_input": pin if use_intensity else xyz, "pts_features": feat.unsqueeze(-1), "gt_boxes3d": out_gt,
            "num_gt": out_ng, "src": src, "nvalid": nvalid, "status": status, "aug": aug}


def gt_database_build(raw, offsets, max_points_per_frame, calib, boxes3d, num_boxes):
    B, total, dev = _frames(raw, offsets, calib)
    _chk(boxes3d, "boxes3d", ndim=3)
    _chk(num_boxes, "num_boxes", _INT, 1)
    G = boxes3d.shape[1]
    if tuple(boxes3d.shape) != (B, G, 7) or num_boxes.shape[0] != B:
        raise ValueError("gt_database_build: boxes3d must be (%d, G, 7), num_boxes (%d,)" % (B, B))
    L = _cabi.lib()
    mp = int(max_points_per_frame)
    ws = torch.empty((int(L.prcnn_gt_database_workspace_bytes(mp, B, G)),), dtype=torch.uint8, device=dev)
    npts = torch.empty((B, G), dtype=_INT, device=dev)
    _cabi.check(L.prcnn_gt_database_count(_p(raw), _p(offsets), B, total, mp, _p(calib), _p(boxes3d), _p(num_boxes), G, _p(npts), _p(ws),
                                          ws.numel(), _stream()), "prcnn_gt_database_count")
    off = torch.zeros((B * G + 1,), dtype=torch.int64, device=dev)
    off[1:] = torch.cumsum(npts.reshape(-1), 0, dtype=torch.int64)
    P = int(off[-1])
    points = torch.empty((P, 3), dtype=_F32, device=dev)
    inten = torch.empty((P,), dtype=_F32, device=dev)
    src = torch.empty((P,), dtype=_INT, device=dev)
    _cabi.check(L.prcnn_gt_database_fill(_p(raw), _p(offsets), B, total, mp, _p(calib), _p(boxes3d), _p(num_boxes), G, _p(off), P, _p(points),
                                         _p(inten), _p(src), _p(ws), ws.numel(), _stream()), "prcnn_gt_database_fill")
    return npts, off, points, inten, src


AUG_SCENE_MAX_ACCEPT = 15


def aug_scene_sample(gt_boxes3d, num_gt, planes, frame_ids, db_boxes, db_npts, area_scope, seed=0, max_accept=AUG_SCENE_MAX_ACCEPT):
    _chk(gt_boxes3d, "gt_boxes3d", ndim=3); _chk(planes, "planes", torch.float64, 2); _chk(frame_ids, "frame_ids", _INT, 1)
    _chk(db_boxes, "db_boxes", ndim=2); _chk(db_npts, "db_npts", _INT, 1)
    B, G, C = gt_boxes3d.shape
    D, K = db_boxes.shape[0], int(max_accept)
    if C != 7 or tuple(planes.shape) != (B, 4) or frame_ids.shape[0] != B:
        raise ValueError("aug_scene_sample: gt_boxes3d must be (B, G, 7), planes (B, 4), frame_ids (B,)")
    if db_boxes.shape[1] != 7 or db_npts.shape[0] != D:
        raise ValueError("aug_scene_sample: db_boxes (D, 7) and db_npts (D,) disagree")
    if num_gt is not None:
        _chk(num_gt, "num_gt", _INT, 1)
        if num_gt.shape[0] != B:
            raise ValueError("aug_scene_sample: num_gt must be (%d,)" % B)
    dev = gt_boxes3d.device
    for name, t in (("num_gt", num_gt), ("planes", planes), ("frame_ids", frame_ids), ("db_boxes", db_boxes), ("db_npts", db_npts)):
        if t is not None and t.device != dev:
            raise RuntimeError("aug_scene_sample: %s is on %s, gt_boxes3d on %s" % (name, t.device, dev))
    if area_scope is None or len(area_scope) != 6:
        raise ValueError("aug_scene_sample: area_scope must be 6 floats [x0 x1 y0 y1 z0 z1]")
    out = {"count": torch.empty((B,), dtype=_INT, device=dev), "db_id": torch.empty((B, max(K, 0)), dtype=_INT, device=dev),
           "boxes3d": torch.empty((B, max(K, 0), 7), dtype=_F32, device=dev),
           "y_shift": torch.empty((B, max(K, 0)), dtype=torch.float64, device=dev),
           "stats": torch.empty((B, 3), dtype=_INT, device=dev), "status": torch.empty((B,), dtype=_INT, device=dev)}
    _cabi.check(_cabi.lib().prcnn_aug_scene_sample(
        _p(gt_boxes3d), _p(num_gt), _p(planes), _p(frame_ids), B, G, _p(db_boxes), _p(db_npts), D, ctypes.cast(_scope(area_scope), ctypes.c_void_p),
        K, int(seed) & 0xFFFFFFFF, _p(out["count"]), _p(out["db_id"]), _p(out["boxes3d"]), _p(out["y_shift"]), _p(out["stats"]),
        _p(out["status"]), _stream()), "prcnn_aug_scene_sample")
    return out


def aug_scene_build(raw, offsets, max_points_per_frame, calib, img_hw, scope, accepted, db_points, db_intensity, db_offsets, guard_rows=0):
    B, total, dev = _frames(raw, offsets, calib, img_hw)
    cnt, ids, boxes = _chk(accepted["count"], "count", _INT, 1), _chk(accepted["db_id"], "db_id", _INT, 2), _chk(accepted["boxes3d"], "boxes3d", ndim=3)
    shift, status = _chk(accepted["y_shift"], "y_shift", torch.float64, 2), _chk(accepted["status"], "status", _INT, 1)
# ... 252 lines not shown
```

Before: 15200 frames/s.

## Store grouped MLP outputs directly to pooled destination, pool only multi-row groups

The group compaction now also emits a per-row destination index: a group with a single deduplicated row maps to its output slot, and all others get -1. The stacked MLP kernels use this index to write single-row and dense-pooled results straight into the concatenated level output, instead of staging them in temporaries. A new residual pool kernel then max-reduces only the groups with two or more rows. This removes the dense temporary buffers and most of the level_pool gather traffic, at the cost of scattered, non-vectorised stores in the first-layer epilogue. The stack2 launch bounds are also relaxed to allow two blocks per CU for narrow variants.

After: 15550 frames/s (median of 6 runs). 2.3% higher.

```diff
diff --git a/include/prcnn_pointops.h b/include/prcnn_pointops.h
--- a/include/prcnn_pointops.h
+++ b/include/prcnn_pointops.h
@@ -130,6 +130,8 @@
     int ld_feat, B, N, M, nsample, C, nlayers, ld_out, col_off, pool_ns;
 } prcnn_chain_group_problem_t;
 int prcnn_mlp_chain_group_multi(int nprob, const prcnn_chain_group_problem_t* prob, prcnn_stream_t stream);
+int prcnn_mlp_chain_group_multi_dst(int nprob, const prcnn_chain_group_problem_t* prob, const int32_t* const* dst, float* out2, int ld_out2,
+                                    const int* col_off2, prcnn_stream_t stream);
 
 int prcnn_maxpool_rows(const float* in, int ld_in, int64_t rows_out, int ns, int C, float* out, int ld_out,
                        int col_off, prcnn_stream_t stream);
@@ -222,6 +224,12 @@
 int prcnn_level_pool(int nprob, const float* const* src, const int* ld_src, const int32_t* const* list, const int32_t* const* off,
                      const int32_t* const* cnt, const int32_t* const* count, const int* max_items, const int* C, const int* col_off,
                      float* dst, int ld_dst, prcnn_stream_t stream);
+int prcnn_group_compact_pair_dst(const int32_t* idx_a, int ns_a, int T_a, const int32_t* idx_b, int ns_b, int T_b, const float* new_xyz,
+                                 int B, int N, int M, void* const* lists_a, void* const* lists_b, int32_t* rdst_a, int32_t* rdst_b,
+                                 int32_t* counts, prcnn_stream_t stream);
+int prcnn_level_pool_residual(int nprob, const float* const* src, const int* ld_src, const int32_t* const* list, const int32_t* const* off,
+                              const int32_t* const* cnt, const int32_t* const* count, const int* max_items, const int* C, const int* col_off,
+                              float* dst, int ld_dst, prcnn_stream_t stream);
 
 size_t prcnn_scene_workspace_bytes(int64_t total_points, int B);
 int prcnn_scene_prepare(const float* raw, const int64_t* offsets, int B, int64_t total_points, int max_points_per_frame,
diff --git a/pointrcnn_amd/_cabi.py b/pointrcnn_amd/_cabi.py
--- a/pointrcnn_amd/_cabi.py
+++ b/pointrcnn_amd/_cabi.py
@@ -97,6 +97,7 @@
     "prcnn_mlp_chain_group": (_I, [_P, _P, _P, _P, _I, _I, _I, _I, _I, _I, _P, _P, _I, _P, _P, _P, _P, _P, _I, _I, _I, _P, _P]),
     "prcnn_mlp_chain_interp": (_I, [_P, _I, _P, _P, _P, _I, _I, _I, _I, _I, _I, _P, _I, _P, _P, _P, _P, _P, _I, _I, _P]),
     "prcnn_mlp_chain_group_multi": (_I, [_I, _P, _P]),
+    "prcnn_mlp_chain_group_multi_dst": (_I, [_I, _P, _P, _P, _I, _P, _P]),
     "prcnn_maxpool_rows": (_I, [_P, _I, _L, _I, _I, _P, _I, _I, _P]),
     "prcnn_roipool3d": (_I, [_P, _P, _P, _I, _I, _I, _I, _I, _P, _P, _P]),
     "prcnn_roipool3d_work_bytes": (_Z, [_I, _I]),
@@ -124,6 +125,8 @@
     "prcnn_scatter_rows": (_I, [_P, _I, _P, _P, _I, _I, _P, _I, _I, _P]),
     "prcnn_group_compact_pair": (_I, [_P, _I, _I, _P, _I, _I, _P, _I, _I, _I, _P, _P, _P, _P]),
     "prcnn_level_pool": (_I, [_I, _P, _P, _P, _P, _P, _P, _P, _P, _P, _P, _I, _P]),
+    "prcnn_group_compact_pair_dst": (_I, [_P, _I, _I, _P, _I, _I, _P, _I, _I, _I, _P, _P, _P, _P, _P, _P]),
+    "prcnn_level_pool_residual": (_I, [_I, _P, _P, _P, _P, _P, _P, _P, _P, _P, _P, _I, _P]),
     "prcnn_scene_workspace_bytes": (_Z, [_L, _I]),
     "prcnn_scene_prepare": (_I, [_P, _P, _I, _L, _I, _P, _P, _P, _I, ctypes.c_uint32, _P, _P, _P, _P, _P, _P, _Z, _P]),
     "prcnn_train_scene_workspace_bytes": (_Z, [_L, _I, _I, _I]),
diff --git a/pointrcnn_amd/csrc/dedup.hip b/pointrcnn_amd/csrc/dedup.hip
--- a/pointrcnn_amd/csrc/dedup.hip
+++ b/pointrcnn_amd/csrc/dedup.hip
@@ -14,6 +14,7 @@
     int32_t* counts;
     const int32_t* valid_n;
     int G, N, M, ns, T;
+    int32_t* rdst;
 };
 
 constexpr int COMPACT_THREADS = 1024;
@@ -87,6 +88,7 @@
         P.slist[j] = g; P.soff[j] = r0; P.scnt[j] = cnt;
         for (int s = 0; s < cnt; s++) {
             P.ridx[r0 + s] = b * P.N + row[s];
+            if (P.rdst) P.rdst[r0 + s] = cnt == 1 ? g : -1;
 #pragma unroll
             for (int c = 0; c < 3; c++) P.rnx[(size_t)(r0 + s) * 3 + c] = c3[c];
         }
@@ -182,6 +184,50 @@
     }
 }
 
+struct ResidualPoolParams {
+    const float* src[LEVEL_POOL_MAX];
+    const int32_t* list[LEVEL_POOL_MAX];
+    const int32_t* off[LEVEL_POOL_MAX];
+    const int32_t* cnt[LEVEL_POOL_MAX];
+    const int32_t* count[LEVEL_POOL_MAX];
+    int ld_src[LEVEL_POOL_MAX], C[LEVEL_POOL_MAX], col_off[LEVEL_POOL_MAX], lane_shift[LEVEL_POOL_MAX];
+    float* dst;
+    int ld_dst;
+};
+
+template <bool VEC>
+__global__ __launch_bounds__(256) void residual_pool_kernel(ResidualPoolParams L) {
+    const int q = blockIdx.y;
+    const float* __restrict__ src = L.src[q];
+    const int32_t* __restrict__ list = L.list[q];
+    const int32_t* __restrict__ off = L.off[q];
+    const int32_t* __restrict__ cnt = L.cnt[q];
+    const int ld_src = L.ld_src[q], C = L.C[q], sh = L.lane_shift[q];
+    const int groups = *L.count[q];
+    const int per_block = 256 >> sh, l = (int)threadIdx.x & ((1 << sh) - 1);
+    constexpr int W = VEC ? 4 : 1;
+    for (int j = (int)blockIdx.x * per_block + ((int)threadIdx.x >> sh); j < groups; j += (int)gridDim.x * per_block) {
+        const int rows = cnt[j];
+        if (rows < 2) continue;
+        const float* p = src + (size_t)off[j] * ld_src;
+        float* o = L.dst + (size_t)list[j] * L.ld_dst + L.col_off[q];
+        for (int c = l * W; c < C; c += W << sh) {
+            if constexpr (VEC) {
+                float4 m = *reinterpret_cast<const float4*>(p + c);
+                for (int r = 1; r < rows; r++) {
+                    const float4 v = *reinterpret_cast<const float4*>(p + r * ld_src + c);
+                    m.x = fmaxf(m.x, v.x); m.y = fmaxf(m.y, v.y); m.z = fmaxf(m.z, v.z); m.w = fmaxf(m.w, v.w);
+                }
+                *reinterpret_cast<float4*>(o + c) = m;
+            } else {
+                float m = p[c];
+                for (int r = 1; r < rows; r++) m = fmaxf(m, p[r * ld_src + c]);
+                o[c] = m;
+            }
+        }
+    }
+}
+
 static int compact_check(const char* who, int B, int N, int M, int nsample, int sparse_max) {
     PRCNN_REQUIRE(B >= 0 && N > 0 && M >= 0 && nsample > 0, "%s: bad shape B=%d N=%d M=%d nsample=%d", who, B, N, M, nsample);
     PRCNN_REQUIRE(sparse_max >= 1 && sparse_max <= nsample, "%s: sparse_max=%d (1..nsample)", who, sparse_max);
@@ -189,8 +235,8 @@
     return PRCNN_OK;
 }
 
-PRCNN_API int prcnn_group_compact_pair(const int32_t* idx_a, int ns_a, int T_a, const int32_t* idx_b, int ns_b, int T_b, const float* new_xyz,
-                                       int B, int N, int M, void* const* lists_a, void* const* lists_b, int32_t* counts, prcnn_stream_t stream) {
+static int compact_pair(const int32_t* idx_a, int ns_a, int T_a, const int32_t* idx_b, int ns_b, int T_b, const float* new_xyz, int B, int N, int M,
+                        void* const* lists_a, void* const* lists_b, int32_t* rdst_a, int32_t* rdst_b, int32_t* counts, prcnn_stream_t stream) {
     int rc = compact_check("prcnn_group_compact_pair", B, N, M, ns_a, T_a);
     if (rc) return rc;
     rc = compact_check("prcnn_group_compact_pair", B, N, M, ns_b, T_b);
@@ -210,6 +256,7 @@
         P[q].ridx = (int32_t*)L[0]; P[q].rnx = (float*)L[1]; P[q].slist = (int32_t*)L[2]; P[q].soff = (int32_t*)L[3]; P[q].scnt = (int32_t*)L[4];
         P[q].idxn = (int32_t*)L[5]; P[q].nxn = (float*)L[6]; P[q].listn = (int32_t*)L[7];
         P[q].counts = counts + 3 * q; P[q].valid_n = nullptr; P[q].G = B * M; P[q].N = N; P[q].M = M; P[q].ns = ns; P[q].T = T;
+        P[q].rdst = q ? rdst_b : rdst_a;
     }
     const dim3 grid(prcnn_divup(B * M, COMPACT_THREADS), 2);
     const bool vec = ((uintptr_t)idx_a % 16) == 0 && ((uintptr_t)idx_b % 16) == 0;
@@ -217,6 +264,18 @@
     else hipLaunchKernelGGL((group_compact_pair_kernel<0, 0>), grid, dim3(COMPACT_THREADS), 0, s, P[0], P[1]);
     PRCNN_LAUNCH_CHECK("prcnn_group_compact_pair");
     return PRCNN_OK;
+}
+
+PRCNN_API int prcnn_group_compact_pair(const int32_t* idx_a, int ns_a, int T_a, const int32_t* idx_b, int ns_b, int T_b, const float* new_xyz,
+                                       int B, int N, int M, void* const* lists_a, void* const* lists_b, int32_t* counts, prcnn_stream_t stream) {
+    return compact_pair(idx_a, ns_a, T_a, idx_b, ns_b, T_b, new_xyz, B, N, M, lists_a, lists_b, nullptr, nullptr, counts, stream);
+}
+
+PRCNN_API int prcnn_group_compact_pair_dst(const int32_t* idx_a, int ns_a, int T_a, const int32_t* idx_b, int ns_b, int T_b, const float* new_xyz,
+                                           int B, int N, int M, void* const* lists_a, void* const* lists_b, int32_t* rdst_a, int32_t* rdst_b,
+                                           int32_t* counts, prcnn_stream_t stream) {
+    PRCNN_REQUIRE(rdst_a && rdst_b, "prcnn_group_compact_pair_dst: null destination list");
+    return compact_pair(idx_a, ns_a, T_a, idx_b, ns_b, T_b, new_xyz, B, N, M, lists_a, lists_b, rdst_a, rdst_b, counts, stream);
 }
 
 PRCNN_API int prcnn_level_pool(int nprob, const float* const* src, const int* ld_src, const int32_t* const* list, const int32_t* const* off,
@@ -244,6 +303,38 @@
     return PRCNN_OK;
 }
 
+PRCNN_API int prcnn_level_pool_residual(int nprob, const float* const* src, const int* ld_src, const int32_t* const* list, const int32_t* const* off,
+                                        const int32_t* const* cnt, const int32_t* const* count, const int* max_items, const int* C, const int* col_off,
+                                        float* dst, int ld_dst, prcnn_stream_t stream) {
+    PRCNN_REQUIRE(nprob >= 1 && nprob <= LEVEL_POOL_MAX, "prcnn_level_pool_residual: nprob=%d (1..%d)", nprob, LEVEL_POOL_MAX);
+    PRCNN_REQUIRE(src && ld_src && list && off && cnt && count && max_items && C && col_off, "prcnn_level_pool_residual: null table");
+    ResidualPoolParams L = {};
+    int n = 0;
+    long need = 0;
+    bool vec = ((uintptr_t)dst % 16) == 0 && ld_dst % 4 == 0;
+    for (int q = 0; q < nprob; q++) {
+        PRCNN_REQUIRE(max_items[q] >= 0 && C[q] > 0 && ld_src[q] >= C[q] && ld_dst >= col_off[q] + C[q] && col_off[q] >= 0,
+                      "prcnn_level_pool_residual: bad shape of problem %d", q);
+        if (max_items[q] == 0) continue;
+        PRCNN_REQUIRE(src[q] && list[q] && off[q] && cnt[q] && count[q] && dst, "prcnn_level_pool_residual: null pointer in problem %d", q);
+        L.src[n] = src[q]; L.list[n] = list[q]; L.off[n] = off[q]; L.cnt[n] = cnt[q]; L.count[n] = count[q];
+        L.ld_src[n] = ld_src[q]; L.C[n] = C[q]; L.col_off[n] = col_off[q];
+        vec = vec && ((uintptr_t)src[q] % 16) == 0 && (ld_src[q] | C[q] | col_off[q]) % 4 == 0;
+        int sh = 3;
+        while (sh < 6 && (4 << sh) < C[q]) sh++;
+        L.lane_shift[n] = sh;
+        need = max(need, (long)prcnn_divup((long)max_items[q], 256 >> sh));
+        n++;
+    }
+    if (n == 0) return PRCNN_OK;
+    L.dst = dst; L.ld_dst = ld_dst;
+    const dim3 grid((unsigned)min(need, (long)(DEDUP_GRID_CAP / 4)), n);
+    if (vec) hipLaunchKernelGGL(residual_pool_kernel<true>, grid, dim3(256), 0, (hipStream_t)stream, L);
+    else hipLaunchKernelGGL(residual_pool_kernel<false>, grid, dim3(256), 0, (hipStream_t)stream, L);
+    PRCNN_LAUNCH_CHECK("prcnn_level_pool_residual");
+    return PRCNN_OK;
+}
+
 PRCNN_API int prcnn_group_compact(const int32_t* idx, const float* new_xyz, int B, int N, int M, int nsample, int sparse_max,
                                   const int32_t* valid_n, int32_t* ridx, float* rnx, int32_t* slist, int32_t* soff, int32_t* scnt,
                                   int32_t* idxn, float* nxn, int32_t* listn, int32_t* counts, prcnn_stream_t stream) {
@@ -258,7 +349,7 @@
     PRCNN_REQUIRE(sparse_max == nsample || (idxn && nxn && listn), "prcnn_group_compact: null dense-list pointer");
     CompactParams P;
     P.idx = idx; P.new_xyz = new_xyz; P.ridx = ridx; P.rnx = rnx; P.slist = slist; P.soff = soff; P.scnt = scnt;
-    P.idxn = idxn; P.nxn = nxn; P.listn = listn;
+    P.idxn = idxn; P.nxn = nxn; P.listn = listn; P.rdst = nullptr;
     P.counts = counts; P.valid_n = valid_n; P.G = B * M; P.N = N; P.M = M; P.ns = nsample; P.T = sparse_max;
     const dim3 grid(prcnn_divup(P.G, COMPACT_THREADS));
     const bool vec = ((uintptr_t)idx % 16) == 0;
diff --git a/pointrcnn_amd/csrc/mlp.hip b/pointrcnn_amd/csrc/mlp.hip
--- a/pointrcnn_amd/csrc/mlp.hip
+++ b/pointrcnn_amd/csrc/mlp.hip
@@ -46,7 +46,16 @@
     int addy_phase;
     const void* wsplit;
     int split_terms;
+    const int32_t* row_dst;
+    const int32_t* grp_dst;
+    float* out2;
+    int ld_out2, col_off2;
 };
+
+__device__ __forceinline__ float* row_dst_base(const MlpParams& P, long row) {
+    const int d = P.row_dst[row];
+    return d >= 0 ? P.out2 + (long)d * P.ld_out2 + P.col_off2 : P.out + row * P.ld_out + P.col_off;
+}
 
 __device__ __forceinline__ long tile_of_block(const MlpParams& P, long bid) {
     if (P.xcd_tpf > 0) {
@@ -1132,10 +1141,11 @@
 __device__ __forceinline__ void chain_store(const ChainParams& C, f32x16 (&acc)[NB], int Nlast, long row, bool valid,
                                             int lane, int h) {
     const MlpParams& P = C.a;
-    const bool vec = ((P.ld_out | P.col_off) % 4 == 0) && aligned16(P.out);
+    const bool remap = P.pool_ns == 0 ? P.row_dst != nullptr : P.grp_dst != nullptr;
+    const bool vec = ((P.ld_out | P.col_off) % 4 == 0) && aligned16(P.out) && (!remap || (((P.ld_out2 | P.col_off2) % 4 == 0) && aligned16(P.out2)));
     if (P.pool_ns == 0) {
         if (!valid) return;
-        float* o = P.out + row * P.ld_out + P.col_off;
+        float* o = remap ? row_dst_base(P, row) : P.out + row * P.ld_out + P.col_off;
 #pragma unroll
         for (int ob = 0; ob < NB; ob++)
 #pragma unroll
@@ -1157,6 +1167,7 @@
     const long group = P.pool_ns == 16 ? (row / 16) : (row / 32);
     const long groups = P.rows / P.pool_ns;
     float* o = P.out + group * P.ld_out + P.col_off;
+    if (remap && writer && valid && group < groups) o = P.out2 + (long)P.grp_dst[group] * P.ld_out2 + P.col_off2;
 #pragma unroll
     for (int ob = 0; ob < NB; ob++)
 #pragma unroll
@@ -2474,7 +2485,25 @@
         const int n = nb * 32 + j;
         const bool n_ok = n < Cin.N1;
         const float bias = (Cin.bias1 && n_ok) ? Cin.bias1[n] : 0.f;
-        if (row0 + 32 <= P.rows && nb * 32 + 32 <= Cin.N1) {
+        if (P.row_dst) {
+            const int32_t* rd = P.row_dst;
+            asm volatile("" : "+s"(rd));
+            int d[16];
+#pragma unroll
+            for (int r = 0; r < 16; r++) d[r] = rd[min(row0 + (r & 3) + 8 * (r >> 2) + 4 * h, P.rows - 1)];
+            auto store_rows = [&](auto guarded) {
+#pragma unroll
+                for (int r = 0; r < 16; r++) {
+                    const long g = row0 + (r & 3) + 8 * (r >> 2) + 4 * h;
+                    float v = acc[0][r] + bias;
+                    v = Cin.relu1 ? fmaxf(v, 0.f) : v;
+                    float* o = d[r] >= 0 ? P.out2 + (long)d[r] * P.ld_out2 + P.col_off2 : P.out + g * P.ld_out + P.col_off;
+                    if (!decltype(guarded)::value || (n_ok && g < P.rows)) o[n] = v;
+                }
+            };
+            if (row0 + 32 <= P.rows && nb * 32 + 32 <= Cin.N1) store_rows(std::false_type{});
+            else store_rows(std::true_type{});
+        } else if (row0 + 32 <= P.rows && nb * 32 + 32 <= Cin.N1) {
             float* o = P.out + (row0 + 4 * h) * P.ld_out + P.col_off + n;
             const long ld = P.ld_out;
 #pragma unroll
@@ -2498,7 +2527,7 @@
     }
 }
 template <int NBW0>
-__global__ __launch_bounds__(256, 1) void mlp_stack2_kernel(const ChainParams Cin) {
+__global__ __launch_bounds__(256, (NBW0 <= 2 ? 2 : 1)) void mlp_stack2_kernel(const ChainParams Cin) {
     extern __shared__ __attribute__((aligned(16))) float st_lds[];
     mlp_stack2_body<NBW0>(Cin, blockIdx.x, gridDim.x, -1, st_lds);
 }
diff --git a/pointrcnn_amd/csrc/mlp_multi.h b/pointrcnn_amd/csrc/mlp_multi.h
--- a/pointrcnn_amd/csrc/mlp_multi.h
+++ b/pointrcnn_amd/csrc/mlp_multi.h
@@ -38,7 +38,7 @@
 }
 
 template <int NBWA, int NBWB>
-__global__ __launch_bounds__(256, 1) void stack2_multi_kernel(const MultiParams M) {
+__global__ __launch_bounds__(256, (NBWA <= 2 ? 2 : 1)) void stack2_multi_kernel(const MultiParams M) {
     extern __shared__ __attribute__((aligned(16))) float st_lds[];
     int prob, local, count;
     level_units_find(M.U, blockIdx.x, prob, local, count);
@@ -50,9 +50,11 @@
 
 #define STACK_MULTI_GRID_CAP 2048L
 
-PRCNN_API int prcnn_mlp_chain_group_multi(int nprob, const prcnn_chain_group_problem_t* prob, prcnn_stream_t stream) {
+static int chain_group_multi(int nprob, const prcnn_chain_group_problem_t* prob, const int32_t* const* dst, float* out2, int ld_out2,
+                             const int* col_off2, prcnn_stream_t stream) {
     PRCNN_REQUIRE(nprob >= 1 && nprob <= LEVEL_MAX_PROBLEMS && prob, "prcnn_mlp_chain_group_multi: nprob=%d (1..%d) or a null table", nprob,
                   LEVEL_MAX_PROBLEMS);
+    PRCNN_REQUIRE(!dst || (out2 && col_off2 && ld_out2 > 0), "prcnn_mlp_chain_group_multi_dst: destination lists without an output to store to");
     MultiParams M = {};
     MlpLaunch L[LEVEL_MAX_PROBLEMS];
     int n = 0, family = K_NONE;
@@ -63,6 +65,12 @@
         int rc = fill_chain_group(C, a.xyz, a.new_xyz, a.idx, a.feat_cl, a.ld_feat, a.B, a.N, a.M, a.nsample, a.C, a.act_wx, a.act_bias, a.nlayers, a.wpack,
                                   a.bias, a.nout, a.relu, a.out, a.ld_out, a.col_off, a.pool_ns, a.groups_dev);
         if (rc) return rc;
+        if (dst && dst[q]) {
+            PRCNN_REQUIRE(col_off2[q] >= 0 && ld_out2 >= col_off2[q] + a.nout[a.nlayers - 1], "prcnn_mlp_chain_group_multi_dst: ld_out2=%d < col_off2+Nout of problem %d",
+                          ld_out2, q);
+            (a.pool_ns ? C.a.grp_dst : C.a.row_dst) = dst[q];
+            C.a.out2 = out2; C.a.ld_out2 = ld_out2; C.a.col_off2 = col_off2[q];
+        }
         L[n] = MlpLaunch();
         rc = decide_chain(MODE_GROUP, C, L[n]);
         if (rc) return rc;
@@ -130,3 +138,12 @@
 #undef X
     return PRCNN_EUNSUPPORTED;
 }
+
+PRCNN_API int prcnn_mlp_chain_group_multi(int nprob, const prcnn_chain_group_problem_t* prob, prcnn_stream_t stream) {
+    return chain_group_multi(nprob, prob, nullptr, nullptr, 0, nullptr, stream);
+}
+
+PRCNN_API int prcnn_mlp_chain_group_multi_dst(int nprob, const prcnn_chain_group_problem_t* prob, const int32_t* const* dst, float* out2,
+                                              int ld_out2, const int* col_off2, prcnn_stream_t stream) {
+    return chain_group_multi(nprob, prob, dst, out2, ld_out2, col_off2, stream);
+}
diff --git a/pointrcnn_amd/dropin/pointnet2_lib/pointnet2/pointnet2_modules.py b/pointrcnn_amd/dropin/pointnet2_lib/pointnet2/pointnet2_modules.py
--- a/pointrcnn_amd/dropin/pointnet2_lib/pointnet2/pointnet2_modules.py
+++ b/pointrcnn_amd/dropin/pointnet2_lib/pointnet2/pointnet2_modules.py
@@ -15,6 +15,7 @@
 STACK_ALL_FLAT = os.environ.get("PRCNN_STACK_ALL_FLAT", "1") != "0"
 STACK_ALL_FLAT_MAX_ROWS = 1 << 20
 LEVEL_MERGE = os.environ.get("PRCNN_LEVEL_MERGE", "1") != "0"
+POOL_DIRECT = os.environ.get("PRCNN_POOL_DIRECT", "1") != "0"
 DENSE_CHUNK_BYTES = int(float(os.environ.get("PRCNN_DENSE_CHUNK_MB", "2048")) * 2 ** 20) or (1 << 62)
 TRAIN_FUSED = os.environ.get("PRCNN_TRAIN_FUSED", "1") != "0"
 TRAIN_DEDUP = os.environ.get("PRCNN_TRAIN_DEDUP", "1") != "0"
@@ -272,26 +273,40 @@
             scales.append((ns, src, act, layers, all_flat))
         (ns_a, _, _, _, flat_a), (ns_b, _, _, _, flat_b) = scales
         sps = ops.GroupSplit.pair(idxs[0], ns_a if flat_a else max(1, ns_a // DEDUP_SPARSE_DIV),
-                                  idxs[1], ns_b if flat_b else max(1, ns_b // DEDUP_SPARSE_DIV), new_xyz, N)
+                                  idxs[1], ns_b if flat_b else max(1, ns_b // DEDUP_SPARSE_DIV), new_xyz, N, rdst=POOL_DIRECT)
         xyz_f = xyz.view(1, B * N, 3)
         dst = out_cl.view(B * M, -1)
-        flat, dense, pools, col = [], [], [], 0
         order = sorted(range(2), key=lambda i: -sum(l.nout for l in scales[i][3]) * scales[i][0])
         cols = [0, c_outs[0]]
-        for i in order:
-            (ns, src, act, layers, all_flat), sp, col = scales[i], sps[i], cols[i]
-            src_f = None if src is None else _flatten_frames(src)
-            t1 = torch.empty((sp.max_rows, c_outs[i]), dtype=torch.float32, device=xyz.device)
-            flat.append(dict(xyz=xyz_f, new_xyz=sp.rnx, idx=sp.ridx, feat_cl=src_f, layers=layers, out=(t1, 0), pool_ns=0, act=act, groups_dev=sp.rows))
-            pools.append((t1, sp, col, "flat"))
-            if not all_flat:
-                tn = torch.empty((sp.G, c_outs[i]), dtype=torch.float32, device=xyz.device)
-                dense.append(dict(xyz=xyz_f, new_xyz=sp.nxn, idx=sp.idxn, feat_cl=src_f, layers=layers, out=(tn, 0), pool_ns=ns, act=act,
-                                  groups_dev=sp.count_dense))
-                pools.append((tn, sp, col, "dense"))
-        if not ops.mlp_chain_group_multi(flat + dense):
-            for pr in flat + dense:
-                ops.mlp_chain_group(**pr)
+
+        def problems(direct):
+            flat, dense, pools = [], [], []
+            for i in order:
+                (ns, src, act, layers, all_flat), sp, col = scales[i], sps[i], cols[i]
+                src_f = None if src is None else _flatten_frames(src)
+                t1 = torch.empty((sp.max_rows, c_outs[i]), dtype=torch.float32, device=xyz.device)
+                flat.append(dict(xyz=xyz_f, new_xyz=sp.rnx, idx=sp.ridx, feat_cl=src_f, layers=layers, out=(t1, 0), pool_ns=0, act=act, groups_dev=sp.rows))
+                pools.append((t1, sp, col, "flat"))
+                if not all_flat:
+                    tn = None if direct else torch.empty((sp.G, c_outs[i]), dtype=torch.float32, device=xyz.device)
+                    dense.append(dict(xyz=xyz_f, new_xyz=sp.nxn, idx=sp.idxn, feat_cl=src_f, layers=layers, out=(dst, col) if direct else (tn, 0), pool_ns=ns,
+                                      act=act, groups_dev=sp.count_dense))
+                    if direct:
+                        dense[-1]["dst"] = (sp.listn, dst, col)
+                    else:
+                        pools.append((tn, sp, col, "dense"))
+                if direct:
+                    flat[-1]["dst"] = (sp.rdst, dst, col)
+            return flat + dense, pools
+
+        stacks, pools = problems(POOL_DIRECT)
+        if ops.mlp_chain_group_multi(stacks):
+            ops.level_pool(pools, dst, residual=POOL_DIRECT)
+            return True
+        if POOL_DIRECT:
+            stacks, pools = problems(False)
+        for pr in stacks:
+            ops.mlp_chain_group(**pr)
         ops.level_pool(pools, dst)
         return True
 
diff --git a/pointrcnn_amd/ops.py b/pointrcnn_amd/ops.py
--- a/pointrcnn_amd/ops.py
+++ b/pointrcnn_amd/ops.py
@@ -387,6 +387,10 @@
 
 
 def mlp_chain_group_multi(problems):
+    by_dst = [pr["dst"] for pr in problems if pr.get("dst") is not None]
+    out2 = by_dst[0][1] if by_dst else None
+    if any(d[1] is not out2 for d in by_dst):
+        raise RuntimeError("mlp_chain_group_multi: the problems that store by destination must share one output")
     arr = (_cabi.ChainGroupProblem * len(problems))()
     for q, pr in zip(arr, problems):
         layers = pr["layers"]
@@ -400,10 +404,15 @@
         q.out, q.groups_dev = _p(buf), _p(pr.get("groups_dev"))
         q.ld_feat, q.B, q.N, q.M, q.nsample, q.C, q.nlayers = ld_feat, B, N, M, ns, C, a.n
         q.ld_out, q.col_off, q.pool_ns = ld_out, col_off, pr.get("pool_ns", 0)
-    rc = _cabi.lib().prcnn_mlp_chain_group_multi(len(problems), arr, _stream())
+    if out2 is None:
+        rc = _cabi.lib().prcnn_mlp_chain_group_multi(len(problems), arr, _stream())
+    else:
+        dst = (ctypes.c_void_p * len(problems))(*[_p(pr["dst"][0]) if pr.get("dst") is not None else None for pr in problems])
+        col2 = (ctypes.c_int * len(problems))(*[int(pr["dst"][2]) if pr.get("dst") is not None else 0 for pr in problems])
+        rc = _cabi.lib().prcnn_mlp_chain_group_multi_dst(len(problems), arr, dst, _p(out2), _row_stride(out2), col2, _stream())
     if rc == _cabi.EUNSUPPORTED:
         return False
-    _cabi.check(rc, "prcnn_mlp_chain_group_multi")
+    _cabi.check(rc, "prcnn_mlp_chain_group_multi_dst" if out2 is not None else "prcnn_mlp_chain_group_multi")
     return True
 
 
@@ -1165,13 +1174,18 @@
         return (ctypes.c_void_p * 8)(*[_p(t) for t in (self.ridx, self.rnx, self.slist, self.soff, self.scnt, self.idxn, self.nxn, self.listn)])
 
     @staticmethod
-    def pair(idx_a, sparse_max_a, idx_b, sparse_max_b, new_xyz, N):
+    def pair(idx_a, sparse_max_a, idx_b, sparse_max_b, new_xyz, N, rdst=False):
         if idx_a.shape[:2] != idx_b.shape[:2]:
             raise RuntimeError("GroupSplit.pair: the two index tensors must share (B, M)")
         counts = torch.empty((6,), dtype=_INT, device=idx_a.device)
         a = GroupSplit(idx_a, new_xyz, N, sparse_max_a, counts=counts[0:3])
         b = GroupSplit(idx_b, new_xyz, N, sparse_max_b, counts=counts[3:6])
         B, M, _ = idx_a.shape
+        if rdst:
+            a.rdst, b.rdst = torch.empty_like(a.ridx), torch.empty_like(b.ridx)
+            _cabi.check(_cabi.lib().prcnn_group_compact_pair_dst(_p(idx_a), a.ns, a.T, _p(idx_b), b.ns, b.T, _p(new_xyz), B, N, M, a._lists(), b._lists(),
+                                                                 _p(a.rdst), _p(b.rdst), _p(counts), _stream()), "prcnn_group_compact_pair_dst")
+            return a, b
         _cabi.check(_cabi.lib().prcnn_group_compact_pair(_p(idx_a), a.ns, a.T, _p(idx_b), b.ns, b.T, _p(new_xyz), B, N, M, a._lists(), b._lists(),
                                                          _p(counts), _stream()), "prcnn_group_compact_pair")
         return a, b
@@ -1189,7 +1203,7 @@
                                                dst.stride(-2), int(col_off), _stream()), "prcnn_scatter_rows")
 
 
-def level_pool(problems, dst):
+def level_pool(problems, dst, residual=False):
     n = len(problems)
     P, I = ctypes.c_void_p * n, ctypes.c_int * n
     src, ld, lst, off, cnt, count, cap, C, col = P(), I(), P(), P(), P(), P(), I(), I(), I()
@@ -1198,7 +1212,8 @@
         src[q], ld[q], C[q], col[q], cap[q] = _p(s), s.stride(-2), s.shape[-1], int(c0), sp.G
         lst[q], count[q] = (_p(sp.slist), _p(sp.count_sparse)) if flat else (_p(sp.listn), _p(sp.count_dense))
         off[q], cnt[q] = (_p(sp.soff), _p(sp.scnt)) if flat else (None, None)
-    _cabi.check(_cabi.lib().prcnn_level_pool(n, src, ld, lst, off, cnt, count, cap, C, col, _p(dst), dst.stride(-2), _stream()), "prcnn_level_pool")
+    name = "prcnn_level_pool_residual" if residual else "prcnn_level_pool"
+    _cabi.check(getattr(_cabi.lib(), name)(n, src, ld, lst, off, cnt, count, cap, C, col, _p(dst), dst.stride(-2), _stream()), name)
 
 
 def _frames(raw, offsets, calib, *img_hw):
```
